# chrisquince/DESMAN

Measured on AMD Instinct MI355X. Metric: Gibbs iterations/sec (VxS updates/s) at V=10k S=64 G=8, higher is better.
Workload: dtype f64; 1 GPU; synthetic V=10000 x S=64, G=8, full Gibbs iteration, 1 chain per GPU (configs[2]); V=10000, S=64, G=8, chains=1, tau_rng=mt19937

## Files before the change

### desman_amd/_lib.py

```python
import ctypes as C
import os

import numpy as np

_HERE = os.path.dirname(os.path.abspath(__file__))
LIB_PATH = os.environ.get("DESMAN_HIP_LIB") or os.path.join(_HERE, "lib", "libdesman_hip.so")
AB_LIB_PATH = os.path.join(_HERE, "lib", "libdesman_hip_ab.so")
HEADER_PATH = os.path.join(os.path.dirname(_HERE), "include", "desman_hip.h")

DSM_OK = 0
RNG_MT19937, RNG_PHILOX = 0, 1
STATS_AGG = 2
K_NAMES = ("stats", "dirichlet", "tau", "finalize", "mt", "nmft_a", "nmft_gamma", "nmft_b", "stats2", "stats_big", "stats_pat")


class DesmanHipError(RuntimeError):
    pass


_i64p = np.ctypeslib.ndpointer(np.int64, flags="C_CONTIGUOUS")
_f64p = np.ctypeslib.ndpointer(np.float64, flags="C_CONTIGUOUS")
_u64p = np.ctypeslib.ndpointer(np.uint64, flags="C_CONTIGUOUS")
_u32p = np.ctypeslib.ndpointer(np.uint32, flags="C_CONTIGUOUS")
_i32p = np.ctypeslib.ndpointer(np.int32, flags="C_CONTIGUOUS")
_vp, _i, _d = C.c_void_p, C.c_int, C.c_double

SIGNATURES = {
    "dsm_last_error": (C.c_char_p, []),
    "dsm_device_count": (_i, []),
    "dsm_version": (C.c_char_p, []),
    "dsm_initRNG": (_i, []),
    "dsm_setRNG": (_i, [C.c_ulong]),
    "dsm_freeRNG": (_i, []),
    "dsm_sample_tau": (_i, [_i64p, _f64p, _f64p, _i64p, _i, _i, _i]),
    "c_initRNG": (None, []),
    "c_setRNG": (None, [C.c_ulong]),
    "c_freeRNG": (None, []),
    "c_sample_tau": (_i, [_i64p, _f64p, _f64p, _i64p, _i, _i, _i]),
    "dsm_getRNG_state": (_i, [_u32p]),
    "dsm_setRNG_state": (_i, [_u32p]),
    "dsm_ctx_create": (_i, [C.POINTER(_vp), _i]),
    "dsm_ctx_destroy": (_i, [_vp]),
    "dsm_ctx_sync": (_i, [_vp]),
    "dsm_ctx_set_counts": (_i, [_vp, _i64p, _i, _i]),
    "dsm_ctx_set_state": (_i, [_vp, _i64p, _f64p, _f64p, _i]),
    "dsm_ctx_get_state": (_i, [_vp, _vp, _vp, _vp]),
    "dsm_ctx_set_gamma_eta": (_i, [_vp, _vp, _vp]),
    "dsm_ctx_set_priors": (_i, [_vp, _d, _d, _d]),
    "dsm_ctx_seed": (_i, [_vp, C.c_ulong, C.c_uint64]),
    "dsm_ctx_set_tau_rng": (_i, [_vp, _i]),
    "dsm_ctx_get_mt_state": (_i, [_vp, _u32p]),
    "dsm_ctx_set_mt_state": (_i, [_vp, _u32p]),
    "dsm_mt_seed_state": (_i, [C.c_ulong, _u32p]),
    "dsm_ctx_debug_mt_fill": (_i, [_vp, C.c_size_t, _u32p]),
    "dsm_ctx_sample_tau": (_i, [_vp, C.POINTER(_i), _vp]),
    "dsm_ctx_sample_stats": (_i, [_vp, C.c_uint32, _u64p, _u64p]),
    "dsm_ctx_stats_spec": (_i, [_vp]),
    "dsm_ctx_sweep_stats": (_i, [_vp, C.POINTER(C.c_uint64), C.POINTER(C.c_uint64), _i]),
    "dsm_ctx_set_tau_screen": (_i, [_vp, _i]),
    "dsm_ctx_set_tau_neartie": (_i, [_vp, _i]),
    "dsm_ctx_set_nmft_fused": (_i, [_vp, _i]),
    "dsm_ctx_set_nmft_persist": (_i, [_vp, _i]),
    "dsm_ctx_tau_launch_info": (_i, [_vp, C.POINTER(_i), C.POINTER(_i)]),
    "dsm_ctx_debug_log2f": (_i, [_vp, _vp, _vp, C.c_size_t]),
    "dsm_debug_fdiv": (_i, [_i, _f64p, _f64p, _f64p, _i]),
    "dsm_release_device_caches": (_i, []),
    "dsm_ctx_force_stats_spec": (_i, [_vp, _i]),
    "dsm_ctx_debug_stage1": (_i, [_vp, C.c_uint32, _vp, _u64p]),
    "dsm_ctx_debug_binom": (_i, [_vp, _i, C.c_uint32, _f64p, C.c_uint64, _i, _u32p, _i]),
    "dsm_ctx_draw_gamma_eta": (_i, [_vp, C.c_uint32, _u64p, _u64p, _f64p, _f64p]),
    "dsm_ctx_loglik": (_i, [_vp, C.POINTER(_d), C.POINTER(_d)]),
    "dsm_ctx_gibbs_update": (_i, [_vp, _i]),
    "dsm_ctx_get_counters": (_i, [_vp, C.POINTER(C.c_uint64), C.POINTER(C.c_uint32)]),
    "dsm_ctx_set_counters": (_i, [_vp, C.c_uint64, C.c_uint32]),
    "dsm_ctx_get_screen_state": (_i, [_vp, _u32p]),
    "dsm_ctx_set_screen_state": (_i, [_vp, _u32p]),
    "dsm_ctx_gibbs_update_sharded": (_i, [_vp, _i, _i, _i, _vp, _vp]),
    "dsm_ctx_gibbs_update_sharded_comm": (_i, [_vp, _i, _i, _i, _vp]),
    "dsm_comm_unique_id": (_i, [_vp]),
    "dsm_comm_create": (_i, [C.POINTER(_vp), _vp, _i, _i, _i]),
    "dsm_comm_destroy": (_i, [_vp]),
    "dsm_comm_rank": (_i, [_vp]),
    "dsm_comm_world": (_i, [_vp]),
    "dsm_comm_allgather_f64": (_i, [_vp, _f64p, _f64p, C.c_size_t]),
    "dsm_comm_allreduce_f64": (_i, [_vp, _vp, C.c_size_t, _i]),
    "dsm_comm_barrier": (_i, [_vp]),
    "dsm_device_read": (_i, [_i, _vp, _vp, C.c_size_t]),
    "dsm_device_write": (_i, [_i, _vp, _vp, C.c_size_t]),
    "dsm_batch_gibbs_update": (_i, [C.POINTER(_vp), _i, _i]),
    "dsm_batch_update_tau": (_i, [C.POINTER(_vp), _i, _i, C.POINTER(_vp), C.POINTER(_vp)]),
    "dsm_batch_nmft_factorize": (_i, [C.POINTER(_vp), _i, _i, _d, _i, C.POINTER(_i), _vp]),
    "dsm_ctx_update_tau": (_i, [_vp, _i, _f64p, _f64p]),
    "dsm_ctx_get_trace": (_i, [_vp, _vp, _vp, _vp, _vp, _vp]),
    "dsm_ctx_get_star": (_i, [_vp, _vp, _vp, _vp, C.POINTER(_d), C.POINTER(_i)]),
    "dsm_ctx_get_tau_sum": (_i, [_vp, _i64p]),
    "dsm_ctx_get_tau_at": (_i, [_vp, _i, _i64p]),
    "dsm_nmft_set": (_i, [_vp, _f64p, _f64p, _i]),
    "dsm_nmft_get": (_i, [_vp, _vp, _vp]),
    "dsm_nmft_factorize": (_i, [_vp, _i, _d, _i, C.POINTER(_i), _vp]),
    "dsm_nmft_objective": (_i, [_vp, C.POINTER(_d)]),
    "dsm_nmft_debug_path": (_i, [_vp, _i, C.POINTER(_i)]),
    "dsm_nmft_get_tau": (_i, [_vp, _i64p]),
    "dsm_lrt_step": (_i, [_i, _f64p, _i32p, _i32p, _f64p, _d, _i, _i, _f64p, _f64p, _f64p]),
    "dsm_assign_tau": (_i, [_i, _i64p, _i, _i, _i, _f64p, _f64p, C.c_uint64, _vp, _vp, _vp, _vp, _vp]),
    "dsm_ctx_assign_tau": (_i, [_vp, _f64p, _f64p, _i, C.c_uint64, _vp, _vp, _vp, _vp, _vp]),
    "dsm_assign_debug_set_chunk": (_i, [_i]),
    "dsm_fit_gamma": (_i, [_i, _i64p, _i, _i, _i, _i64p, _f64p, _i, _d, _i, _vp, _vp, _vp, _vp, _vp, _vp]),
    "dsm_ctx_fit_gamma": (_i, [_vp, _i, _vp, _f64p, _i, _d, _i, _vp, _vp, _vp, _vp, _vp, _vp]),
    "dsm_abund_debug_set_chunk": (_i, [_i]),
    "dsm_fit_gamma_interval": (_i, [_i, _i64p, _i, _i, _i, _i64p, _f64p, _f64p, _d, _i, _d, _d, _vp, _vp, _vp]),
    "dsm_ctx_fit_gamma_interval": (_i, [_vp, _i, _vp, _f64p, _f64p, _d, _i, _d, _d, _vp, _vp, _vp]),
    "dsm_genes_create": (_i, [C.POINTER(_vp), _i]),
    "dsm_genes_destroy": (_i, [_vp]),
    "dsm_genes_set_data": (_i, [_vp, _vp, _i, _i, _i, _i32p, _f64p]),
    "dsm_genes_set_model": (_i, [_vp, _f64p, _f64p, _f64p, _i, _i, _f64p, _f64p, _f64p]),
    "dsm_genes_set_state": (_i, [_vp, _vp, _vp]),
    "dsm_genes_get_state": (_i, [_vp, _vp, _vp]),
    "dsm_genes_seed": (_i, [_vp, C.c_ulong, C.c_uint64]),
    "dsm_genes_set_gene_base": (_i, [_vp, _i]),
    "dsm_genes_get_mt_state": (_i, [_vp, _u32p]),
    "dsm_genes_set_mt_state": (_i, [_vp, _u32p]),
    "dsm_genes_nmft_tau": (_i, [_vp, _vp, _f64p, _i, _d, _vp]),
    "dsm_genes_sweep_all": (_i, [_vp, _vp, _i, _vp, _vp, _vp]),
    "dsm_genes_step_candidates": (_i, [_vp, _i, _i, _f64p, _vp]),
    "dsm_genes_step_choose": (_i, [_vp, _i, _i, _i]),
    "dsm_genes_update": (_i, [_vp, _i, _i, _vp, _vp, _vp, _vp]),
    "dsm_genes_loglik": (_i, [_vp, _vp]),
    "dsm_genes_get_star": (_i, [_vp, _vp, _vp]),
    "dsm_genes_set_star": (_i, [_vp, _vp, _vp]),
    "dsm_genes_debug_tile": (_i, [_vp, C.POINTER(_i), C.POINTER(_i), C.POINTER(_i), C.POINTER(C.c_size_t)]),
    "dsm_kl_assign": (_i, [_i, _f64p, _f64p, _f64p, _i, _i, _i, _i, _d, C.POINTER(_i), C.POINTER(_d)]),
    "dsm_ctx_set_timing": (_i, [_vp, _i]),
    "dsm_ctx_get_timing": (_i, [_vp, _vp, _vp]),
    "dsm_kernel_name": (C.c_char_p, [_i]),
}

EXCHANGE_FN = C.CFUNCTYPE(C.c_int, C.c_void_p, C.c_void_p, C.c_size_t, C.c_void_p, C.c_size_t)
_lib = None


def _digest(a):
    try:
        import xxhash
# ... 259 lines not shown
        return dict(tau=tau, gamma=gamma, eta=eta, mt_state=mt, ctr_seed=np.uint64(key), iter_ctr=np.uint32(it), screen=self.screen_state())

    def counters(self):
        key, it = C.c_uint64(0), C.c_uint32(0)
        check(self.lib.dsm_ctx_get_counters(self._h, C.byref(key), C.byref(it)))
        return int(key.value), int(it.value)

    def screen_state(self):
        out = np.zeros(2, dtype=np.uint32)
        check(self.lib.dsm_ctx_get_screen_state(self._h, out))
        return out

    def set_screen_state(self, words):
        check(self.lib.dsm_ctx_set_screen_state(self._h, np.ascontiguousarray(words, dtype=np.uint32)))

    def restore(self, ck):
        self.set_state(np.ascontiguousarray(ck["tau"], dtype=np.int64), np.ascontiguousarray(ck["gamma"], dtype=np.float64),
                       np.ascontiguousarray(ck["eta"], dtype=np.float64))
        mt = np.asarray(ck["mt_state"], dtype=np.uint32)
        if mt.size == 625:
            self.set_mt_state(np.ascontiguousarray(mt))
        check(self.lib.dsm_ctx_set_counters(self._h, int(ck["ctr_seed"]), int(ck["iter_ctr"])))
        self.set_screen_state(ck["screen"] if "screen" in ck else np.zeros(2, dtype=np.uint32))

    def set_mt_state(self, st):
        check(self.lib.dsm_ctx_set_mt_state(self._h, np.ascontiguousarray(st, dtype=np.uint32)))

    def debug_mt_fill(self, n):
        out = np.empty(int(n), dtype=np.uint32)
        check(self.lib.dsm_ctx_debug_mt_fill(self._h, int(n), out))
        return out

    def set_tau_rng(self, mode):
        check(self.lib.dsm_ctx_set_tau_rng(self._h, int(mode)))

    def assign_tau(self, gamma, eta, seed=None):
        gamma, eta = _assign_model(gamma, eta, self.S)
        G = gamma.shape[1]
        out = _assign_out(self.V, G, seed)
        check(self.lib.dsm_ctx_assign_tau(self._h, gamma, eta, G, int(seed or 0) & 0xFFFFFFFFFFFFFFFF, _ptr(out["map_state"]),
                                          _ptr(out["conf"]), _ptr(out["logz"]), _ptr(out["marg"]), _ptr(out.get("draw_state"))))
        return out

    def fit_gamma(self, eta, tau=None, max_iter=FIT_MAX_ITER, tol=FIT_TOL, presence=False):
        eta = _fit_eta(eta)
        t = None if tau is None else _fit_tau(tau, self.V)
        G = self.G if t is None else t.shape[1]
        out = _fit_out(self.S, G, presence)
        check(self.lib.dsm_ctx_fit_gamma(self._h, G, _ptr(t), eta, int(max_iter), float(tol), int(bool(presence)), _ptr(out["gamma"]),
                                         _ptr(out["loglik"]), _ptr(out["deviance"]), _ptr(out["iters"]), _ptr(out["converged"]),
                                         _ptr(out.get("lr_absent"))))
        return out

    def fit_gamma_interval(self, eta, gamma_hat, tau=None, level=0.95, q=None, max_iter=FIT_MAX_ITER, tol=FIT_TOL, ctol=FIT_CTOL):
        eta = _fit_eta(eta)
        t = None if tau is None else _fit_tau(tau, self.V)
        G = self.G if t is None else t.shape[1]
        g, q, out = _interval_args(gamma_hat, self.S, G, level, q)
        check(self.lib.dsm_ctx_fit_gamma_interval(self._h, G, _ptr(t), eta, g, q, int(max_iter), float(tol), float(ctol), _ptr(out["lo"]),
                                                  _ptr(out["hi"]), _ptr(out["flags"])))
        return out

    def sample_tau(self, want_logp=False):
        n = _i(0)
        logp = np.empty((self.V, self.G, 4)) if want_logp else None
        check(self.lib.dsm_ctx_sample_tau(self._h, C.byref(n), _ptr(logp)))
        return (n.value, logp) if want_logp else n.value

    def sample_stats(self, it):
        mu = np.zeros((self.S, self.G), dtype=np.uint64)
        E = np.zeros((4, 4), dtype=np.uint64)
        check(self.lib.dsm_ctx_sample_stats(self._h, int(it), mu, E))
        return mu, E

    def debug_log2f(self, x):
        x = np.ascontiguousarray(x, dtype=np.float32)
        out = np.empty_like(x)
        check(self.lib.dsm_ctx_debug_log2f(self._h, x.ctypes.data, out.ctypes.data, x.size))
        return out

    def set_tau_neartie(self, mode=-1):
        check(self.lib.dsm_ctx_set_tau_neartie(self._h, int(mode)))

    def set_tau_screen(self, on):
        check(self.lib.dsm_ctx_set_tau_screen(self._h, 1 if on else 0))

    def tau_launch_info(self):
        a, b = _i(0), _i(0)
        check(self.lib.dsm_ctx_tau_launch_info(self._h, C.byref(a), C.byref(b)))
        return a.value, b.value

    def set_nmft_persist(self, mode=-1):
        check(self.lib.dsm_ctx_set_nmft_persist(self._h, int(mode)))

    def set_nmft_fused(self, mode=-1):
        check(self.lib.dsm_ctx_set_nmft_fused(self._h, int(mode)))

    def sweep_stats(self, reset=False):
        a, b = C.c_uint64(0), C.c_uint64(0)
        check(self.lib.dsm_ctx_sweep_stats(self._h, C.byref(a), C.byref(b), 1 if reset else 0))
        return a.value, b.value

    def stats_spec(self):
        r = self.lib.dsm_ctx_stats_spec(self._h)
        if r < 0:
            check(r)
        return r

    def force_stats_spec(self, spec=0):
        check(self.lib.dsm_ctx_force_stats_spec(self._h, int(spec)))

    def debug_stage1(self, it):
        nt = np.zeros((self.S, 1 << self.G), dtype=np.uint32)
        E = np.zeros((4, 4), dtype=np.uint64)
        check(self.lib.dsm_ctx_debug_stage1(self._h, int(it), nt.ctypes.data, E))
        return nt, E

    def debug_binom(self, kind, n, w, seed, nsamp, spec=STATS_AGG):
        w4 = np.zeros(4)
        w4[:len(w)] = w
        out = np.zeros((nsamp, 4) if kind == 2 else nsamp, dtype=np.uint32)
        check(self.lib.dsm_ctx_debug_binom(self._h, int(kind), int(n), w4, int(seed), int(nsamp), out.reshape(-1), int(spec)))
        return out

    def draw_gamma_eta(self, it, sum_mu, esum):
        g = np.empty((self.S, self.G)); e = np.empty((4, 4))
        check(self.lib.dsm_ctx_draw_gamma_eta(self._h, int(it), np.ascontiguousarray(sum_mu, dtype=np.uint64),
                                              np.ascontiguousarray(esum, dtype=np.uint64), g, e))
        return g, e

    def loglik(self):
        ll, lp = _d(0), _d(0)
        check(self.lib.dsm_ctx_loglik(self._h, C.byref(ll), C.byref(lp)))
        return ll.value, lp.value

    def gibbs_update(self, n_iter):
        check(self.lib.dsm_ctx_gibbs_update(self._h, int(n_iter)))
        self.n_trace = int(n_iter)

    def gibbs_update_sharded(self, n_iter, v_offset, v_total, exchange):
        err = []

        def cb(user, tab, n_tab, vec, n_vec):
            try:
                exchange(tab or 0, int(n_tab), vec, int(n_vec))
                return 0
            except BaseException as e:
                err.append(e)
                return 1
        fn = EXCHANGE_FN(cb)
        rc = self.lib.dsm_ctx_gibbs_update_sharded(self._h, int(n_iter), int(v_offset), int(v_total), C.cast(fn, _vp), None)
        if err:
            raise err[0]
        check(rc)
        self.n_trace = int(n_iter)

    def gibbs_update_sharded_comm(self, n_iter, v_offset, v_total, comm):
        check(self.lib.dsm_ctx_gibbs_update_sharded_comm(self._h, int(n_iter), int(v_offset), int(v_total), comm._h))
        self.n_trace = int(n_iter)

    @staticmethod
    def batch_gibbs_update(ctxs, n_iter):
        ctxs = list(ctxs)
        arr = (_vp * len(ctxs))(*[c._h.value for c in ctxs])
        check(load().dsm_batch_gibbs_update(arr, len(ctxs), int(n_iter)))
        for c in ctxs:
            c.n_trace = int(n_iter)

    def update_tau(self, gamma_store, eta_store):
        g = np.ascontiguousarray(gamma_store, dtype=np.float64)
        e = np.ascontiguousarray(eta_store, dtype=np.float64)
        check(self.lib.dsm_ctx_update_tau(self._h, g.shape[0], g, e))
        self.n_trace = g.shape[0]

    def get_trace(self):
        n = self.n_trace
        ll = np.empty(n); lp = np.empty(n); nch = np.empty(n, dtype=np.int32)
        g = np.empty((n, self.S, self.G)); e = np.empty((n, 4, 4))
        check(self.lib.dsm_ctx_get_trace(self._h, _ptr(ll), _ptr(lp), _ptr(nch), _ptr(g), _ptr(e)))
        return dict(ll=ll, lp=lp, nchange=nch, gamma=g, eta=e)

    def get_star(self):
        tau = np.empty((self.V, self.G, 4), dtype=np.int64)
        g = np.empty((self.S, self.G)); e = np.empty((4, 4))
        lp, it = _d(0), _i(0)
        check(self.lib.dsm_ctx_get_star(self._h, _ptr(tau), _ptr(g), _ptr(e), C.byref(lp), C.byref(it)))
        return dict(tau=tau, gamma=g, eta=e, lp=lp.value, it=it.value)

    def get_tau_sum(self):
        out = np.empty((self.V, self.G, 4), dtype=np.int64)
        check(self.lib.dsm_ctx_get_tau_sum(self._h, out))
        return out

    def get_tau_at(self, it):
        out = np.empty((self.V, self.G, 4), dtype=np.int64)
        check(self.lib.dsm_ctx_get_tau_at(self._h, int(it), out))
        return out

    def nmft_set(self, tau, gamma):
# ... 199 lines not shown
```

### desman_amd/csrc/api.hip

```cpp
#include <math.h>
#include <stdarg.h>
#include <stdio.h>
#include <string.h>

#include <algorithm>
#include <mutex>
#include <numeric>
#include <thread>

#include "dsm_host.h"
#include "log_table.h"

static thread_local char g_err[512] = "";

void dsm_set_error(const char *fmt, ...)
{
    va_list ap;
    va_start(ap, fmt);
    vsnprintf(g_err, sizeof g_err, fmt, ap);
    va_end(ap);
}

extern "C" const char *dsm_last_error(void) { return g_err; }
extern "C" const char *dsm_version(void) { return "desman_hip 0.1 (gfx950)"; }
// ... 81 lines not shown
static void dev_free(T **p) { if (*p) { (void)hipFree(*p); *p = nullptr; } }

template <typename T>
struct Scratch {
    T *p = nullptr;
    ~Scratch() { if (p) (void)hipFree(p); }
    int alloc(size_t n) { return dev_alloc(&p, n); }
    operator T *() const { return p; }
    Scratch() = default;
    Scratch(const Scratch &) = delete;
    Scratch &operator=(const Scratch &) = delete;
};

#define TRY(x) do { int _r = (x); if (_r != DSM_OK) return _r; } while (0)
#define BIND(c) HIP_TRY(hipSetDevice((c)->device))

static int need(dsm_ctx *c, bool counts, bool state)
{
    if (!c) { dsm_set_error("null context"); return DSM_ERR_ARG; }
    if (counts && !c->cnt_vs) { dsm_set_error("no count tensor: call dsm_ctx_set_counts first"); return DSM_ERR_STATE; }
    if (state && !c->have_state) { dsm_set_error("no chain state: call dsm_ctx_set_state first"); return DSM_ERR_STATE; }
    return DSM_OK;
}

static int esum_reset(dsm_ctx *c)
{
    HIP_TRY(hipMemsetAsync(c->esum, 0, (16 + 16 * DSM_ESUM_PARTS) * sizeof(unsigned long long), c->stream));
    return DSM_OK;
}

static int reset_blk_order(dsm_ctx *c)
{
    static const std::vector<uint32_t> ident = [] { std::vector<uint32_t> v((size_t)2 * DSM_MAX_GRID); for (size_t i = 0; i < v.size(); ++i) v[i] = (uint32_t)(i % DSM_MAX_GRID); return v; }();
    c->blk_order_n[0] = c->blk_order_n[1] = 0;
    if (!c->blk_order) return DSM_OK;
    HIP_TRY(hipMemcpyAsync(c->blk_order, ident.data(), ident.size() * sizeof(uint32_t), hipMemcpyHostToDevice, c->stream));
    return DSM_OK;
}

extern "C" int dsm_ctx_create(dsm_ctx **out, int device)
{
    if (!out) return DSM_ERR_ARG;
    *out = nullptr;
    int n = dsm_device_count();
    if (n <= 0) { dsm_set_error("no HIP device visible"); return DSM_ERR_NODEVICE; }
    if (device < 0 || device >= n) { dsm_set_error("device %d out of range (0..%d)", device, n - 1); return DSM_ERR_ARG; }
    HIP_TRY(hipSetDevice(device));
    hipDeviceProp_t prop;
    HIP_TRY(hipGetDeviceProperties(&prop, device));
    if (strncmp(prop.gcnArchName, "gfx950", 6) != 0) {
        dsm_set_error("device %d is %s; this library is built for gfx950 only", device, prop.gcnArchName);
        return DSM_ERR_NODEVICE;
    }
    dsm_ctx *c = new dsm_ctx();
    c->device = device;
    HIP_TRY(hipStreamCreateWithFlags(&c->stream, hipStreamNonBlocking));
    if (getenv("DESMAN_HIP_ONE_STREAM")) c->stream_rng = c->stream;
    else {
        int lo = 0, hi = 0;
        HIP_TRY(hipDeviceGetStreamPriorityRange(&lo, &hi));
        HIP_TRY(hipStreamCreateWithPriority(&c->stream_rng, hipStreamNonBlocking, hi));
    }
    for (int i = 0; i < 2; ++i) {
        HIP_TRY(hipEventCreateWithFlags(&c->ev_u_ready[i], hipEventDisableTiming));
        HIP_TRY(hipEventCreateWithFlags(&c->ev_u_free[i], hipEventDisableTiming));
    }
    TRY(dev_alloc(&c->mt_state, 625));
    TRY(dev_alloc(&c->ll_partial, 2 * DSM_MAX_GRID));
    TRY(dev_alloc(&c->nchange, 2));
    TRY(dev_alloc(&c->sweep_stats, 2));
    HIP_TRY(hipMemsetAsync(c->sweep_stats, 0, 2 * sizeof(unsigned long long), c->stream));
    TRY(dev_alloc(&c->step_cnt, (size_t)2 * 2 * DSM_MAX_GRID));
    HIP_TRY(hipMemsetAsync(c->step_cnt, 0, (size_t)2 * 2 * DSM_MAX_GRID * sizeof(uint32_t), c->stream));
    TRY(dev_alloc(&c->blk_order, (size_t)2 * DSM_MAX_GRID));
    TRY(reset_blk_order(c));
    TRY(dev_alloc(&c->screen_ctl, 4));
    HIP_TRY(hipMemsetAsync(c->screen_ctl, 0, 4 * sizeof(uint32_t), c->stream));
    TRY(dev_alloc(&c->prior, 2 * (DSM_MAX_S + 4)));
    TRY(dev_alloc(&c->scalars, 8));
    TRY(dev_alloc(&c->star, 2));
    TRY(dev_alloc(&c->eta, 16));
    TRY(dev_alloc(&c->eta_new, 16));
    TRY(dev_alloc(&c->eta_star, 16));
    TRY(dev_alloc(&c->esum, 16 + 16 * DSM_ESUM_PARTS));
    TRY(dev_alloc(&c->log_tab, 2 * DSM_LOG_TAB_N + DSM_EXP_TAB_N));
    HIP_TRY(hipMemcpyAsync(c->log_tab, dsm_log_table_host, sizeof dsm_log_table_host, hipMemcpyHostToDevice, c->stream));
    HIP_TRY(hipMemcpyAsync(c->log_tab + 2 * DSM_LOG_TAB_N, dsm_exp_table_host, sizeof dsm_exp_table_host, hipMemcpyHostToDevice, c->stream));
    HIP_TRY(hipMemsetAsync(c->nchange, 0, 2 * sizeof(int), c->stream));
    TRY(esum_reset(c));
    HIP_TRY(hipStreamSynchronize(c->stream));
    *out = c;
    return DSM_OK;
}

static void free_traces(dsm_ctx *c)
{
    dev_free(&c->tau_trace); dev_free(&c->ll_trace); dev_free(&c->lp_trace); dev_free(&c->nchange_trace);
    dev_free(&c->gamma_trace); dev_free(&c->eta_trace); dev_free(&c->gamma_in); dev_free(&c->eta_in);
    c->in_cap = 0;
    c->n_trace = 0;
    c->trace_cap = 0;
}

extern "C" int dsm_ctx_destroy(dsm_ctx *c)
{
    if (!c) return DSM_OK;
    (void)hipSetDevice(c->device);
    (void)hipStreamSynchronize(c->stream);
    collect_spans(c);
    for (auto e : c->free_events) (void)hipEventDestroy(e);
    free_traces(c);
    dev_free(&c->cnt_vs); dev_free(&c->items); dev_free(&c->nitems); dev_free(&c->tau);
    dev_free(&c->pat_rep); dev_free(&c->pat_x); dev_free(&c->pat_list); c->pat_rep_len = c->pat_x_len = 0;
    if (c->h_rare) { (void)hipHostFree(c->h_rare); c->h_rare = nullptr; }
    dev_free(&c->s2_scratch);
    dev_free(&c->blk_tab); stats_release_ntab(c); dev_free(&c->big_list); dev_free(&c->big_count);
    dev_free(&c->gamma); dev_free(&c->eta);
    dev_free(&c->eta_new); dev_free(&c->sum_mu); dev_free(&c->esum); dev_free(&c->mt_state); dev_free(&c->mt_jstates); dev_free(&c->u_raw);
    dev_free(&c->ll_partial); dev_free(&c->nchange); dev_free(&c->sweep_stats); dev_free(&c->step_cnt); dev_free(&c->blk_order); dev_free(&c->screen_ctl); dev_free(&c->prior); dev_free(&c->prior_all); dev_free(&c->scalars); dev_free(&c->star);
    dev_free(&c->gamma_star); dev_free(&c->eta_star); dev_free(&c->log_tab); dev_free(&c->shard_vec); dev_free(&c->np_part); if (c->np_bar) { (void)hipFree(c->np_bar); c->np_bar = nullptr; } dev_free(&c->F); dev_free(&c->ntau); dev_free(&c->ntau2); dev_free(&c->ngam); dev_free(&c->ngam_raw);
    dev_free(&c->npart); dev_free(&c->nstat); dev_free(&c->ngam2); dev_free(&c->ngam_raw2);
    for (int i = 0; i < 2; ++i) { (void)hipEventDestroy(c->ev_u_ready[i]); (void)hipEventDestroy(c->ev_u_free[i]); }
    if (c->stream_rng != c->stream) (void)hipStreamDestroy(c->stream_rng);
    (void)hipStreamDestroy(c->stream);
    delete c;
    return DSM_OK;
}

extern "C" int dsm_ctx_sync(dsm_ctx *c)
{
    if (!c) return DSM_ERR_ARG;
    BIND(c);
    HIP_TRY(hipStreamSynchronize(c->stream));
    HIP_TRY(hipStreamSynchronize(c->stream_rng));
    return DSM_OK;
}

extern "C" int dsm_ctx_set_counts(dsm_ctx *c, const int64_t *variants, int V, int S)
{
    if (!c || !variants || V < 1 || S < 1) { dsm_set_error("set_counts: bad arguments"); return DSM_ERR_ARG; }
    if (S > DSM_MAX_S) { dsm_set_error("S=%d exceeds DSM_MAX_S=%d", S, DSM_MAX_S); return DSM_ERR_UNSUPPORTED; }
    if ((int64_t)V * S >= ((int64_t)1 << 32)) { dsm_set_error("V*S must be below 2^32"); return DSM_ERR_UNSUPPORTED; }
    BIND(c);
    HIP_TRY(hipStreamSynchronize(c->stream));
    HIP_TRY(hipStreamSynchronize(c->stream_rng));
    const size_t n = (size_t)V * S;
    c->V = V; c->S = S;
    c->have_state = false;
    c->G = 0;
    TRY(dev_alloc(&c->cnt_vs, n * 4));
    TRY(dev_alloc(&c->nitems, (size_t)S));
    TRY(dev_alloc(&c->tau, (size_t)V));
    dev_free(&c->F); dev_free(&c->ntau); dev_free(&c->ntau2); dev_free(&c->ngam); dev_free(&c->ngam_raw); c->nG = 0;
    free_traces(c);
    Scratch<int64_t> d_in; Scratch<int> d_flag; Scratch<double> d_part; Scratch<unsigned long long> d_depth;
    const int nblk = (int)((n + 255) / 256 < 1024 ? (n + 255) / 256 : 1024);
    TRY(d_in.alloc(n * 4));
    TRY(d_flag.alloc(1));
    TRY(d_part.alloc((size_t)nblk));
    TRY(d_depth.alloc((size_t)S));
    HIP_TRY(hipMemcpyAsync(d_in, variants, n * 4 * sizeof(int64_t), hipMemcpyHostToDevice, c->stream));
    HIP_TRY(hipMemsetAsync(d_flag, 0, sizeof(int), c->stream));
    HIP_TRY(hipMemsetAsync(d_depth, 0, (size_t)S * sizeof(unsigned long long), c->stream));
    TRY(k_convert_counts(c, d_in, d_flag, d_part, nblk, d_depth));
    std::vector<double> part(nblk);
    std::vector<unsigned long long> dep((size_t)S);
    int flag = 0;
    HIP_TRY(hipMemcpyAsync(part.data(), d_part, nblk * sizeof(double), hipMemcpyDeviceToHost, c->stream));
    HIP_TRY(hipMemcpyAsync(dep.data(), d_depth, (size_t)S * sizeof(unsigned long long), hipMemcpyDeviceToHost, c->stream));
    HIP_TRY(hipMemcpyAsync(&flag, d_flag, sizeof(int), hipMemcpyDeviceToHost, c->stream));
    HIP_TRY(hipStreamSynchronize(c->stream));
    c->items_built = false;
    c->max_items = 0;
    c->blk_gmax = 0;
    c->stats_grid = 0;
    dev_free(&c->pat_x); c->pat_x_len = 0;
    TRY(reset_blk_order(c));
    HIP_TRY(hipMemsetAsync(c->screen_ctl, 0, 4 * sizeof(uint32_t), c->stream));
    dev_free(&c->items);
    c->depth.assign((size_t)S, 0);
    c->max_depth = 0;
    for (int s = 0; s < S; ++s) { c->depth[s] = (int64_t)dep[s]; c->max_depth = std::max<uint64_t>(c->max_depth, dep[s]); }
    if (flag) {
        dev_free(&c->cnt_vs); dev_free(&c->items);
        dsm_set_error("set_counts: negative count or depth above 2^31-1");
        return DSM_ERR_ARG;
    }
    double s = 0.0;
    for (double p : part) s += p;
    c->ll_const = s;
    return DSM_OK;
}

int build_stats_items(dsm_ctx *c)
{
    const int V = c->V, S = c->S;
    std::vector<int32_t> cnt((size_t)V * S * 4);
    HIP_TRY(hipMemcpyAsync(cnt.data(), c->cnt_vs, cnt.size() * sizeof(int32_t), hipMemcpyDeviceToHost, c->stream));
    HIP_TRY(hipStreamSynchronize(c->stream));
    const int64_t cells = (int64_t)V * S;
    const int CH = cells <= 65536 ? 64 : cells <= 262144 ? 128 : 0;
    c->chunked = CH != 0;
    std::vector<int32_t> nit(S);
    std::vector<std::vector<std::pair<int32_t, int32_t>>> lst((size_t)S);
    std::vector<int32_t> top(S, 0);
    for (int s = 0; s < S; ++s) lst[s].reserve((size_t)V * 2);
    for (int v = 0; v < V; ++v) {
        const int32_t *row = cnt.data() + (size_t)v * S * 4;
        for (int s = 0; s < S; ++s)
            for (int b = 0; b < 4; ++b) {
                const int64_t x = row[s * 4 + b];
                if (x <= 0) continue;
                if (!CH) {
                    lst[s].emplace_back((int32_t)x, v * 4 + b);
                    if (x > top[s]) top[s] = (int32_t)x;
                } else {
                    for (int64_t j = 0; j * CH < x; ++j) {
                        const int32_t nrd = (int32_t)(x - j * CH < CH ? x - j * CH : CH);
                        lst[s].emplace_back(nrd | (int32_t)(j << 12), v * 4 + b);
                        if (nrd > top[s]) top[s] = nrd;
                    }
                }
            }
    }
    int max_items = 0;
    for (int s = 0; s < S; ++s) max_items = std::max(max_items, (int)lst[s].size());
    c->item_stride = max_items > 0 ? max_items : 1;
    std::vector<int32_t> items((size_t)S * c->item_stride * 2, 0);
    TRY(dev_alloc(&c->items, items.size()));
    std::vector<int32_t> first;
    const int32_t rd_mask = CH ? 0xfff : 0x7fffffff;
    for (int s = 0; s < S; ++s) {
        const auto &l = lst[s];
        nit[s] = (int32_t)l.size();
        int32_t *dst = items.data() + (size_t)s * c->item_stride * 2;
        if (top[s] <= (1 << 20)) {
            first.assign((size_t)top[s] + 2, 0);
            for (const auto &e : l) first[e.first & rd_mask]++;
            int32_t run = 0;
            for (int32_t cval = top[s]; cval >= 1; --cval) { const int32_t h = first[cval]; first[cval] = run; run += h; }
            for (const auto &e : l) { const int32_t k = first[e.first & rd_mask]++; dst[2 * k] = e.second; dst[2 * k + 1] = e.first; }
        } else {
            std::vector<std::pair<int32_t, int32_t>> t(l);
            std::stable_sort(t.begin(), t.end(), [](const std::pair<int32_t, int32_t> &p, const std::pair<int32_t, int32_t> &q) { return p.first > q.first; });
            for (size_t k = 0; k < t.size(); ++k) { dst[2 * k] = t[k].second; dst[2 * k + 1] = t[k].first; }
        }
    }
    c->max_items = max_items;
    c->nitems_h = nit;
    c->blk_gmax = 0;
    HIP_TRY(hipMemcpyAsync(c->items, items.data(), items.size() * sizeof(int32_t), hipMemcpyHostToDevice, c->stream));
    HIP_TRY(hipMemcpyAsync(c->nitems, nit.data(), (size_t)S * sizeof(int32_t), hipMemcpyHostToDevice, c->stream));
    HIP_TRY(hipStreamSynchronize(c->stream));
    c->items_built = true;
    return DSM_OK;
}

static int ensure_state_buffers(dsm_ctx *c, int G)
{
    if (G < 1 || G > DSM_MAX_G) { dsm_set_error("G=%d outside 1..%d", G, DSM_MAX_G); return DSM_ERR_UNSUPPORTED; }
    if (G != c->G || !c->gamma) {
        c->G = G;
        const size_t sg = (size_t)c->S * G;
        TRY(dev_alloc(&c->gamma, sg));
        TRY(dev_alloc(&c->gamma_star, sg));
        TRY(dev_alloc(&c->sum_mu, sg));
        HIP_TRY(hipMemsetAsync(c->sum_mu, 0, sg * sizeof(unsigned long long), c->stream));
        c->stats_grid = 0;
        c->u_cap = (size_t)c->V * G;
        c->u_chunk_words = c->u_cap * std::max<size_t>(1, std::min<size_t>(DSM_U_CHUNK, ((size_t)16 << 20) / std::max<size_t>(1, c->u_cap)));
        TRY(dev_alloc(&c->u_raw, 2 * c->u_chunk_words));
        free_traces(c);
    }
    return DSM_OK;
}

extern "C" int dsm_ctx_set_state(dsm_ctx *c, const int64_t *tau, const double *gamma, const double *eta, int G)
{
    TRY(need(c, true, false));
    if (!tau || !gamma || !eta) { dsm_set_error("set_state: null pointer"); return DSM_ERR_ARG; }
    BIND(c);
    HIP_TRY(hipStreamSynchronize(c->stream));
    TRY(ensure_state_buffers(c, G));
    const size_t nt = (size_t)c->V * G * 4;
    Scratch<int64_t> d_t;
    TRY(d_t.alloc(nt));
    HIP_TRY(hipMemcpyAsync(d_t, tau, nt * sizeof(int64_t), hipMemcpyHostToDevice, c->stream));
    TRY(k_pack_tau(c, d_t, c->tau, c->V, G));
    HIP_TRY(hipMemcpyAsync(c->gamma, gamma, (size_t)c->S * G * sizeof(double), hipMemcpyHostToDevice, c->stream));
    c->tau_rare_n = tau_rare_from_host(gamma, c->S, G);
    HIP_TRY(hipMemcpyAsync(c->eta, eta, 16 * sizeof(double), hipMemcpyHostToDevice, c->stream));
    HIP_TRY(hipStreamSynchronize(c->stream));
    c->have_state = true;
    return DSM_OK;
}

extern "C" int dsm_ctx_set_gamma_eta(dsm_ctx *c, const double *gamma, const double *eta)
{
    TRY(need(c, true, true));
    BIND(c);
    if (gamma) HIP_TRY(hipMemcpyAsync(c->gamma, gamma, (size_t)c->S * c->G * sizeof(double), hipMemcpyHostToDevice, c->stream));
    if (gamma) c->tau_rare_n = tau_rare_from_host(gamma, c->S, c->G);
    if (eta) HIP_TRY(hipMemcpyAsync(c->eta, eta, 16 * sizeof(double), hipMemcpyHostToDevice, c->stream));
    HIP_TRY(hipStreamSynchronize(c->stream));
    return DSM_OK;
}

static int fetch_tau(dsm_ctx *c, const uint64_t *d_packed, int64_t *host_onehot)
{
    const size_t nt = (size_t)c->V * c->G * 4;
    Scratch<int64_t> d_t;
    TRY(d_t.alloc(nt));
    TRY(k_unpack_tau(c, d_packed, d_t, c->V, c->G));
    HIP_TRY(hipMemcpyAsync(host_onehot, d_t, nt * sizeof(int64_t), hipMemcpyDeviceToHost, c->stream));
    HIP_TRY(hipStreamSynchronize(c->stream));
    return DSM_OK;
}

extern "C" int dsm_ctx_get_state(dsm_ctx *c, int64_t *tau, double *gamma, double *eta)
{
    TRY(need(c, true, true));
    BIND(c);
    if (tau) TRY(fetch_tau(c, c->tau, tau));
    if (gamma) HIP_TRY(hipMemcpyAsync(gamma, c->gamma, (size_t)c->S * c->G * sizeof(double), hipMemcpyDeviceToHost, c->stream));
    if (eta) HIP_TRY(hipMemcpyAsync(eta, c->eta, 16 * sizeof(double), hipMemcpyDeviceToHost, c->stream));
    HIP_TRY(hipStreamSynchronize(c->stream));
    return DSM_OK;
}

extern "C" int dsm_ctx_set_priors(dsm_ctx *c, double alpha, double delta, double epsilon)
{
    if (!c || !(alpha > 0) || !(delta > 0) || !(epsilon >= 0)) { dsm_set_error("set_priors: bad value"); return DSM_ERR_ARG; }
    c->alpha = alpha; c->delta = delta; c->epsilon = epsilon;
    return DSM_OK;
}

static void mt_seed_host(uint32_t *st, unsigned long seed)
{
    if (seed == 0) seed = 4357;
    st[0] = (uint32_t)(seed & 0xffffffffUL);
    for (int i = 1; i < 624; ++i) st[i] = 1812433253u * (st[i - 1] ^ (st[i - 1] >> 30)) + (uint32_t)i;
    st[624] = 624;
}

static int seed_mt(dsm_ctx *c, unsigned long seed)
{
    uint32_t st[625];
    mt_seed_host(st, seed);
    HIP_TRY(hipStreamSynchronize(c->stream_rng));
    HIP_TRY(hipMemcpyAsync(c->mt_state, st, sizeof st, hipMemcpyHostToDevice, c->stream));
    HIP_TRY(hipStreamSynchronize(c->stream));
    c->mt_seeded = true;
    return DSM_OK;
}

extern "C" int dsm_ctx_seed(dsm_ctx *c, unsigned long mt_seed, uint64_t ctr_seed)
{
    if (!c) return DSM_ERR_ARG;
    BIND(c);
    c->ctr_seed = ctr_seed;
    c->iter_ctr = 0;
    return seed_mt(c, mt_seed);
}

extern "C" int dsm_ctx_get_screen_state(dsm_ctx *c, uint32_t *out2)
{
    if (!c || !out2) { dsm_set_error("get_screen_state: null argument"); return DSM_ERR_ARG; }
    BIND(c);
    HIP_TRY(hipMemcpyAsync(out2, c->screen_ctl, 2 * sizeof(uint32_t), hipMemcpyDeviceToHost, c->stream));
    HIP_TRY(hipStreamSynchronize(c->stream));
    return DSM_OK;
}
extern "C" int dsm_ctx_set_screen_state(dsm_ctx *c, const uint32_t *in2)
{
    if (!c || !in2) { dsm_set_error("set_screen_state: null argument"); return DSM_ERR_ARG; }
// ... 110 lines not shown
            if (filled < total) TRY(fill_next());
            HIP_TRY(hipStreamWaitEvent(c->stream, c->ev_u_ready[slot], 0));
        }
        *u = c->u_raw + (size_t)slot * c->u_chunk_words + (size_t)(it - first[slot]) * c->u_cap;
        return DSM_OK;
    }
    int release(int it)
    {
        if (!active()) return DSM_OK;
        for (int slot = 0; slot < 2; ++slot)
            if (len[slot] && it == first[slot] + len[slot] - 1) HIP_TRY(hipEventRecord(c->ev_u_free[slot], c->stream));
        return DSM_OK;
    }
};

extern "C" int dsm_ctx_sample_tau(dsm_ctx *c, int *nchange, double *logp_out)
{
    TRY(need(c, true, true));
    BIND(c);
    Scratch<double> d_logp;
    const size_t nl = (size_t)c->V * c->G * 4;
    if (logp_out) TRY(d_logp.alloc(nl));
    const uint32_t *u = nullptr;
    SweepWords words(c, 1);
    HIP_TRY(hipMemsetAsync(c->nchange, 0, sizeof(int), c->stream));
    TRY(words.acquire(0, &u));
    TRY(k_tau_sweep(c, 1, c->gamma, c->eta, c->eta, nullptr, d_logp, c->iter_ctr++, nullptr, u));
    TRY(words.release(0));
    int n = 0;
    HIP_TRY(hipMemcpyAsync(&n, c->nchange, sizeof(int), hipMemcpyDeviceToHost, c->stream));
    if (logp_out) HIP_TRY(hipMemcpyAsync(logp_out, d_logp, nl * sizeof(double), hipMemcpyDeviceToHost, c->stream));
    HIP_TRY(hipMemsetAsync(c->nchange, 0, sizeof(int), c->stream));
    HIP_TRY(hipStreamSynchronize(c->stream));
    if (nchange) *nchange = n;
    return DSM_OK;
}

extern "C" int dsm_ctx_sample_stats(dsm_ctx *c, uint32_t iter, uint64_t *sum_mu, uint64_t *esum)
{
    TRY(need(c, true, true));
    BIND(c);
    const size_t sg = (size_t)c->S * c->G;
    HIP_TRY(hipMemsetAsync(c->sum_mu, 0, sg * sizeof(unsigned long long), c->stream));
    TRY(stats_ensure_ntab(c));
    TRY(esum_reset(c));
    TRY(k_stats(c, iter));
    TRY(k_esum_fold(c));
    if (sum_mu) HIP_TRY(hipMemcpyAsync(sum_mu, c->sum_mu, sg * sizeof(uint64_t), hipMemcpyDeviceToHost, c->stream));
    if (esum) HIP_TRY(hipMemcpyAsync(esum, c->esum, 16 * sizeof(uint64_t), hipMemcpyDeviceToHost, c->stream));
    HIP_TRY(hipMemsetAsync(c->sum_mu, 0, sg * sizeof(unsigned long long), c->stream));
    TRY(esum_reset(c));
    HIP_TRY(hipStreamSynchronize(c->stream));
    return DSM_OK;
}

extern "C" int dsm_ctx_stats_spec(dsm_ctx *c)
{
    if (!c || c->G < 1) { dsm_set_error("stats_spec: no chain state"); return DSM_ERR_STATE; }
    return stats_spec(c);
}

extern "C" int dsm_ctx_force_stats_spec(dsm_ctx *c, int spec)
{
    if (!c || spec < 0 || spec > 4) { dsm_set_error("force_stats_spec: 0 (rule), 1, 2, 3 or 4"); return DSM_ERR_ARG; }
    c->force_stats_spec = spec;
    return DSM_OK;
}

extern "C" int dsm_ctx_debug_stage1(dsm_ctx *c, uint32_t iter, uint32_t *ntab, uint64_t *esum)
{
    TRY(need(c, true, true));
    if (stats_spec(c) < 2) { dsm_set_error("debug_stage1: the aggregated specification does not apply to this shape (force it with dsm_ctx_force_stats_spec)"); return DSM_ERR_UNSUPPORTED; }
    BIND(c);
    TRY(esum_reset(c));
    TRY(k_stats_stage1(c, iter));
    TRY(k_esum_fold(c));
    const size_t NH = (size_t)1 << c->G, S = (size_t)c->S;
    const size_t ld = (size_t)c->ntab_ld;
    std::vector<uint32_t> t((size_t)c->ntab_rep * NH * ld);
    HIP_TRY(hipMemcpyAsync(t.data(), c->ntab, t.size() * sizeof(uint32_t), hipMemcpyDeviceToHost, c->stream));
    if (esum) HIP_TRY(hipMemcpyAsync(esum, c->esum, 16 * sizeof(uint64_t), hipMemcpyDeviceToHost, c->stream));
    HIP_TRY(hipMemsetAsync(c->ntab, 0, t.size() * sizeof(uint32_t), c->stream));
    TRY(esum_reset(c));
    HIP_TRY(hipMemsetAsync(c->big_count, 0, DSM_BIG_NT * DSM_BIG_NL * DSM_BIG_STRIDE * sizeof(uint32_t), c->stream));
    HIP_TRY(hipStreamSynchronize(c->stream));
    if (ntab)
        for (size_t h = 0; h < NH; ++h)
            for (size_t s = 0; s < S; ++s) {
                uint32_t v = 0;
                for (int r = 0; r < c->ntab_rep; ++r) v += t[((size_t)r * NH + ((h * DSM_NTAB_HMUL + (s >> 4) * DSM_NTAB_SWZ) & (NH - 1))) * ld + s];
                ntab[s * NH + h] = v;
            }
    return DSM_OK;
}

extern "C" int dsm_ctx_debug_binom(dsm_ctx *c, int kind, uint32_t n, const double *w4, uint64_t seed, int nsamp, uint32_t *out, int spec)
{
    if (!c || !w4 || !out || nsamp < 1 || kind < 0 || kind > 2 || spec < 2 || spec > 3) { dsm_set_error("debug_binom: bad arguments"); return DSM_ERR_ARG; }
    BIND(c);
    const size_t len = (size_t)nsamp * (kind == 2 ? 4 : 1);
    Scratch<uint32_t> d;
    TRY(d.alloc(len));
    TRY(k_binom_test(c, kind, n, w4, seed, nsamp, d, spec));
    HIP_TRY(hipMemcpyAsync(out, d, len * sizeof(uint32_t), hipMemcpyDeviceToHost, c->stream));
    HIP_TRY(hipStreamSynchronize(c->stream));
    return DSM_OK;
}

extern "C" int dsm_ctx_draw_gamma_eta(dsm_ctx *c, uint32_t iter, const uint64_t *sum_mu, const uint64_t *esum,
                                      double *gamma_out, double *eta_out)
{
    TRY(need(c, true, true));
    if (!sum_mu || !esum) { dsm_set_error("draw_gamma_eta: null sums"); return DSM_ERR_ARG; }
    BIND(c);
    const size_t sg = (size_t)c->S * c->G;
    Scratch<double> d_g, d_e;
    TRY(d_g.alloc(sg));
    TRY(d_e.alloc(16));
    HIP_TRY(hipMemcpyAsync(c->sum_mu, sum_mu, sg * sizeof(uint64_t), hipMemcpyHostToDevice, c->stream));
    HIP_TRY(hipMemcpyAsync(c->esum, esum, 16 * sizeof(uint64_t), hipMemcpyHostToDevice, c->stream));
    TRY(k_dirichlet(c, iter, d_g, nullptr, d_e, nullptr, c->prior, -1, 0, nullptr));
    if (gamma_out) HIP_TRY(hipMemcpyAsync(gamma_out, d_g, sg * sizeof(double), hipMemcpyDeviceToHost, c->stream));
    if (eta_out) HIP_TRY(hipMemcpyAsync(eta_out, d_e, 16 * sizeof(double), hipMemcpyDeviceToHost, c->stream));
    HIP_TRY(hipStreamSynchronize(c->stream));
    return DSM_OK;
}

static int eval_state(dsm_ctx *c, const double *gamma, const double *eta, uint64_t *trace_slot, int star_mode)
{
    int nb = 0;
    TRY(k_prior(c, gamma, eta, c->prior));
    TRY(k_tau_sweep(c, 2, gamma, eta, eta, trace_slot, nullptr, 0, &nb, nullptr));
    return k_finalize(c, nb, -1, star_mode, c->prior, gamma, eta);
}

extern "C" int dsm_ctx_loglik(dsm_ctx *c, double *ll, double *lp)
{
    TRY(need(c, true, true));
    BIND(c);
    double sc[2];
    TRY(eval_state(c, c->gamma, c->eta, nullptr, 2));
    HIP_TRY(hipMemcpyAsync(sc, c->scalars, sizeof sc, hipMemcpyDeviceToHost, c->stream));
    HIP_TRY(hipStreamSynchronize(c->stream));
    if (ll) *ll = sc[0];
    if (lp) *lp = sc[1];
    return DSM_OK;
}

static int alloc_traces(dsm_ctx *c, int n)
{
    const size_t sg = (size_t)c->S * c->G;
    if (n > c->trace_cap || !c->tau_trace) {
        free_traces(c);
        const int want = n;
        if (n < 512 && (size_t)513 * c->V * sizeof(uint64_t) <= ((size_t)1 << 30)) n = 512;
        TRY(dev_alloc(&c->tau_trace, (size_t)(n + 1) * c->V));
        TRY(dev_alloc(&c->ll_trace, (size_t)n));
        TRY(dev_alloc(&c->lp_trace, (size_t)n));
        TRY(dev_alloc(&c->nchange_trace, (size_t)n));
        TRY(dev_alloc(&c->gamma_trace, (size_t)n * sg));
        TRY(dev_alloc(&c->eta_trace, (size_t)n * 16));
        c->trace_cap = n;
        n = want;
    }
    c->n_trace = n;
    return DSM_OK;
}

thread_local BatchCtl g_batch;

struct Chains {
    dsm_ctx *const *c;
    int K;
    bool batched;
    struct Home { hipStream_t stream, stream_rng; bool timing; int nmft_fused; };
    std::vector<Home> home;
    dsm_ctx *lead() const { return c[0]; }
    ~Chains()
    {
        if (home.empty()) return;
        (void)hipStreamSynchronize(lead()->stream);
        (void)hipStreamSynchronize(lead()->stream_rng);
        for (size_t k = 0; k < home.size(); ++k) {
            c[k]->stream = home[k].stream; c[k]->stream_rng = home[k].stream_rng; c[k]->timing = home[k].timing; c[k]->nmft_fused = home[k].nmft_fused;
        }
    }
    template <class Fits> int open(bool state, bool nmft, Fits fits)
    {
        if (!c || K < 1 || K > DSM_MAX_BATCH) { dsm_set_error("batch of %d chains (1..%d)", K, DSM_MAX_BATCH); return DSM_ERR_ARG; }
        for (int k = 0; k < K; ++k) {
            TRY(need(c[k], true, state));
            const dsm_ctx *a = c[0], *b = c[k];
            if (b->device != a->device || b->V != a->V || b->S != a->S) { dsm_set_error("batch: chain %d differs from chain 0 in device or shape", k); return DSM_ERR_ARG; }
            TRY(fits(a, b, k));
            for (int j = 0; j < k; ++j) if (c[j] == b) { dsm_set_error("batch: chain %d listed twice", k); return DSM_ERR_ARG; }
        }
        BIND(lead());
        for (int k = 0; batched && k < K; ++k) {
            HIP_TRY(hipStreamSynchronize(c[k]->stream));
            HIP_TRY(hipStreamSynchronize(c[k]->stream_rng));
            home.push_back(Home{c[k]->stream, c[k]->stream_rng, c[k]->timing, c[k]->nmft_fused});
            c[k]->stream = lead()->stream; c[k]->stream_rng = lead()->stream_rng; c[k]->timing = false;
            if (nmft) c[k]->nmft_fused = home[0].nmft_fused;
        }
        return DSM_OK;
    }
    template <class F> int each(F f) const
    {
        for (int k = 0; k < K; ++k) TRY(f(c[k], k));
        return DSM_OK;
    }
    template <class F> int launch(F f) const
    {
        int r = DSM_OK;
        for (int k = 0; k < K && r == DSM_OK; ++k) {
            if (batched) g_batch = BatchCtl{K, k};
            r = f(c[k], k);
        }
        g_batch = BatchCtl{};
        return r;
    }
};

static int same_G_and_rng(const dsm_ctx *a, const dsm_ctx *b, int k)
{
    if (b->G != a->G || b->tau_rng != a->tau_rng) { dsm_set_error("batch: chain %d differs from chain 0 in shape or tau RNG", k); return DSM_ERR_ARG; }
    return DSM_OK;
}

static double *prior_slot(dsm_ctx *c, int it) { return c->prior + (it & 1) * (DSM_MAX_S + 4); }

static int gibbs_update(dsm_ctx *const *ctxs, int K, bool batched, int n_iter)
{
    if (n_iter < 0) { dsm_set_error("n_iter < 0"); return DSM_ERR_ARG; }
    Chains ch{ctxs, K, batched};
    TRY(ch.open(true, false, [](const dsm_ctx *a, const dsm_ctx *b, int k) -> int {
        TRY(same_G_and_rng(a, b, k));
        if (stats_spec(b) == stats_spec(a)) return DSM_OK;
        dsm_set_error("batch: chain %d runs mu/E specification %d, chain 0 specification %d (different tables or different dsm_ctx_force_stats_spec)", k, stats_spec(b), stats_spec(a));
        return DSM_ERR_ARG;
    }));
    dsm_ctx *const lead = ch.lead();
    const int spec = stats_spec(lead);
    const bool agg = spec >= 2;
    const bool fuse_s2 = agg && lead->G < 10;
    const size_t sg = (size_t)lead->S * lead->G;
    std::vector<SweepWords> words;
    words.reserve(K);
    std::vector<int> nb_prev(K, 0);
    std::vector<uint32_t> ic(K);
    std::vector<const uint32_t *> u(K, nullptr);
    TRY(ch.each([&](dsm_ctx *c, int) -> int {
        TRY(alloc_traces(c, n_iter));
        HIP_TRY(hipMemsetAsync(c->nchange, 0, sizeof(int), c->stream));
        TRY(eval_state(c, c->gamma, c->eta, c->tau_trace, 1));
        TRY(stats_ensure_ntab(c));
        if (!batched) TRY(k_tau_neartie_hint(c));
        words.emplace_back(c, n_iter);
        return DSM_OK;
    }));
    TRY(ch.launch([&](dsm_ctx *, int k) { return words[k].prefetch(); }));
    for (int it = 0; it < n_iter; ++it) {
        if (!batched && it && (it & 63) == 0 && lead->tau_neartie_mode == -1) { TRY(k_tau_rare_count(lead, true)); TRY(k_tau_neartie_hint(lead)); }
        TRY(ch.launch([&](dsm_ctx *c, int k) { ic[k] = c->iter_ctr++; return agg ? k_stats_stage1(c, ic[k]) : k_stats_v1(c, ic[k]); }));
        if (agg && !fuse_s2) TRY(ch.launch([&](dsm_ctx *c, int k) { return k_stats_stage2(c, ic[k]); }));
        TRY(ch.launch([&](dsm_ctx *c, int k) {
            return k_dirichlet(c, ic[k], c->gamma, c->gamma_trace + (size_t)it * sg, c->eta_new, c->eta_trace + (size_t)it * 16,
                               prior_slot(c, it), it - 1, nb_prev[k], prior_slot(c, it - 1), fuse_s2 ? 1 : 0);
        }));
        TRY(ch.launch([&](dsm_ctx *, int k) { return words[k].acquire(it, &u[k]); }));
        TRY(ch.launch([&](dsm_ctx *c, int k) {
            return k_tau_sweep(c, 3, c->gamma, c->eta, c->eta_new, c->tau_trace + (size_t)(it + 1) * c->V, nullptr, ic[k], &nb_prev[k], u[k]);
        }));
        TRY(ch.each([&](dsm_ctx *c, int k) -> int {
            TRY(words[k].release(it));
            std::swap(c->eta, c->eta_new);
            return DSM_OK;
        }));
    }
    const bool want_rare = !batched && n_iter > 0 && lead->tau_neartie_mode == -1;
    if (want_rare && !lead->h_rare) HIP_TRY(hipHostMalloc((void **)&lead->h_rare, sizeof(int), hipHostMallocDefault));
    if (n_iter > 0)
        TRY(ch.each([&](dsm_ctx *c, int k) {
            return k_finalize(c, nb_prev[k], n_iter - 1, 0, prior_slot(c, n_iter - 1), c->gamma_trace + (size_t)(n_iter - 1) * sg,
                              c->eta_trace + (size_t)(n_iter - 1) * 16, 0, want_rare ? c->h_rare : nullptr);
        }));
    HIP_TRY(hipStreamSynchronize(lead->stream));
    if (want_rare) lead->tau_rare_n = *lead->h_rare;
    return DSM_OK;
}

extern "C" int dsm_ctx_gibbs_update(dsm_ctx *c, int n_iter) { return gibbs_update(&c, 1, false, n_iter); }

extern "C" int dsm_batch_gibbs_update(dsm_ctx *const *ctxs, int K, int n_iter) { return gibbs_update(ctxs, K, true, n_iter); }

struct dsm_comm;
int comm_enqueue_exchange(dsm_comm *m, uint32_t *tab, size_t n_tab, double *vec, size_t n_vec, hipStream_t stream);
int comm_device(const dsm_comm *m);

static int gibbs_update_sharded(dsm_ctx *c, int n_iter, int v_offset, int v_total, dsm_exchange_fn exchange, void *user, dsm_comm *comm)
{
    TRY(need(c, true, true));
    c->tau_neartie_on = false;
    if (n_iter < 0 || (!exchange && !comm) || v_offset < 0 || v_total < v_offset + c->V) { dsm_set_error("gibbs_update_sharded: bad arguments"); return DSM_ERR_ARG; }
    if (comm && comm_device(comm) != c->device) { dsm_set_error("gibbs_update_sharded: the communicator lives on device %d, the context on %d", comm_device(comm), c->device); return DSM_ERR_ARG; }
    if (c->tau_rng != DSM_RNG_PHILOX) { dsm_set_error("gibbs_update_sharded: needs counter-based tau uniforms (DSM_RNG_PHILOX)"); return DSM_ERR_STATE; }
    BIND(c);
    const int keep_force = c->force_stats_spec;
    if (c->force_stats_spec < 2) c->force_stats_spec = DSM_STATS_AGG;
    struct Guard { dsm_ctx *c; int f; ~Guard() { c->shard_on = false; c->force_stats_spec = f; } } guard{c, keep_force};
    if (stats_spec(c) < 2) { dsm_set_error("gibbs_update_sharded: the aggregated mu/E pass does not apply to this shape (G <= 16)"); return DSM_ERR_UNSUPPORTED; }
    if (!c->shard_vec) TRY(dev_alloc(&c->shard_vec, (size_t)18));
    c->shard_on = true; c->shard_voff = v_offset; c->shard_vtot = v_total;
    TRY(alloc_traces(c, n_iter));
    const size_t sg = (size_t)c->S * c->G;
    HIP_TRY(hipMemsetAsync(c->nchange, 0, sizeof(int), c->stream));
    TRY(esum_reset(c));
    auto swap_vec = [&](uint32_t *tab, size_t n_tab) -> int {
        if (comm) return comm_enqueue_exchange(comm, tab, n_tab, c->shard_vec, (size_t)18, c->stream);
        HIP_TRY(hipStreamSynchronize(c->stream));
        if (exchange(user, tab, n_tab, c->shard_vec, (size_t)18) != 0) { dsm_set_error("gibbs_update_sharded: the exchange callback failed"); return DSM_ERR_STATE; }
        return DSM_OK;
    };
    {
        int nb = 0;
        TRY(k_prior(c, c->gamma, c->eta, c->prior));
        TRY(k_tau_sweep(c, 2, c->gamma, c->eta, c->eta, c->tau_trace, nullptr, 0, &nb, nullptr));
        TRY(k_shard_pack(c, nb));
        TRY(swap_vec(nullptr, 0));
        TRY(k_finalize(c, nb, -1, 1, c->prior, c->gamma, c->eta));
        TRY(esum_reset(c));
    }
    TRY(stats_ensure_ntab(c));
    double *const P[2] = {c->prior, c->prior + (DSM_MAX_S + 4)};
    int nb_prev = 0;
    for (int it = 0; it < n_iter; ++it) {
        const uint32_t ic = c->iter_ctr++;
        const bool fuse_s2 = c->G < 10;
        TRY(k_stats_stage1(c, ic));
        TRY(k_shard_pack(c, nb_prev));
        TRY(swap_vec(c->ntab, c->ntab_len));
        TRY(k_shard_unpack(c));
        if (!fuse_s2) TRY(k_stats_stage2(c, ic));
        TRY(k_dirichlet(c, ic, c->gamma, c->gamma_trace + (size_t)it * sg, c->eta_new, c->eta_trace + (size_t)it * 16,
                        P[it & 1], it - 1, nb_prev, P[(it - 1) & 1], fuse_s2 ? 1 : 0));
        TRY(k_tau_sweep(c, 3, c->gamma, c->eta, c->eta_new, c->tau_trace + (size_t)(it + 1) * c->V, nullptr, ic, &nb_prev, nullptr));
        std::swap(c->eta, c->eta_new);
    }
    if (n_iter > 0) {
        TRY(k_shard_pack(c, nb_prev));
        TRY(swap_vec(nullptr, 0));
        TRY(k_finalize(c, nb_prev, n_iter - 1, 0, P[(n_iter - 1) & 1], c->gamma_trace + (size_t)(n_iter - 1) * sg,
                       c->eta_trace + (size_t)(n_iter - 1) * 16));
        TRY(esum_reset(c));
    }
    HIP_TRY(hipStreamSynchronize(c->stream));
    return DSM_OK;
}

extern "C" int dsm_ctx_gibbs_update_sharded(dsm_ctx *c, int n_iter, int v_offset, int v_total, dsm_exchange_fn exchange, void *user)
{
    if (!exchange) { dsm_set_error("gibbs_update_sharded: no exchange callback"); return DSM_ERR_ARG; }
    return gibbs_update_sharded(c, n_iter, v_offset, v_total, exchange, user, nullptr);
}

extern "C" int dsm_ctx_gibbs_update_sharded_comm(dsm_ctx *c, int n_iter, int v_offset, int v_total, dsm_comm *comm)
{
    if (!comm) { dsm_set_error("gibbs_update_sharded_comm: no communicator"); return DSM_ERR_ARG; }
    return gibbs_update_sharded(c, n_iter, v_offset, v_total, nullptr, nullptr, comm);
}

// ... 43 lines not shown
    words.reserve(K);
    TRY(ch.each([&](dsm_ctx *c, int) -> int { TRY(alloc_traces(c, n_iter)); words.emplace_back(c, n_iter); return DSM_OK; }));
    TRY(ch.launch([&](dsm_ctx *, int k) { return words[k].prefetch(); }));
    TRY(ch.each([&](dsm_ctx *c, int k) { return tau_inputs(c, n_iter, gamma_stores[k], eta_stores[k]); }));
    std::vector<int> nb_prev(K, 0);
    std::vector<const uint32_t *> u(K, nullptr);
    for (int it = 0; it < n_iter; ++it) {
        TRY(ch.launch([&](dsm_ctx *, int k) { return words[k].acquire(it, &u[k]); }));
        TRY(ch.launch([&](dsm_ctx *c, int k) -> int {
            const uint32_t ic = c->iter_ctr++;
            const double *g = c->gamma_in + (size_t)it * sg, *e = c->eta_in + (size_t)it * 16;
            TauFinalRider rider;
            if (it > 0) {
                rider.nblocks = nb_prev[k]; rider.it = it - 1; rider.prior = c->prior_all + (size_t)(it - 1) * (c->S + 4);
                rider.gamma_src = c->gamma_in + (size_t)(it - 1) * sg; rider.eta_src = c->eta_in + (size_t)(it - 1) * 16;
            }
            return k_tau_sweep(c, 3, g, e, e, c->tau_trace + (size_t)(it + 1) * c->V, nullptr, ic, &nb_prev[k], u[k], it & 1,
                               it > 0 ? &rider : nullptr);
        }));
        TRY(ch.each([&](dsm_ctx *, int k) { return words[k].release(it); }));
    }
    TRY(ch.each([&](dsm_ctx *c, int k) {
        return k_finalize(c, nb_prev[k], n_iter - 1, 0, c->prior_all + (size_t)(n_iter - 1) * (c->S + 4),
                          c->gamma_in + (size_t)(n_iter - 1) * sg, c->eta_in + (size_t)(n_iter - 1) * 16, (n_iter - 1) & 1);
    }));
    HIP_TRY(hipStreamSynchronize(ch.lead()->stream));
    return DSM_OK;
}

extern "C" int dsm_ctx_update_tau(dsm_ctx *c, int n_iter, const double *gamma_store, const double *eta_store) { return update_tau(&c, 1, false, n_iter, &gamma_store, &eta_store); }

extern "C" int dsm_batch_update_tau(dsm_ctx *const *ctxs, int K, int n_iter, const double *const *gamma_stores, const double *const *eta_stores)
{
    return update_tau(ctxs, K, true, n_iter, gamma_stores, eta_stores);
}

extern "C" int dsm_release_device_caches(void)
{
    mt_jump_release();
    return DSM_OK;
}

extern "C" int dsm_ctx_debug_log2f(dsm_ctx *c, const float *in, float *out, size_t n)
{
    if (!c || !in || !out) { dsm_set_error("debug_log2f: bad arguments"); return DSM_ERR_ARG; }
    if (n == 0) return DSM_OK;
    BIND(c);
    Scratch<float> d_in, d_out;
    TRY(d_in.alloc(n)); TRY(d_out.alloc(n));
    HIP_TRY(hipMemcpyAsync(d_in, in, n * sizeof(float), hipMemcpyHostToDevice, c->stream));
    TRY(k_log2f_test(c, d_in, d_out, n));
    HIP_TRY(hipMemcpyAsync(out, d_out, n * sizeof(float), hipMemcpyDeviceToHost, c->stream));
    HIP_TRY(hipStreamSynchronize(c->stream));
    return DSM_OK;
}

extern "C" int dsm_ctx_tau_launch_info(dsm_ctx *c, int *launched, int *resident)
{
    TRY(need(c, true, true));
    if (!launched || !resident) { dsm_set_error("tau_launch_info: null argument"); return DSM_ERR_ARG; }
    BIND(c);
    return tau_launch_info(c, launched, resident);
}

extern "C" int dsm_ctx_set_nmft_persist(dsm_ctx *c, int mode)
{
    if (!c || mode < -1 || mode > 1) { dsm_set_error("set_nmft_persist: mode -1, 0 or 1"); return DSM_ERR_ARG; }
    c->nmft_persist = mode;
    return DSM_OK;
}

extern "C" int dsm_ctx_set_nmft_fused(dsm_ctx *c, int mode)
{
    if (!c || mode < -1 || mode > 3 || mode == 2) { dsm_set_error("set_nmft_fused: mode -1, 0, 1 or 3"); return DSM_ERR_ARG; }
    c->nmft_fused = mode;
    return DSM_OK;
}

extern "C" int dsm_ctx_set_tau_neartie(dsm_ctx *c, int mode)
{
    if (!c || mode < -1 || mode > 1) { dsm_set_error("set_tau_neartie: -1 (by the abundances), 0 or 1"); return DSM_ERR_ARG; }
    c->tau_neartie_mode = mode;
    return DSM_OK;
}

extern "C" int dsm_ctx_set_tau_screen(dsm_ctx *c, int on)
{
    if (!c) { dsm_set_error("set_tau_screen: null context"); return DSM_ERR_ARG; }
    c->tau_screen = on != 0;
    return DSM_OK;
}

extern "C" int dsm_ctx_sweep_stats(dsm_ctx *c, uint64_t *steps, uint64_t *exact_steps, int mode)
{
    if (!c || mode < 0 || mode > 1) { dsm_set_error("sweep_stats: bad arguments"); return DSM_ERR_ARG; }
    BIND(c);
    unsigned long long h[2] = {0, 0};
    HIP_TRY(hipMemcpyAsync(h, c->sweep_stats, sizeof h, hipMemcpyDeviceToHost, c->stream));
    if (mode == 1) HIP_TRY(hipMemsetAsync(c->sweep_stats, 0, sizeof h, c->stream));
    HIP_TRY(hipStreamSynchronize(c->stream));
    if (steps) *steps = h[0];
    if (exact_steps) *exact_steps = h[1];
    return DSM_OK;
}

extern "C" int dsm_ctx_get_trace(dsm_ctx *c, double *ll, double *lp, int32_t *nchange, double *gamma_store, double *eta_store)
{
    TRY(need(c, true, true));
    BIND(c);
    const size_t n = (size_t)c->n_trace, sg = (size_t)c->S * c->G;
    if (n == 0) return DSM_OK;
    if (ll) HIP_TRY(hipMemcpyAsync(ll, c->ll_trace, n * sizeof(double), hipMemcpyDeviceToHost, c->stream));
    if (lp) HIP_TRY(hipMemcpyAsync(lp, c->lp_trace, n * sizeof(double), hipMemcpyDeviceToHost, c->stream));
    if (nchange) HIP_TRY(hipMemcpyAsync(nchange, c->nchange_trace, n * sizeof(int), hipMemcpyDeviceToHost, c->stream));
    if (gamma_store) HIP_TRY(hipMemcpyAsync(gamma_store, c->gamma_trace, n * sg * sizeof(double), hipMemcpyDeviceToHost, c->stream));
    if (eta_store) HIP_TRY(hipMemcpyAsync(eta_store, c->eta_trace, n * 16 * sizeof(double), hipMemcpyDeviceToHost, c->stream));
    HIP_TRY(hipStreamSynchronize(c->stream));
    return DSM_OK;
}

extern "C" int dsm_ctx_get_star(dsm_ctx *c, int64_t *tau_star, double *gamma_star, double *eta_star, double *lp_star, int *iter_star)
{
    TRY(need(c, true, true));
    if (!c->tau_trace) { dsm_set_error("get_star: no update has run"); return DSM_ERR_STATE; }
    BIND(c);
    double st[2];
    HIP_TRY(hipMemcpyAsync(st, c->star, sizeof st, hipMemcpyDeviceToHost, c->stream));
    HIP_TRY(hipStreamSynchronize(c->stream));
    const int slot = (int)st[1];
    if (tau_star) TRY(fetch_tau(c, c->tau_trace + (size_t)slot * c->V, tau_star));
    if (gamma_star) HIP_TRY(hipMemcpyAsync(gamma_star, c->gamma_star, (size_t)c->S * c->G * sizeof(double), hipMemcpyDeviceToHost, c->stream));
    if (eta_star) HIP_TRY(hipMemcpyAsync(eta_star, c->eta_star, 16 * sizeof(double), hipMemcpyDeviceToHost, c->stream));
    HIP_TRY(hipStreamSynchronize(c->stream));
    if (lp_star) *lp_star = st[0];
    if (iter_star) *iter_star = slot > 0 ? slot - 1 : 0;
    return DSM_OK;
}

extern "C" int dsm_ctx_get_tau_sum(dsm_ctx *c, int64_t *tau_sum)
{
    TRY(need(c, true, true));
    if (!c->tau_trace || !tau_sum) { dsm_set_error("get_tau_sum: no update has run"); return DSM_ERR_STATE; }
    BIND(c);
    const size_t nt = (size_t)c->V * c->G * 4;
    Scratch<int64_t> d;
    TRY(d.alloc(nt));
    TRY(k_tau_sum(c, c->tau_trace, c->n_trace, d));
    HIP_TRY(hipMemcpyAsync(tau_sum, d, nt * sizeof(int64_t), hipMemcpyDeviceToHost, c->stream));
    HIP_TRY(hipStreamSynchronize(c->stream));
    return DSM_OK;
}

extern "C" int dsm_ctx_get_tau_at(dsm_ctx *c, int it, int64_t *tau)
{
    TRY(need(c, true, true));
    if (!c->tau_trace || !tau || it < -1 || it >= c->n_trace) { dsm_set_error("get_tau_at: bad iteration"); return DSM_ERR_ARG; }
    BIND(c);
    return fetch_tau(c, c->tau_trace + (size_t)(it + 1) * c->V, tau);
}

extern "C" int dsm_nmft_set(dsm_ctx *c, const double *tau, const double *gamma, int G)
{
    TRY(need(c, true, false));
    if (!tau || !gamma || G < 1 || G > DSM_MAX_G) { dsm_set_error("nmft_set: bad arguments"); return DSM_ERR_ARG; }
    BIND(c);
    HIP_TRY(hipStreamSynchronize(c->stream));
// ... 336 lines not shown
```

### desman_amd/csrc/dsm_host.h

```cpp
#pragma once
#include <hip/hip_runtime.h>
#include <stdint.h>
#include <string>
#include <vector>

#include "../../include/desman_hip.h"

#define DSM_MAX_GRID 4096
#define DSM_ESUM_PARTS 64
#define DSM_BIG_NL 64
#define DSM_BIG_STRIDE 16
#define DSM_BIG_NT 3
#define DSM_U_CHUNK 8

#define DSM_STATS_AGG 2
#define DSM_MAX_BATCH 8

void dsm_set_error(const char *fmt, ...);

#ifdef DSM_AB_SWITCHES
#define DSM_AB_ENV(name) getenv(name)
#else
#define DSM_AB_ENV(name) ((const char *)nullptr)
#endif

struct BatchCtl { int K = 0, k = 0; };
extern thread_local BatchCtl g_batch;
template <class P> struct BatchArgs { P p[DSM_MAX_BATCH]; };
#define LAUNCH_OR_COLLECT(PT, P, NORMAL, BATCHED)                                          \
    do {                                                                                    \
        if (g_batch.K == 0) { NORMAL; }                                                     \
        else {                                                                              \
            static thread_local BatchArgs<PT> acc;                                          \
            acc.p[g_batch.k] = (P);                                                         \
            if (g_batch.k == g_batch.K - 1) { const int K = g_batch.K; (void)K; BATCHED; }  \
        }                                                                                   \
    } while (0)

#define HIP_TRY(expr)                                                                       \
    do {                                                                                    \
        hipError_t _e = (expr);                                                             \
        if (_e != hipSuccess) {                                                             \
            dsm_set_error("%s failed: %s (%s:%d)", #expr, hipGetErrorString(_e), __FILE__, \
                          __LINE__);                                                        \
            return DSM_ERR_HIP;                                                             \
        }                                                                                   \
    } while (0)

struct TimedSpan { int k; hipEvent_t e0, e1; };

struct dsm_ctx {
    int device = 0;
    hipStream_t stream = nullptr;
    hipStream_t stream_rng = nullptr;
    hipEvent_t ev_u_ready[2] = {nullptr, nullptr}, ev_u_free[2] = {nullptr, nullptr};
    int V = 0, S = 0, G = 0;
    int32_t *cnt_vs = nullptr;
    int32_t *items = nullptr;
    int32_t *nitems = nullptr;
    int max_items = 0;
    bool items_built = false;
    uint64_t max_depth = 0;
    int force_stats_spec = 0;
    uint32_t *ntab = nullptr;
    size_t ntab_len = 0;
    unsigned long long *pat_rep = nullptr;
    uint32_t *pat_x = nullptr;
    uint32_t *pat_list = nullptr;
    size_t pat_rep_len = 0, pat_x_len = 0;
    uint32_t pat_gen = 0;
    uint32_t *s2_scratch = nullptr;
    uint32_t *ntab_raw = nullptr;
    int ntab_ld = 0;
    int ntab_rep = 1;
    unsigned long long *big_list = nullptr;
    uint32_t *big_count = nullptr;
    size_t big_cap = 0;
    int stats_grid = 0;
    int stats_grid_key = -1;
    int item_stride = 1;
    bool chunked = false;
    int32_t *blk_tab = nullptr;
    int blk_n = 0, blk_gmax = 0;
    std::vector<int64_t> depth;
    std::vector<int32_t> nitems_h;
    double ll_const = 0.0;
    uint64_t *tau = nullptr;
    double *gamma = nullptr;
    double *eta = nullptr;
    double *eta_new = nullptr;
    bool have_state = false;
    double alpha = 0.1, delta = 0.1, epsilon = 1e-6;
    unsigned long long *sum_mu = nullptr;
    unsigned long long *esum = nullptr;
    uint32_t *mt_state = nullptr;
    uint32_t *mt_jstates = nullptr;
    bool mt_seeded = false;
    uint32_t *u_raw = nullptr;
    size_t u_cap = 0;
    size_t u_chunk_words = 0;
    bool mt_attr_set = false;
    uint64_t ctr_seed = 0x243F6A8885A308D3ull;
    uint32_t iter_ctr = 0;
    int tau_rng = DSM_RNG_MT19937;
    double *ll_partial = nullptr;
    int *nchange = nullptr;
    unsigned long long *sweep_stats = nullptr;
    uint32_t *blk_order = nullptr;
    int tau_resident = 0, tau_resident_key = -1;
    int blk_order_n[2] = {0, 0};
    uint32_t *step_cnt = nullptr;
    uint32_t *screen_ctl = nullptr;
    bool tau_screen = true;
    int tau_neartie_mode = -1;
    bool tau_neartie_on = false;
    int tau_rare_n = 0;
    int *h_rare = nullptr;
    double *prior_all = nullptr;
    double *prior = nullptr;
    double *scalars = nullptr;
    double *log_tab = nullptr;
    int n_trace = 0, trace_cap = 0;
    uint64_t *tau_trace = nullptr;
    double *ll_trace = nullptr, *lp_trace = nullptr;
    int *nchange_trace = nullptr;
    double *gamma_trace = nullptr;
    double *eta_trace = nullptr;
    double *gamma_in = nullptr, *eta_in = nullptr;
    int in_cap = 0;
    double *star = nullptr;
    double *gamma_star = nullptr;
    double *eta_star = nullptr;
    bool shard_on = false;
    int shard_voff = 0, shard_vtot = 0;
    double *shard_vec = nullptr;
    double *F = nullptr;
    double *ntau = nullptr;
    double *ntau2 = nullptr;
    double *ngam = nullptr;
    double *ngam_raw = nullptr;
    int npart_cols = 0;
    double *npart = nullptr;
    double *nstat = nullptr;
    double *ndiv_trace = nullptr;
    int nG = 0;
    int nmft_blocks = 0;
    int nmft_persist = -1;
    double *np_part = nullptr;
    size_t np_cap = 0;
    unsigned *np_bar = nullptr;
    int nmft_fix_gamma = 0;
    int nmft_fused = -1;
    double *ngam2 = nullptr, *ngam_raw2 = nullptr;
    int nmft_gstep = 0, nmft_gstep_parity = 0, nmft_gstep_max_iter = 0;
    double nmft_gstep_min_change = 0.0;
    bool timing = false;
    std::vector<TimedSpan> spans;
    std::vector<hipEvent_t> free_events;
    double k_ms[DSM_K_COUNT] = {0};
    int64_t k_launches[DSM_K_COUNT] = {0};
};

struct KTimer {
    dsm_ctx *c; int k; hipStream_t st; hipEvent_t e0 = nullptr, e1 = nullptr;
    KTimer(dsm_ctx *ctx, int kid, hipStream_t stream = nullptr);
    ~KTimer();
};

int k_convert_counts(dsm_ctx *c, const int64_t *d_in, int *d_flag, double *d_partial, int nblk, unsigned long long *d_depth);
int k_pack_tau(dsm_ctx *c, const int64_t *d_onehot, uint64_t *d_packed, int V, int G);
int k_unpack_tau(dsm_ctx *c, const uint64_t *d_packed, int64_t *d_onehot, int V, int G);
int k_tau_sum(dsm_ctx *c, const uint64_t *trace, int n, int64_t *d_sum);
int k_mt_fill(dsm_ctx *c, uint32_t *out, size_t n, hipStream_t stream);
int k_stats_v1(dsm_ctx *c, uint32_t iter);
int k_log2f_test(dsm_ctx *c, const float *d_in, float *d_out, size_t n);
int build_stats_items(dsm_ctx *c);

#define DSM_NTAB_HMUL 0x9E3779B1u
#define DSM_NTAB_SWZ 17u
int stats_ensure_ntab(dsm_ctx *c);
void stats_release_ntab(dsm_ctx *c);
void mt_jump_release();
int stats_ntab_rep(const dsm_ctx *c);
int stats_spec(const dsm_ctx *c);
static inline int stats_draw_version(int spec) { return spec == 4 ? 2 : spec; }
int k_tau_neartie_hint(dsm_ctx *c);
int k_tau_rare_count(dsm_ctx *c, bool wait);
int tau_rare_from_host(const double *gamma, int S, int G);
int k_stats(dsm_ctx *c, uint32_t iter);
int k_stats_stage1(dsm_ctx *c, uint32_t iter);
int k_stats_stage2(dsm_ctx *c, uint32_t iter);
int k_binom_test(dsm_ctx *c, int kind, uint32_t n, const double *w, uint64_t seed, int nsamp, uint32_t *d_out, int spec);
int k_esum_fold(dsm_ctx *c);
int k_dirichlet(dsm_ctx *c, uint32_t iter, double *gamma_out, double *gamma_trace, double *eta_out, double *eta_trace,
                double *prior_out, int fin_it, int fin_nblocks, const double *fin_prior, int do_s2 = 0);
int k_prior(dsm_ctx *c, const double *gamma, const double *eta, double *prior_out);
int k_prior_batch(dsm_ctx *c, const double *gamma, const double *eta, int n, double *prior_out);
struct TauFinalRider { int nblocks, it; const double *prior, *gamma_src, *eta_src; };
int k_tau_sweep(dsm_ctx *c, int mode, const double *gamma, const double *eta_sweep,
                const double *eta_ll, uint64_t *trace_slot, double *d_logp, uint32_t iter, int *nblocks,
                const uint32_t *u_raw, int slot = 0, const TauFinalRider *rider = nullptr);
int tau_launch_info(dsm_ctx *c, int *launched, int *resident);
int k_shard_pack(dsm_ctx *c, int nblocks);
int k_shard_unpack(dsm_ctx *c);
int k_finalize(dsm_ctx *c, int nblocks, int it, int star_mode, const double *prior, const double *gamma_src,
               const double *eta_src, int slot = 0, int *rare_out = nullptr);

int k_nmft_freq(dsm_ctx *c);
int k_nmft_clamp(dsm_ctx *c);
int k_nmft_pass_a(dsm_ctx *c);
int k_nmft_gamma(dsm_ctx *c, int max_iter, double min_change, int fix_gamma, int adjust, int parity);
int k_nmft_reduce(dsm_ctx *c);
bool nmft_gstep_applies(const dsm_ctx *c, int fix_gamma);
int k_nmft_pass_b(dsm_ctx *c, int adjust);
int k_nmft_get_tau(dsm_ctx *c, uint64_t *d_packed);
int nmft_grid(dsm_ctx *c);
bool nmft_use_wave(const dsm_ctx *c);
bool nmft_use_mfma(const dsm_ctx *c);
bool nmft_use_wide(const dsm_ctx *c);
int nmft_wide_grid(const dsm_ctx *c);
int nmft_mfma_grid(const dsm_ctx *c, bool fix = false);
int k_nmft_wave(dsm_ctx *c, int adjust, int do_update);
int k_nmft_persist(dsm_ctx *c, int max_iter, double min_change, int fix_gamma, int adjust, int *used);
int nmft_debug_path(const dsm_ctx *c, int fix_gamma, int out[8]);
```

### desman_amd/csrc/dsm_stage2.h

```cpp
#pragma once
#include "dsm_binom.h"
#include "log_table.h"

#define S2_MAX_NODES 32
#define S2_MAX_LEVELS 6
#define S2_TAB_ENTRIES 1024
struct S2Plan {
    int nlevels, tab_entries;
    int level_start[S2_MAX_LEVELS + 2];
    signed char lo[S2_MAX_NODES], hi[S2_MAX_NODES], child[S2_MAX_NODES];
    unsigned char idx[S2_MAX_NODES];
    short off[S2_MAX_NODES];
};

struct Stage2Params {
    uint32_t *ntab;
    int rep, ld;
    const double *gamma;
    unsigned long long *sum_mu;
    const double *log_tab;
    int S, G;
    uint32_t k0, k1, iter;
    uint32_t hmul, swz;
    uint32_t *big_count;
    int nsplit;
    uint32_t *scratch, *ticket;
};

S2Plan make_stage2_plan(int G);

#define S2_SMEM_BYTES (DSM_LOG_TAB_N * 16 + DSM_EXP_TAB_N * 8 + DSM_RCP_TAB_N * 8 + 32 * 8 + S2_TAB_ENTRIES * 4 + 32 * 4 + 5 * S2_MAX_NODES * 4)

#ifdef DSM_AB_SWITCHES
__device__ unsigned long long s2_clk[1024 * 8];
#define S2_CLK(row, k) do { if (threadIdx.x == 0 && blockIdx.y == 0 && (row) < 1024) s2_clk[(size_t)(row) * 8 + (k)] = __builtin_amdgcn_s_memrealtime(); } while (0)
#else
#define S2_CLK(row, k) do { } while (0)
#endif
template <int SPEC>
__device__ __forceinline__ const uint32_t *stage2_sample(const Stage2Params &p, const S2Plan &pl, int s, char *smem, bool to_global, int part = 0)
{
    const int G = p.G, tid = threadIdx.x, nthr = blockDim.x;
    double2 *ltab = reinterpret_cast<double2 *>(smem);
    double *etab = reinterpret_cast<double *>(ltab + DSM_LOG_TAB_N);
    double *rcp = etab + DSM_EXP_TAB_N;
    double *gs = rcp + DSM_RCP_TAB_N;
    uint32_t *tab = reinterpret_cast<uint32_t *>(gs + 32);
    uint32_t *leaf = tab + S2_TAB_ENTRIES;
    int *n_lo = reinterpret_cast<int *>(leaf + 32);
    int *n_hi = n_lo + S2_MAX_NODES, *n_off = n_hi + S2_MAX_NODES, *n_idx = n_off + S2_MAX_NODES, *n_child = n_idx + S2_MAX_NODES;

    const int nsplit = p.nsplit > 1 ? p.nsplit : 1;
    S2_CLK(s, 0);
    uint32_t pre_n = 0;
    bool pre_ok = false;
    {
        const int total0 = 1 << G, share0 = nsplit > 1 ? (total0 + nsplit - 1) / nsplit : total0;
        const int j0 = (nsplit > 1 ? part * share0 : 0) + tid, jh0 = nsplit > 1 ? min(total0, part * share0 + share0) : total0;
        if (p.rep == 1 && j0 < jh0 && j0 != 0) {
            pre_n = p.ntab[(size_t)(((uint32_t)j0 * p.hmul + ((uint32_t)s >> 4) * p.swz) & ((1u << G) - 1u)) * (size_t)p.ld + s];
            pre_ok = true;
        }
    }
    if (s == 0 && part == 0 && tid < DSM_BIG_NT * DSM_BIG_NL && p.big_count) p.big_count[tid * DSM_BIG_STRIDE] = 0u;
    if (tid < DSM_LOG_TAB_N) ltab[tid] = reinterpret_cast<const double2 *>(p.log_tab)[tid];
    if (tid < DSM_EXP_TAB_N) etab[tid] = p.log_tab[2 * DSM_LOG_TAB_N + tid];
    for (int k = tid; k < DSM_RCP_TAB_N; k += nthr) rcp[k] = k ? 1.0 / (double)k : 0.0;
    if (tid < 32) {
        gs[tid] = (tid < G) ? p.gamma[(size_t)s * G + tid] : 0.0; leaf[tid] = 0u;
        n_lo[tid] = pl.lo[tid]; n_hi[tid] = pl.hi[tid]; n_off[tid] = pl.off[tid]; n_idx[tid] = pl.idx[tid];
        n_child[tid] = pl.child[tid];
    }
    for (int i = tid; i < S2_TAB_ENTRIES; i += nthr) tab[i] = 0u;
    __syncthreads();
    S2_CLK(s, 1);

    const int nlev = pl.nlevels > 1 ? pl.nlevels - 1 : pl.nlevels;
    for (int level = 0; level < nlev; ++level) {
        const int n0 = pl.level_start[level], n1 = pl.level_start[level + 1];
        const int base = pl.off[n0];
        const int total = (level == 0) ? (1 << G) : (pl.off[n1 - 1] + (1 << (pl.hi[n1 - 1] - pl.lo[n1 - 1]))) - base;
        const int share = (level == 0 && nsplit > 1) ? (total + nsplit - 1) / nsplit : total;
        const int j_lo = (level == 0 && nsplit > 1) ? part * share : 0, j_hi = (level == 0 && nsplit > 1) ? min(total, j_lo + share) : total;
        for (int j = j_lo + tid; j < j_hi; j += nthr) {
            int i = n0;
            for (int k = n0 + 1; k < n1; ++k) if (j + base >= pl.off[k]) i = k;
            const int lo = n_lo[i], hi = n_hi[i], w = hi - lo;
            const uint32_t Hs = (uint32_t)(j + base - n_off[i]);
            if (Hs == 0) continue;
            uint32_t n;
            if (level == 0) {
                uint32_t *cell = p.ntab + (size_t)((Hs * p.hmul + ((uint32_t)s >> 4) * p.swz) & ((1u << G) - 1u)) * (size_t)p.ld + s;
                const size_t cstride = ((size_t)1 << G) * (size_t)p.ld;
                if (p.rep == 8) {
                    uint32_t m[8];
#pragma unroll
                    for (int r = 0; r < 8; ++r) m[r] = __builtin_nontemporal_load(cell + r * cstride);
                    n = 0;
#pragma unroll
                    for (int r = 0; r < 8; ++r) { n += m[r]; if (m[r]) cell[r * cstride] = 0u; }
                } else {
                    n = (pre_ok && j == j_lo + tid) ? pre_n : *cell;
                    if (n) *cell = 0u;
                    for (int r = 1; r < p.rep; ++r) {
                        const uint32_t m = cell[r * cstride];
                        if (m) { cell[r * cstride] = 0u; n += m; }
                    }
                }
            } else n = tab[base + j];
            if (w == 1) {
                if (level == 0) leaf[lo] = n;
                continue;
            }
            if (!n) continue;
            const int wl = w / 2, wh = w - wl, mid = lo + wl;
            const int ch = n_child[i];
            uint32_t *L = tab + n_off[ch], *R = tab + n_off[ch + 1];
            const uint32_t HL = Hs & ((1u << wl) - 1u), HR = Hs >> wl;
            if (wl == 1) L = leaf + lo - 1;
            if (wh == 1) R = leaf + mid - 1;
            if (!HR) { atomicAdd(&L[HL], n); continue; }
            if (!HL) { atomicAdd(&R[HR], n); continue; }
            double wL = 0.0, wR = 0.0;
            for (int jj = 0; jj < wl; ++jj) if ((HL >> jj) & 1u) wL = wL + gs[lo + jj];
            for (int jj = 0; jj < wh; ++jj) if ((HR >> jj) & 1u) wR = wR + gs[mid + jj];
            Xo128 rng = xo_seed(Hs, (uint32_t)s | ((uint32_t)n_idx[i] << 16) | ((uint32_t)level << 24), p.iter, DSM_STREAM_STA2,
                                p.k0, p.k1);
            bool dummy = false;
            const uint32_t k = binom<true, SPEC>(rng, n, wL, wR, rcp, ltab, dummy, DSM_BINV_MEAN_CAP_S2);
            if (k) atomicAdd(&L[HL], k);
            if (n - k) atomicAdd(&R[HR], n - k);
        }
        __syncthreads();
        if (level < 4) S2_CLK(s, 2 + level);
        if (level == 0 && nsplit > 1) {
            const int l1 = pl.level_start[1], l2 = pl.level_start[2];
            const int b1 = pl.off[l1], n1 = (pl.off[l2 - 1] + (1 << (pl.hi[l2 - 1] - pl.lo[l2 - 1]))) - b1;
            uint32_t *row = p.scratch + (size_t)s * S2_TAB_ENTRIES;
            uint32_t sink = 0;
            for (int i = tid; i < n1; i += nthr) { const uint32_t v = tab[b1 + i]; if (v) sink += atomicAdd(&row[i], v); }
            asm volatile("" :: "v"(sink));
            __syncthreads();
            __shared__ int last_wg;
            if (tid == 0) last_wg = (atomicAdd(&p.ticket[s], 1u) == (uint32_t)(nsplit - 1)) ? 1 : 0;
            __syncthreads();
            if (!last_wg) return leaf;
            for (int i = tid; i < n1; i += nthr) tab[b1 + i] = atomicExch(&row[i], 0u);
            if (tid == 0) p.ticket[s] = 0u;
            __syncthreads();
        }
    }
    if (to_global && tid < G && leaf[tid]) p.sum_mu[(size_t)s * G + tid] += leaf[tid];
    return leaf;
}
```

### desman_amd/csrc/kernels_gibbs.hip

```cpp
#include <string.h>

#include <mutex>

#include "dsm_device.h"
#include "dsm_host.h"
#include "dsm_stage2.h"
#include "log_table.h"

__global__ __launch_bounds__(256) void convert_counts_kernel(const int64_t *__restrict__ in,
                                                             int32_t *__restrict__ cnt_vs, int V, int S,
                                                             int *flag, double *partial,
                                                             unsigned long long *__restrict__ depth)
{
    __shared__ double red[256];
    __shared__ unsigned long long dep[DSM_MAX_S];
    for (int i = threadIdx.x; i < S; i += 256) dep[i] = 0ull;
    __syncthreads();
    const size_t n = (size_t)V * S;
    double acc = 0.0;
    for (size_t i = (size_t)blockIdx.x * 256 + threadIdx.x; i < n; i += (size_t)gridDim.x * 256) {
        int4 c;
        int64_t x[4];
        int64_t tot = 0;
        bool bad = false;
// ... 460 lines not shown
            p.sweep_stats[0] += (unsigned long long)red[0];
            p.sweep_stats[1] += (unsigned long long)redp[0];
            if (any_plain) { if (p.screen_ctl[0] > 0) p.screen_ctl[0] -= 1; }
            else if (5.0 * redp[0] > 4.0 * red[0]) p.screen_ctl[0] = 15;
        }
        if (p.blk_order) {
            __syncthreads();
            int *cnt = reinterpret_cast<int *>(red);
            const int per = (p.nblocks + nthr - 1) / nthr, lo = tid * per, hi = min(p.nblocks, lo + per);
            auto cold = [&](int i) { const uint32_t b = p.step_cnt[2 * i + 1]; return b != 0u && b != 0xFFFFFFFFu; };
            int nc = 0;
            for (int i = lo; i < hi; ++i) nc += cold(i) ? 1 : 0;
            int incl = nc;
            for (int o = 1; o < 64; o <<= 1) { const int y = __shfl_up(incl, o, 64); if ((tid & 63) >= o) incl += y; }
            if ((tid & 63) == 63) cnt[tid >> 6] = incl;
            __syncthreads();
            int before = incl - nc, total = 0;
            for (int k = 0; k < nthr / 64; ++k) { const int x = cnt[k]; if (k < (tid >> 6)) before += x; total += x; }
            int pc = before, pw = total + (lo - before);
            for (int i = lo; i < hi; ++i) { if (cold(i)) p.blk_order[pc++] = (uint32_t)i; else p.blk_order[pw++] = (uint32_t)i; }
        }
    }
}

__global__ __launch_bounds__(256) void finalize_kernel(FinalParams p)
{
    __shared__ double red[256], redp[256];
    __shared__ int flag;
    finalize_body(p, red, redp, &flag, threadIdx.x, 256);
    if (p.rare_out) {
        __syncthreads();
        if (threadIdx.x == 0) flag = 0;
        __syncthreads();
        for (int g = threadIdx.x; g < p.G; g += 256) {
            double m = 0.0;
            for (int s = 0; s < p.S; ++s) m = fmax(m, p.gamma_src[(size_t)s * p.G + g]);
            if ((float)m <= (float)DSM_NT_RARE) atomicAdd(&flag, 1);
        }
        __syncthreads();
        if (threadIdx.x == 0) *p.rare_out = flag;
    }
}

__device__ double gamma_variate(double shape, uint32_t idx, uint32_t iter, uint32_t k0, uint32_t k1)
{
    const double a = (shape < 1.0) ? shape + 1.0 : shape;
    const double d = a - 1.0 / 3.0;
    const double c = 1.0 / sqrt(9.0 * d);
    double res = 0.0, uboost = 1.0;
    for (uint32_t attempt = 0; attempt < 4096u; ++attempt) {
        uint32_t r0[4], r1[4];
        philox4x32_10(idx, 2u * attempt, iter, DSM_STREAM_DIRI, k0, k1, r0);
        philox4x32_10(idx, 2u * attempt + 1u, iter, DSM_STREAM_DIRI, k0, k1, r1);
        const double u1 = u01_open(r0[0], r0[1]), u2 = u01_open(r0[2], r0[3]);
        const double u3 = u01_open(r1[0], r1[1]);
        uboost = u01_open(r1[2], r1[3]);
        const double x = sqrt(-2.0 * log(u1)) * cos(6.283185307179586 * u2);
        double vv = 1.0 + c * x;
        if (vv <= 0.0) continue;
        vv = vv * vv * vv;
        const double x2 = x * x;
        if (u3 < 1.0 - 0.0331 * x2 * x2 || log(u3) < 0.5 * x2 + d * (1.0 - vv + log(vv))) {
            res = d * vv;
            break;
        }
    }
    if (shape < 1.0) res *= pow(uboost, 1.0 / shape);
    return res;
}

struct DirParams {
    unsigned long long *sum_mu, *esum;
    int S, G;
    double alpha, delta, epsilon, lgc_gamma, lgc_eta;
    uint32_t k0, k1, iter;
    int zero_after;
    double *gamma_out, *gamma_trace, *eta_out, *eta_trace, *rowprior;
    int do_fin;
    FinalParams fin;
    int do_s2;
    Stage2Params s2;
};

__device__ __forceinline__ void dirichlet_body(const DirParams &q, const S2Plan &plan)
{
    unsigned long long *__restrict__ sum_mu = q.sum_mu, *__restrict__ esum = q.esum;
    const int S = q.S, G = q.G;
    const double alpha = q.alpha, delta = q.delta, epsilon = q.epsilon, lgc_gamma = q.lgc_gamma, lgc_eta = q.lgc_eta;
    const uint32_t k0 = q.k0, k1 = q.k1, iter = q.iter;
    const int zero_after = q.zero_after;
    double *__restrict__ gamma_out = q.gamma_out, *__restrict__ gamma_trace = q.gamma_trace;
    double *__restrict__ eta_out = q.eta_out, *__restrict__ eta_trace = q.eta_trace, *__restrict__ rowprior = q.rowprior;
    const int do_fin = q.do_fin, do_s2 = q.do_s2;
    const FinalParams &fin = q.fin;
    const Stage2Params &s2 = q.s2;
    __shared__ __attribute__((aligned(16))) char smem_d[S2_SMEM_BYTES];
    if (do_fin && (int)blockIdx.x == S + 4) {
        double *red = reinterpret_cast<double *>(smem_d), *redp = red + 256;
        int *flag = reinterpret_cast<int *>(redp + 256);
        finalize_body(fin, red, redp, flag, threadIdx.x, 256);
        return;
    }
    const int row = blockIdx.x;
    const bool is_gamma = row < S;
    const uint32_t *leaf = nullptr;
    if (do_s2 && is_gamma)
        leaf = do_s2 >= 3 ? stage2_sample<3>(s2, plan, row, smem_d, false) : stage2_sample<2>(s2, plan, row, smem_d, false);
    if (!is_gamma) {
        static_assert(DSM_ESUM_PARTS * 4 == 256, "one thread per (copy, observed base)");
        unsigned long long *ef = reinterpret_cast<unsigned long long *>(smem_d);
        if (threadIdx.x < 4) ef[threadIdx.x] = 0ull;
        __syncthreads();
        const int ob = threadIdx.x & 3, k = threadIdx.x >> 2;
        unsigned long long *pp = esum + 16 + k * 16 + ob * 4 + (row - S);
        const unsigned long long v = *pp;
        if (v) { *pp = 0ull; atomicAdd(&ef[ob], v); }
        __syncthreads();
    }
    S2_CLK(row, 6);
    if (threadIdx.x >= 64) return;
    const int lane = threadIdx.x;
    const int n = is_gamma ? G : 4;
    const int SG = S * G;
    double y = 0.0;
    if (lane < n) {
        double shape;
        uint32_t vid;
        if (is_gamma) { vid = (uint32_t)(row * G + lane); shape = alpha + (double)(sum_mu[vid] + (leaf ? (unsigned long long)leaf[lane] : 0ull)); }
        else { const int a = row - S; vid = (uint32_t)(SG + a * 4 + lane); shape = delta + (double)(esum[lane * 4 + a] + reinterpret_cast<const unsigned long long *>(smem_d)[lane]); }
        y = gamma_variate(shape, vid, iter, k0, k1);
        if (zero_after) { if (is_gamma) sum_mu[row * G + lane] = 0ull; else esum[lane * 4 + (row - S)] = 0ull; }
    }
    double x = y / group_allreduce_sum<64>(y);
    if (is_gamma) {
        if (lane < n && x < epsilon) x = epsilon;
        x = x / group_allreduce_sum<64>(lane < n ? x : 0.0);
    }
    const double a1 = is_gamma ? alpha : delta;
    const double lsum = group_allreduce_sum<64>(lane < n ? (a1 - 1.0) * log(x) : 0.0);
    if (lane == 0) rowprior[row] = (is_gamma ? lgc_gamma : lgc_eta) + lsum;
    if (lane < n) {
        if (is_gamma) { gamma_out[row * G + lane] = x; if (gamma_trace) gamma_trace[row * G + lane] = x; }
        else { eta_out[(row - S) * 4 + lane] = x; if (eta_trace) eta_trace[(row - S) * 4 + lane] = x; }
    }
    S2_CLK(row, 7);
}
#ifdef DSM_AB_SWITCHES
extern "C" int dsm_debug_s2_clocks(unsigned long long *out, int nrows)
{
    if (nrows > 1024) nrows = 1024;
    if (hipMemcpyFromSymbol(out, HIP_SYMBOL(s2_clk), (size_t)nrows * 8 * sizeof(unsigned long long)) != hipSuccess) return -1;
    return 8;
}
#endif

struct DirBatch { DirParams p[DSM_MAX_BATCH]; S2Plan plan; };
__global__ __launch_bounds__(256) void dirichlet_kernel(DirParams q, S2Plan plan) { dirichlet_body(q, plan); }
__global__ __launch_bounds__(256) void dirichlet_kernel_b(DirBatch b) { dirichlet_body(b.p[blockIdx.y], b.plan); }
static_assert(sizeof(DirBatch) <= 4096, "kernarg segment");

__global__ __launch_bounds__(256) void prior_kernel(const double *__restrict__ gamma, const double *__restrict__ eta,
                                                    int S, int G, double alpha, double delta, double lgc_gamma,
                                                    double lgc_eta, double *__restrict__ rowprior)
{
    for (int r = blockIdx.x * 256 + threadIdx.x; r < S + 4; r += gridDim.x * 256) {
        double lsum = 0.0;
        if (r < S) { for (int g = 0; g < G; ++g) lsum += (alpha - 1.0) * log(gamma[(size_t)r * G + g]); rowprior[r] = lgc_gamma + lsum; }
        else { for (int b = 0; b < 4; ++b) lsum += (delta - 1.0) * log(eta[(r - S) * 4 + b]); rowprior[r] = lgc_eta + lsum; }
    }
}

struct TauParams {
    const int32_t *cnt_vs;
    uint64_t *tau;
    uint64_t *trace;
    const double *gamma, *eta_sweep, *eta_ll;
    const uint32_t *u_raw;
    double *logp;
    double *ll_partial;
    const double *log_tab;
    int *nchange;
    uint32_t *step_cnt;
    const uint32_t *screen_ctl;
    int screen;
    int nt_skip;
    int V, S, G;
    int v_off;
    uint32_t k0, k1, iter;
    const uint32_t *order;
    int do_fin;
    FinalParams fin;
};

#ifdef TAU_NO_LEAN
#define TAU_LEAN(LPV, NSL) false
#else
#ifdef TAU_LEAN2
#define TAU_LEAN(LPV, NSL) ((LPV) >= 32 && ((NSL) == 2 || (NSL) == 3 || (NSL) == 6 || (NSL) == 8))
#else
#define TAU_LEAN(LPV, NSL) ((LPV) >= 32 && ((NSL) == 3 || (NSL) == 6 || (NSL) == 8))
#endif
#endif

template <int LPV, int NSL, bool SWEEP, bool LL, bool NT = false>
__device__ __forceinline__ void tau_body(const TauParams &p)
{
    extern __shared__ __attribute__((aligned(16))) char smem_t[];
    const int nblk = (int)gridDim.x - p.do_fin;
    if (p.do_fin && (int)blockIdx.x == nblk) {
        double *fr = reinterpret_cast<double *>(smem_t);
        finalize_body(p.fin, fr, fr + 256, reinterpret_cast<int *>(fr + 512), threadIdx.x, 256);
        return;
    }
    constexpr bool LEAN = TAU_LEAN(LPV, NSL) && SWEEP;
    const int bid = p.order ? (int)p.order[blockIdx.x] : (int)blockIdx.x;
    constexpr int SP = LPV * NSL;
    constexpr int GPB = 256 / LPV;
    double *gT = reinterpret_cast<double *>(smem_t);
    double *eS = gT + (size_t)p.G * SP;
    double *eL = eS + 16;
    double *red = eL + 16;
    int *redi = reinterpret_cast<int *>(red + 4);
    double2 *ltab = reinterpret_cast<double2 *>(red + 6);
    float *gT32 = reinterpret_cast<float *>(ltab + DSM_LOG_TAB_N);
    float *eS32 = gT32 + (size_t)p.G * SP;
    uint32_t *gmaxb = reinterpret_cast<uint32_t *>(eS32 + 24);
    const int tid = threadIdx.x, G = p.G, S = p.S;
    if (tid < DSM_LOG_TAB_N) ltab[tid] = reinterpret_cast<const double2 *>(p.log_tab)[tid];
    if constexpr (NT) {
        if (tid < 32) gmaxb[tid] = 0u;
        __syncthreads();
    }
    for (int i = tid; i < G * SP; i += 256) {
        const int g = i / SP, s = i % SP;
        const double x = (s < S) ? p.gamma[(size_t)s * G + g] : 1.0;
        gT[i] = x;
        if (SWEEP) gT32[i] = (float)x;
        if constexpr (NT) { if (s < S && g < 32) atomicMax(&gmaxb[g], __float_as_uint((float)x)); }
    }
    if (tid < 16) { eS[tid] = p.eta_sweep[tid]; eL[tid] = p.eta_ll[tid]; if (SWEEP) eS32[tid] = (float)p.eta_sweep[tid]; }
    if (SWEEP && tid < 4) {
// ... 372 lines not shown
    if (c->blk_gmax != key) {
        int occ = 0;
        HIP_TRY(hipOccupancyMaxActiveBlocksPerMultiprocessor(&occ, fn, 256, 0));
        hipDeviceProp_t prop;
        HIP_TRY(hipGetDeviceProperties(&prop, c->device));
        if (occ < 1) occ = 1;
        const int S = c->S, budget = std::max(S, occ * prop.multiProcessorCount);
        double tot = 0.0;
        for (int s = 0; s < S; ++s) tot += (double)c->depth[s];
        std::vector<int32_t> nb(S, 1);
        int used = S;
        if (tot > 0)
            for (int s = 0; s < S; ++s) {
                int extra = (int)((double)(budget - S) * (double)c->depth[s] / tot);
                const int most = (c->nitems_h[s] + 255) / 256;
                if (1 + extra > most) extra = std::max(0, most - 1);
                nb[s] += extra; used += extra;
            }
        std::vector<int32_t> tab;
        tab.reserve((size_t)used * 3);
        int maxnb = 0;
        for (int s = 0; s < S; ++s) maxnb = std::max(maxnb, nb[s]);
        for (int j = 0; j < maxnb; ++j)
            for (int s = 0; s < S; ++s)
                if (j < nb[s]) { tab.push_back(s); tab.push_back(j); tab.push_back(nb[s]); }
        if (c->blk_tab) { (void)hipFree(c->blk_tab); c->blk_tab = nullptr; }
        HIP_TRY(hipMalloc((void **)&c->blk_tab, tab.size() * sizeof(int32_t)));
        HIP_TRY(hipMemcpyAsync(c->blk_tab, tab.data(), tab.size() * sizeof(int32_t), hipMemcpyHostToDevice, c->stream));
        HIP_TRY(hipStreamSynchronize(c->stream));
        c->blk_n = used;
        c->blk_gmax = key;
    }
    const dim3 grid(c->blk_n), block(256);
    const uint32_t k0 = (uint32_t)c->ctr_seed, k1 = (uint32_t)(c->ctr_seed >> 32);
#define LAUNCH_STATS(GM, EX)                                                                                          \
    hipLaunchKernelGGL((stats_kernel<GM, EX>), grid, block, 0, c->stream, reinterpret_cast<const int2 *>(c->items),   \
                       c->nitems, c->blk_tab, c->tau, c->gamma, c->eta,                                               \
                       c->V, c->S, c->G, c->item_stride, c->chunked ? 1 : 0, k0, k1, iter, c->sum_mu, c->esum)
#define STATS_CASE(GM) if (gm == GM) { if (exact) LAUNCH_STATS(GM, true); else LAUNCH_STATS(GM, (GM <= 8)); }
    STATS_CASE(1); STATS_CASE(2); STATS_CASE(3); STATS_CASE(4); STATS_CASE(5); STATS_CASE(6); STATS_CASE(7);
    STATS_CASE(8); STATS_CASE(10); STATS_CASE(12); STATS_CASE(14); STATS_CASE(16); STATS_CASE(20); STATS_CASE(24);
    STATS_CASE(28); STATS_CASE(32);
#undef STATS_CASE
#undef LAUNCH_STATS
    HIP_TRY(hipGetLastError());
    return DSM_OK;
}

static void dirichlet_consts(const dsm_ctx *c, double *lgc_gamma, double *lgc_eta)
{
    *lgc_gamma = lgamma(c->alpha * c->G) - c->G * lgamma(c->alpha);
    *lgc_eta = lgamma(c->delta * 4) - 4 * lgamma(c->delta);
}

static FinalParams make_final(dsm_ctx *c, int nblocks, int it, int star_mode, const double *prior, const double *gamma_src,
                              const double *eta_src, int slot = 0)
{
    FinalParams p;
    p.ll_partial = c->ll_partial + (size_t)slot * DSM_MAX_GRID; p.nblocks = nblocks;
    p.ll_const = c->ll_const;
    p.tau_prior = (double)(c->shard_on ? c->shard_vtot : c->V) * (double)c->G * log(1.0 / 4.0);
    p.ll_given = c->shard_on ? c->shard_vec : nullptr;
    p.prior = prior; p.S = c->S; p.nchange = c->nchange + slot; p.it = it;
    p.ll_trace = c->ll_trace; p.lp_trace = c->lp_trace; p.nchange_trace = c->nchange_trace;
    p.star = c->star; p.gamma_src = gamma_src; p.gamma_star = c->gamma_star; p.SG = c->S * c->G;
    p.eta_src = eta_src; p.eta_star = c->eta_star;
    p.star_mode = star_mode; p.scalars = c->scalars;
    p.step_cnt = c->step_cnt + (size_t)slot * 2 * DSM_MAX_GRID; p.sweep_stats = c->sweep_stats; p.screen_ctl = c->screen_ctl + slot;
    static const bool order_on = !(getenv("DESMAN_HIP_TAU_ORDER") && atoi(getenv("DESMAN_HIP_TAU_ORDER")) == 0);
    p.blk_order = nullptr;
    p.rare_out = nullptr; p.G = c->G;
    if (order_on && c->blk_order && nblocks > 0 && nblocks <= DSM_MAX_GRID) {
        if (c->tau_resident_key != c->S * 64 + c->G) {
            int launched = 0, resident = 0;
            if (tau_launch_info(c, &launched, &resident) == DSM_OK) { c->tau_resident = resident; c->tau_resident_key = c->S * 64 + c->G; }
        }
        if (c->tau_resident > 0 && nblocks > c->tau_resident) { p.blk_order = c->blk_order + (size_t)slot * DSM_MAX_GRID; c->blk_order_n[slot] = nblocks; }
        else c->blk_order_n[slot] = 0;
    }
    return p;
}

int k_dirichlet(dsm_ctx *c, uint32_t iter, double *gamma_out, double *gamma_trace, double *eta_out, double *eta_trace,
                double *prior_out, int fin_it, int fin_nblocks, const double *fin_prior, int do_s2)
{
    KTimer tm(c, DSM_K_DIRICH);
    double lg, le;
    dirichlet_consts(c, &lg, &le);
    const uint32_t k0 = (uint32_t)c->ctr_seed, k1 = (uint32_t)(c->ctr_seed >> 32);
    const int do_fin = fin_it >= 0 ? 1 : 0;
    FinalParams fin = {};
    if (do_fin)
        fin = make_final(c, fin_nblocks, fin_it, 0, fin_prior, c->gamma_trace + (size_t)fin_it * c->S * c->G,
                         c->eta_trace + (size_t)fin_it * 16);
    Stage2Params s2 = {};
    if (do_s2) {
        s2.ntab = c->ntab; s2.rep = c->ntab_rep; s2.ld = c->ntab_ld; s2.gamma = c->gamma; s2.sum_mu = c->sum_mu; s2.log_tab = c->log_tab;
        s2.S = c->S; s2.G = c->G; s2.k0 = k0; s2.k1 = k1; s2.iter = iter; s2.hmul = DSM_NTAB_HMUL; s2.swz = DSM_NTAB_SWZ;
        s2.big_count = c->big_count;
    }
    DirParams q;
    q.sum_mu = c->sum_mu; q.esum = c->esum; q.S = c->S; q.G = c->G;
    q.alpha = c->alpha; q.delta = c->delta; q.epsilon = c->epsilon; q.lgc_gamma = lg; q.lgc_eta = le;
    q.k0 = k0; q.k1 = k1; q.iter = iter; q.zero_after = 1;
    q.gamma_out = gamma_out; q.gamma_trace = gamma_trace; q.eta_out = eta_out; q.eta_trace = eta_trace; q.rowprior = prior_out;
    q.do_fin = do_fin; q.fin = fin; q.do_s2 = do_s2 ? stats_draw_version(stats_spec(c)) : 0; q.s2 = s2;
    if (g_batch.K == 0) {
        const S2Plan plan = do_s2 ? make_stage2_plan(c->G) : S2Plan{};
        hipLaunchKernelGGL(dirichlet_kernel, dim3(c->S + 4 + do_fin), dim3(256), 0, c->stream, q, plan);
    } else {
        static thread_local DirBatch acc;
        acc.p[g_batch.k] = q;
        if (g_batch.k == g_batch.K - 1) {
            acc.plan = do_s2 ? make_stage2_plan(c->G) : S2Plan{};
            hipLaunchKernelGGL(dirichlet_kernel_b, dim3(c->S + 4 + do_fin, g_batch.K), dim3(256), 0, c->stream, acc);
        }
    }
    HIP_TRY(hipGetLastError());
    return DSM_OK;
}

__global__ __launch_bounds__(256) void prior_batch_kernel(const double *__restrict__ gamma, const double *__restrict__ eta,
                                                          int n, int S, int G, double alpha, double delta,
                                                          double lgc_gamma, double lgc_eta, double *__restrict__ rowprior)
{
    const int rows = S + 4;
    for (size_t i = (size_t)blockIdx.x * 256 + threadIdx.x; i < (size_t)n * rows; i += (size_t)gridDim.x * 256) {
        const int it = (int)(i / rows), r = (int)(i % rows);
        double lsum = 0.0;
        if (r < S) {
            const double *g = gamma + ((size_t)it * S + r) * G;
            for (int k = 0; k < G; ++k) lsum += (alpha - 1.0) * log(g[k]);
            rowprior[i] = lgc_gamma + lsum;
        } else {
            const double *e = eta + (size_t)it * 16 + (r - S) * 4;
            for (int b = 0; b < 4; ++b) lsum += (delta - 1.0) * log(e[b]);
            rowprior[i] = lgc_eta + lsum;
        }
    }
}

int k_prior_batch(dsm_ctx *c, const double *gamma, const double *eta, int n, double *prior_out)
{
    double lg, le;
    dirichlet_consts(c, &lg, &le);
    const size_t tot = (size_t)n * (c->S + 4);
    const int grid = (int)std::min<size_t>((tot + 255) / 256, 1024);
    hipLaunchKernelGGL(prior_batch_kernel, dim3(grid), dim3(256), 0, c->stream, gamma, eta, n, c->S, c->G, c->alpha, c->delta,
                       lg, le, prior_out);
    HIP_TRY(hipGetLastError());
    return DSM_OK;
}

int k_prior(dsm_ctx *c, const double *gamma, const double *eta, double *prior_out)
{
    double lg, le;
    dirichlet_consts(c, &lg, &le);
    hipLaunchKernelGGL(prior_kernel, dim3(1), dim3(256), 0, c->stream, gamma, eta, c->S, c->G, c->alpha, c->delta, lg,
                       le, prior_out);
    HIP_TRY(hipGetLastError());
    return DSM_OK;
}

__global__ __launch_bounds__(256) void gamma_rare_kernel(const double *__restrict__ gamma, int S, int G, int *__restrict__ out)
{
    __shared__ int cnt;
    if (threadIdx.x == 0) cnt = 0;
    __syncthreads();
    for (int g = threadIdx.x; g < G; g += 256) {
        double m = 0.0;
        for (int s = 0; s < S; ++s) m = fmax(m, gamma[(size_t)s * G + g]);
        if ((float)m <= (float)DSM_NT_RARE) atomicAdd(&cnt, 1);
    }
    __syncthreads();
    if (threadIdx.x == 0) *out = cnt;
}
int k_tau_neartie_hint(dsm_ctx *c)
{
    c->tau_neartie_on = false;
    if (c->tau_neartie_mode == 0 || g_batch.K || c->shard_on || !c->tau_screen || c->G < 2) return DSM_OK;
    c->tau_neartie_on = c->tau_neartie_mode == 1 || (c->tau_rare_n > 0 && c->tau_rare_n < c->G);
    return DSM_OK;
}
int tau_rare_from_host(const double *gamma, int S, int G)
{
    int n = 0;
    for (int g = 0; g < G; ++g) {
        double m = 0.0;
        for (int s = 0; s < S; ++s) m = std::max(m, gamma[(size_t)s * G + g]);
        n += (float)m <= (float)DSM_NT_RARE;
    }
    return n;
// ... 164 lines not shown
```

### desman_amd/csrc/kernels_stats.hip

```cpp
#include "dsm_binom.h"
#include "dsm_host.h"
#include "log_table.h"

#include <string.h>

#include <algorithm>
#include <vector>

#ifdef DSM_AB_SWITCHES
#define STATS_DBG(p, mask) ((p).dbg & (mask))
#else
#define STATS_DBG(p, mask) 0
#endif
#ifdef DSM_AB_SWITCHES
#define S1_NCLK 16
__device__ unsigned long long s1_clk[8192 * S1_NCLK];
#define S1_CLK(k) do { if ((threadIdx.x & 63) == 0 && blockIdx.y == 0) s1_clk[(size_t)(blockIdx.x * 4 + (threadIdx.x >> 6)) * S1_NCLK + (k)] = __builtin_amdgcn_s_memrealtime(); } while (0)
extern "C" int dsm_debug_s1_clocks(unsigned long long *out, int nwaves)
{
    if (nwaves > 8192) nwaves = 8192;
    if (hipMemcpyFromSymbol(out, HIP_SYMBOL(s1_clk), (size_t)nwaves * S1_NCLK * sizeof(unsigned long long)) != hipSuccess) return -1;
    return S1_NCLK;
}
#else
#define S1_CLK(k) do { } while (0)
#endif
#define S1_CLKP(j) do { if (s1_pass < 3) S1_CLK(2 + 4 * s1_pass + (j)); } while (0)
struct StatsAggParams {
    const int32_t *cnt_vs;
    const uint64_t *tau;
    const double *gamma, *eta;
    int V, S, G;
    int v_off, V_tot;
    uint32_t k0, k1, iter;
    uint32_t *ntab;
    int rep, ld;
    unsigned long long *esum;
    const double *log_tab;
    unsigned long long *big_list;
    uint32_t *big_count;
    size_t big_seg;
    double lean_cap;
    uint32_t swz;
    uint32_t hmul;
    int xcd;
    const unsigned long long *pat_rep;
    uint32_t *pat_x;
    const uint32_t *pat_list, *pat_n;
    int dbg;
};

__device__ __forceinline__ uint64_t wave_uniform_u64(uint64_t x)
{
    const uint32_t lo = __builtin_amdgcn_readfirstlane((uint32_t)x), hi = __builtin_amdgcn_readfirstlane((uint32_t)(x >> 32));
    return ((uint64_t)hi << 32) | lo;
}

template <int LPV, int SPEC, bool PAT = false>
__device__ __forceinline__ void stats_agg_body(const StatsAggParams &p)
{
    extern __shared__ __attribute__((aligned(16))) char smem_s[];
    S1_CLK(0);
#ifdef DSM_AB_SWITCHES
    if ((threadIdx.x & 63) == 0 && blockIdx.y == 0)
        s1_clk[(size_t)(blockIdx.x * 4 + (threadIdx.x >> 6)) * S1_NCLK + 13] =
            ((unsigned long long)(__builtin_amdgcn_s_getreg((31 << 11) | 4)) << 8) | (__builtin_amdgcn_s_getreg((3 << 11) | 20) & 15u) | (1ull << 63);
#endif
    constexpr int NG = 64 / LPV;
    constexpr int NTAB = SPEC >= 3 ? (2 * DSM_LOG_TAB_N + DSM_EXP_TAB_N) : 0;
    const int S = p.S, G = p.G, V = p.V;
    const int NCH = (S + LPV - 1) / LPV, SP = NCH * LPV;
    double *tabs = reinterpret_cast<double *>(smem_s);
    double *gT = tabs + NTAB;
    double *rcp = gT + (size_t)G * SP;
    double *es = rcp + DSM_RCP_TAB_N;
    uint32_t *eacc = reinterpret_cast<uint32_t *>(es + 16);
    const double2 *ltab = reinterpret_cast<const double2 *>(tabs);
    const int tid = threadIdx.x, lane = tid & 63;
    const int grp = lane / LPV, lig = lane % LPV;
    const int nwaves = gridDim.x * 4;
    const int wid = __builtin_amdgcn_readfirstlane(blockIdx.x * 4 + (tid >> 6));
    const int nunit = PAT ? (int)__builtin_amdgcn_readfirstlane((int)*p.pat_n) : V;
    const int ntask = nunit * NCH;
    const int nslot = (ntask + NG - 1) / NG;
// ... 211 lines not shown
    const int chunk = (int)blockIdx.x / nvsplit, part = (int)blockIdx.x % nvsplit;
    const int s = chunk * LPW + (lane % LPW);
    const uint64_t mask = (1ull << (2 * G)) - 1ull;
    for (int v0 = (part * 16 + wv) * PPW; v0 < V; v0 += nvsplit * 16 * PPW) {
        const int v = v0 + lane / LPW;
        if (v < V && s < S) {
            const int4 c = reinterpret_cast<const int4 *>(cnt_vs)[(size_t)v * S + s];
            uint32_t *row = ptab + (size_t)(tau[v] & mask) * 4 * LPW + (lane % LPW);
            if (c.x) atomicAdd(row, (uint32_t)c.x);
            if (c.y) atomicAdd(row + LPW, (uint32_t)c.y);
            if (c.z) atomicAdd(row + 2 * LPW, (uint32_t)c.z);
            if (c.w) atomicAdd(row + 3 * LPW, (uint32_t)c.w);
        }
    }
    __syncthreads();
    for (int i = tid; i < words * 4 * LPW; i += 1024) {
        const uint32_t n = ptab[i];
        if (!n) continue;
        const int w = i / (4 * LPW), b = (i / LPW) & 3, sl = chunk * LPW + i % LPW;
        atomicAdd(x + ((size_t)(uint32_t)rep[w] * 4 + b) * S + sl, n);
    }
}

__global__ __launch_bounds__(256) void pat_list_kernel(const unsigned long long *__restrict__ rep, int words, uint32_t hi, uint32_t *__restrict__ list,
                                                       uint32_t *__restrict__ n_this, uint32_t *__restrict__ n_next)
{
    const int w = blockIdx.x * 256 + threadIdx.x;
    if (w == 0) *n_next = 0u;
    if (w >= words) return;
    const unsigned long long e = rep[w];
    if ((uint32_t)(e >> 32) == hi) list[atomicAdd(n_this, 1u)] = (uint32_t)e;
}

__global__ __launch_bounds__(256) void pat_agg_kernel(const int32_t *__restrict__ cnt_vs, const uint64_t *__restrict__ tau, int V, int S, int G,
                                                      const unsigned long long *__restrict__ rep, uint32_t *__restrict__ x)
{
    const size_t n = (size_t)V * S;
    for (size_t i = (size_t)blockIdx.x * 256 + threadIdx.x; i < n; i += (size_t)gridDim.x * 256) {
        const int v = (int)(i / (size_t)S), s = (int)(i - (size_t)v * S);
        const int4 c = reinterpret_cast<const int4 *>(cnt_vs)[i];
        const uint32_t r = (uint32_t)rep[tau[v] & ((1ull << (2 * G)) - 1ull)];
        uint32_t *xr = x + (size_t)r * 4 * S + s;
        if (c.x) atomicAdd(xr, (uint32_t)c.x);
        if (c.y) atomicAdd(xr + S, (uint32_t)c.y);
        if (c.z) atomicAdd(xr + 2 * (size_t)S, (uint32_t)c.z);
        if (c.w) atomicAdd(xr + 3 * (size_t)S, (uint32_t)c.w);
    }
}
template <int LPV, int SPEC>
__global__ __launch_bounds__(256, 6) void stats_agg_kernel_b(BatchArgs<StatsAggParams> b) { stats_agg_body<LPV, SPEC>(b.p[blockIdx.y]); }
template <int LPV>
__global__ __launch_bounds__(256, 5) void stats_pat_kernel_b(BatchArgs<StatsAggParams> b) { stats_agg_body<LPV, 2, true>(b.p[blockIdx.y]); }

template <int SPEC>
__device__ __forceinline__ void stats_big_body(const StatsAggParams &p)
{
    __shared__ double2 ltab[DSM_LOG_TAB_N + DSM_EXP_TAB_N / 2];
    __shared__ double rcp[DSM_RCP_TAB_N];
    __shared__ double es[16];
    __shared__ unsigned long long acc[16];
    __shared__ uint32_t eacc[16 * 256];
    const int tid = threadIdx.x, lane = tid & 63;
    const uint32_t sub = blockIdx.x % (DSM_BIG_NT * DSM_BIG_NL), bi = blockIdx.x / (DSM_BIG_NT * DSM_BIG_NL), nb = gridDim.x / (DSM_BIG_NT * DSM_BIG_NL);
    const uint32_t nbig = p.big_count[sub * DSM_BIG_STRIDE];
    if (bi * 256u >= nbig) return;
    const unsigned long long *list = p.big_list + (size_t)sub * p.big_seg;
    ltab[tid] = reinterpret_cast<const double2 *>(p.log_tab)[tid];
    if (tid < DSM_EXP_TAB_N / 2) ltab[DSM_LOG_TAB_N + tid] = reinterpret_cast<const double2 *>(p.log_tab)[DSM_LOG_TAB_N + tid];
    for (int k = tid; k < DSM_RCP_TAB_N; k += blockDim.x) rcp[k] = k ? 1.0 / (double)k : 0.0;
    if (tid < 16) { es[tid] = p.eta[tid]; acc[tid] = 0ull; }
#pragma unroll
    for (int i = 0; i < 16; ++i) eacc[i * 256 + tid] = 0u;
    __syncthreads();
    const int S = p.S, G = p.G;
    for (uint32_t i = bi * 256u + tid; i < nbig; i += nb * 256u) {
        const unsigned long long item = list[i];
        const uint32_t cell = (uint32_t)(item >> 2);
        const int b = (int)(item & 3ull);
        const int s = (int)(cell / (uint32_t)p.V_tot), v = (int)(cell - (uint32_t)s * (uint32_t)p.V_tot) - p.v_off;
        const uint64_t t = p.tau[v];
        uint32_t xb;
        if (p.pat_x) { uint32_t *xw = p.pat_x + ((size_t)v * 4 + b) * S + s; xb = *xw; *xw = 0u; }
        else xb = (uint32_t)p.cnt_vs[((size_t)v * S + s) * 4 + b];
        uint32_t H[4] = {0, 0, 0, 0};
        double Gam[4] = {0.0, 0.0, 0.0, 0.0};
        for (int g = 0; g < G; ++g) {
            const int a = (int)((t >> (2 * g)) & 3);
            const double x = p.gamma[(size_t)s * G + g];
#pragma unroll
            for (int k = 0; k < 4; ++k) if (a == k) { H[k] |= 1u << g; Gam[k] = Gam[k] + x; }
        }
        double W[4];
#pragma unroll
        for (int a = 0; a < 4; ++a) W[a] = es[a * 4 + b] * Gam[a];
        const double Wt = ((W[0] + W[1]) + W[2]) + W[3];
        if (!(Wt > 0.0)) {
#pragma unroll
            for (int a = 0; a < 4; ++a) W[a] = Gam[a];
        }
        uint32_t n[4], cbase[4];
        philox4x32_10(cell, 0u, p.iter, DSM_STREAM_STA1, p.k0, p.k1, cbase);
        Xo128 rng = item_seed<SPEC>(cbase, (uint32_t)b, p.k0, p.k1);
        bool defer = false;
        mult4<true, SPEC>(rng, xb, W, n, rcp, ltab, defer);
        uint32_t *erow = eacc + (b * 4) * 256 + tid;
#pragma unroll
        for (int a = 0; a < 4; ++a) {
            erow[a * 256] += n[a];
            if (n[a]) atomicAdd(p.ntab + (size_t)(blockIdx.x % (unsigned)p.rep) * (((size_t)1 << G) * (size_t)p.ld) + (size_t)((H[a] * p.hmul + ((uint32_t)s >> 4) * p.swz) & ((1u << G) - 1u)) * (size_t)p.ld + s, n[a]);
        }
    }
    {
        uint32_t e[16];
#pragma unroll
        for (int i = 0; i < 16; ++i) e[i] = eacc[i * 256 + tid];
        const uint32_t tot = wave_transpose_reduce<16>(e);
        const int idx = transpose_index<16>(lane);
        if (lane < 16 && tot) atomicAdd(&acc[idx], (unsigned long long)tot);
    }
    __syncthreads();
    if (tid < 16 && acc[tid]) atomicAdd(&p.esum[tid], acc[tid]);
}

__global__ __launch_bounds__(256) void esum_fold_kernel(unsigned long long *__restrict__ esum)
{
    static_assert(DSM_ESUM_PARTS * 4 == 256, "one thread per (copy, group of four counters)");
    const int k = threadIdx.x >> 2, q = threadIdx.x & 3;
    unsigned long long *pp = esum + 16 + k * 16 + q * 4;
#pragma unroll
    for (int i = 0; i < 4; ++i) {
        const unsigned long long v = pp[i];
        if (v) { pp[i] = 0ull; atomicAdd(&esum[q * 4 + i], v); }
    }
}
int k_esum_fold(dsm_ctx *c)
{
    hipLaunchKernelGGL(esum_fold_kernel, dim3(1), dim3(256), 0, c->stream, c->esum);
    HIP_TRY(hipGetLastError());
    return DSM_OK;
}

template <int SPEC>
__global__ __launch_bounds__(256) void stats_big_kernel(StatsAggParams p) { stats_big_body<SPEC>(p); }
template <int SPEC>
__global__ __launch_bounds__(256) void stats_big_kernel_b(BatchArgs<StatsAggParams> b) { stats_big_body<SPEC>(b.p[blockIdx.y]); }

#include "dsm_stage2.h"

struct Stage2Batch { Stage2Params p[DSM_MAX_BATCH]; S2Plan plan; };
template <int SPEC>
__global__ __launch_bounds__(1024) void stats_stage2_kernel(Stage2Params p, S2Plan plan)
{
    __shared__ __attribute__((aligned(16))) char smem2[S2_SMEM_BYTES];
    stage2_sample<SPEC>(p, plan, (int)blockIdx.x / p.nsplit, smem2, true, (int)blockIdx.x % p.nsplit);
}
template <int SPEC>
__global__ __launch_bounds__(1024) void stats_stage2_kernel_b(Stage2Batch b)
{
    __shared__ __attribute__((aligned(16))) char smem2[S2_SMEM_BYTES];
    stage2_sample<SPEC>(b.p[blockIdx.y], b.plan, blockIdx.x, smem2, true);
}

template <int SPEC>
__global__ __launch_bounds__(256) void binom_test_kernel(int kind, uint32_t n, double wa, double wb, double w2, double w3,
                                                         uint32_t k0, uint32_t k1, int nsamp, const double *log_tab,
                                                         uint32_t *out)
{
    __shared__ double2 ltab[DSM_LOG_TAB_N + DSM_EXP_TAB_N / 2];
    __shared__ double rcp[DSM_RCP_TAB_N];
    const int tid = threadIdx.x;
    ltab[tid] = reinterpret_cast<const double2 *>(log_tab)[tid];
    if (tid < DSM_EXP_TAB_N / 2) ltab[DSM_LOG_TAB_N + tid] = reinterpret_cast<const double2 *>(log_tab)[DSM_LOG_TAB_N + tid];
    for (int k = tid; k < DSM_RCP_TAB_N; k += blockDim.x) rcp[k] = k ? 1.0 / (double)k : 0.0;
    __syncthreads();
    const int i = blockIdx.x * 256 + tid;
    if (i >= nsamp) return;
    Xo128 rng = xo_seed((uint32_t)i, 0u, 0u, DSM_STREAM_TEST, k0, k1);
    bool dummy = false;
    if (kind != 2) out[i] = binom<true, SPEC>(rng, n, wa, wb, rcp, ltab, dummy, kind == 0 ? DSM_BINV_MEAN_CAP : DSM_BINV_MEAN_CAP_S2);
    else {
        const double W[4] = {wa, wb, w2, w3};
        uint32_t m[4];
        mult4<true, SPEC>(rng, n, W, m, rcp, ltab, dummy);
        out[i * 4 + 0] = m[0]; out[i * 4 + 1] = m[1]; out[i * 4 + 2] = m[2]; out[i * 4 + 3] = m[3];
    }
}

static int stats_agg_lpv(int S)
{
    int best = 64;
    for (int l : {32, 16}) if ((S + l - 1) / l * l < (S + best - 1) / best * best) best = l;
    return best;
}

int stats_spec(const dsm_ctx *c)
{
    int force = c->force_stats_spec;
    if (force == 0) {
        const char *e = getenv("DESMAN_HIP_STATS_SPEC");
        if (e && (e[0] == '1' || e[0] == '2' || e[0] == '3' || e[0] == '4') && e[1] == 0) force = e[0] - '0';
    }
    if (force == 1) return 1;
    if (c->G < 1 || c->G > 16) return 1;
    if (((size_t)1 << c->G) * (size_t)c->S * 4 > ((size_t)64 << 20)) return 1;
    if (c->max_depth >= ((uint64_t)1 << 32)) return 1;
    const bool pat_ok = c->G <= 8 && !c->shard_on;
    if (force == 4) return pat_ok ? 4 : 2;
    if (force >= 2) return force;
    double reads = 0.0;
    for (int64_t d : c->depth) reads += (double)d;
    const int lpv = stats_agg_lpv(c->S);
    const double cells = (double)c->V * (double)((c->S + lpv - 1) / lpv * lpv);
    const double g = (double)c->G;
    const double t1 = 25.0 + (0.25 + 0.02 * g + 0.0029 * g * g) * 1e-6 * reads;
    const double stage2 = 14.0 + (c->G >= 10 ? 0.012 * (double)(1u << c->G) : 0.0);
    const int rep = stats_ntab_rep(c);
    const double per = 3.0 * (double)c->V / (double)(1u << c->G);
    const double t2 = 24.0 + stage2 + 0.062e-3 * cells + (rep == 1 ? 0.03 * per : 0.003 * per / rep);
    if (pat_ok && force == 0 && t2 < t1) {
        const bool small_g = (c->G <= 2 && cells >= 0.5e6) || (c->G == 3 && cells >= 1.0e6);
        const bool mid_g = c->G >= 4 && cells >= 2.5e6 && 64.0 * (double)((size_t)1 << c->G) <= (double)c->V;
        if (small_g || mid_g) return 4;
    }
    return t2 < t1 ? DSM_STATS_AGG : 1;
}

int stats_ntab_rep(const dsm_ctx *c)
{
    const double per = 3.0 * (double)(c->shard_on ? c->shard_vtot : c->V) / (double)((size_t)1 << c->G);
    if (per <= 128.0) return 1;
    const double lines = (double)((((size_t)1 << c->G) * (size_t)c->S * 4 + 63) / 64);
    int rep = 2;
    while (lines * rep < 384.0 && rep < 64 && (size_t)(2 * rep) * ((size_t)1 << c->G) * (size_t)c->S * 4 <= ((size_t)64 << 20)) rep *= 2;
    return rep;
}

void stats_release_ntab(dsm_ctx *c)
{
    if (c->ntab_raw) (void)hipFree(c->ntab_raw);
    c->ntab_raw = nullptr; c->ntab = nullptr; c->ntab_len = 0;
}
static int ensure_ntab(dsm_ctx *c)
{
    const int rep = stats_ntab_rep(c), ld = c->S;
    const size_t need = (size_t)rep * ((size_t)1 << c->G) * (size_t)ld;
    if (c->ntab && c->ntab_len == need && c->ntab_ld == ld && c->ntab_rep == rep) return DSM_OK;
    stats_release_ntab(c);
    c->ntab_rep = rep; c->ntab_ld = ld;
    const char *eo = DSM_AB_ENV("DESMAN_HIP_NTAB_OFF");
    const size_t off = eo ? ((size_t)strtoull(eo, nullptr, 0) & ~(size_t)255) : 0;
    const size_t spare = off + 4096;
    hipError_t e = hipMalloc((void **)&c->ntab_raw, need * sizeof(uint32_t) + spare);
    if (e != hipSuccess) { dsm_set_error("hipMalloc(%zu B) failed: %s", need * 4 + spare, hipGetErrorString(e)); return DSM_ERR_NOMEM; }
    c->ntab = reinterpret_cast<uint32_t *>(((uintptr_t)c->ntab_raw + 4095) & ~(uintptr_t)4095) + off / 4;
    c->ntab_len = need;
    HIP_TRY(hipMemsetAsync(c->ntab, 0, need * sizeof(uint32_t), c->stream));
    return DSM_OK;
}

int stats_ensure_ntab(dsm_ctx *c)
{
    return stats_spec(c) < 2 ? DSM_OK : ensure_ntab(c);
}

static int ensure_big_list(dsm_ctx *c, size_t seg)
{
    const size_t need = seg * DSM_BIG_NT * DSM_BIG_NL;
    if (c->big_list && c->big_cap == need) return DSM_OK;
    if (c->big_list) { (void)hipFree(c->big_list); c->big_list = nullptr; }
    if (!c->big_count) {
        hipError_t e = hipMalloc((void **)&c->big_count, DSM_BIG_NT * DSM_BIG_NL * DSM_BIG_STRIDE * sizeof(uint32_t));
        if (e != hipSuccess) { dsm_set_error("hipMalloc failed: %s", hipGetErrorString(e)); return DSM_ERR_NOMEM; }
    }
    hipError_t e = hipMalloc((void **)&c->big_list, need * sizeof(unsigned long long));
    if (e != hipSuccess) { dsm_set_error("hipMalloc(%zu B) failed: %s", need * 8, hipGetErrorString(e)); return DSM_ERR_NOMEM; }
    c->big_cap = need;
    HIP_TRY(hipMemsetAsync(c->big_count, 0, DSM_BIG_NT * DSM_BIG_NL * DSM_BIG_STRIDE * sizeof(uint32_t), c->stream));
    return DSM_OK;
}

static int ensure_pat(dsm_ctx *c)
{
    const size_t nrep = (size_t)1 << (2 * c->G), nx = (size_t)c->V * 4 * (size_t)c->S;
    if (!c->pat_rep || c->pat_rep_len != nrep) {
        if (c->pat_rep) { (void)hipFree(c->pat_rep); c->pat_rep = nullptr; }
        hipError_t e = hipMalloc((void **)&c->pat_rep, nrep * sizeof(unsigned long long));
        if (e != hipSuccess) { dsm_set_error("hipMalloc(%zu B) failed: %s", nrep * 8, hipGetErrorString(e)); return DSM_ERR_NOMEM; }
        c->pat_rep_len = nrep;
        c->pat_gen = 0;
        HIP_TRY(hipMemsetAsync(c->pat_rep, 0xFF, nrep * sizeof(unsigned long long), c->stream));
    }
    if (!c->pat_list || c->pat_rep_len != nrep || c->pat_gen == 0) {
        if (c->pat_list) { (void)hipFree(c->pat_list); c->pat_list = nullptr; }
        hipError_t e = hipMalloc((void **)&c->pat_list, (nrep + 2) * sizeof(uint32_t));
        if (e != hipSuccess) { dsm_set_error("hipMalloc(%zu B) failed: %s", (nrep + 2) * 4, hipGetErrorString(e)); return DSM_ERR_NOMEM; }
        HIP_TRY(hipMemsetAsync(c->pat_list + nrep, 0, 2 * sizeof(uint32_t), c->stream));
    }
    if (!c->pat_x || c->pat_x_len != nx) {
        if (c->pat_x) { (void)hipFree(c->pat_x); c->pat_x = nullptr; }
        hipError_t e = hipMalloc((void **)&c->pat_x, nx * sizeof(uint32_t));
        if (e != hipSuccess) { dsm_set_error("hipMalloc(%zu B) failed: %s", nx * 4, hipGetErrorString(e)); return DSM_ERR_NOMEM; }
        c->pat_x_len = nx;
        HIP_TRY(hipMemsetAsync(c->pat_x, 0, nx * sizeof(uint32_t), c->stream));
    }
    return DSM_OK;
}

int k_stats_stage1(dsm_ctx *c, uint32_t iter)
{
    int r = ensure_ntab(c);
    if (r != DSM_OK) return r;
    const int S = c->S, G = c->G, V = c->V;
    const int LPV = stats_agg_lpv(S);
    const int NCH = (S + LPV - 1) / LPV, SP = NCH * LPV, NG = 64 / LPV;
    const int spec_full = stats_spec(c);
    const bool pat = spec_full == 4;
    const int spec = stats_draw_version(spec_full);
    const size_t sh = ((size_t)G * SP + (spec >= 3 ? 2 * DSM_LOG_TAB_N + DSM_EXP_TAB_N : 0) + DSM_RCP_TAB_N + 16) * sizeof(double) +
                      16 * 256 * sizeof(uint32_t);
    if (sh > 160 * 1024) { dsm_set_error("stats_agg: gamma tile (%zu B) exceeds LDS", sh); return DSM_ERR_UNSUPPORTED; }
    const void *fn = nullptr, *fn_b = nullptr;
#define AGG_CASE(L, SP_) if (LPV == L && spec == SP_) { fn = (const void *)stats_agg_kernel<L, SP_>; fn_b = (const void *)stats_agg_kernel_b<L, SP_>; }
    AGG_CASE(16, 2) AGG_CASE(32, 2) AGG_CASE(64, 2) AGG_CASE(16, 3) AGG_CASE(32, 3) AGG_CASE(64, 3)
#undef AGG_CASE
    if (pat) {
        fn = LPV == 16 ? (const void *)stats_pat_kernel<16> : LPV == 32 ? (const void *)stats_pat_kernel<32> : (const void *)stats_pat_kernel<64>;
        fn_b = LPV == 16 ? (const void *)stats_pat_kernel_b<16> : LPV == 32 ? (const void *)stats_pat_kernel_b<32> : (const void *)stats_pat_kernel_b<64>;
    }
    if (!fn) { dsm_set_error("stats_agg: no kernel for spec %d", spec); return DSM_ERR_UNSUPPORTED; }
    if (c->stats_grid == 0 || c->stats_grid_key != spec_full) {
        int occ = 0;
        HIP_TRY(hipOccupancyMaxActiveBlocksPerMultiprocessor(&occ, fn, 256, sh));
        hipDeviceProp_t prop;
        HIP_TRY(hipGetDeviceProperties(&prop, c->device));
        const int wgs = std::min(6, std::max(1, occ));
        const int n_xcd = prop.multiProcessorCount % 8 == 0 && prop.multiProcessorCount >= 64 ? 8 : 1;
        const long passes4 = (((long)V * NCH + NG - 1) / NG) / std::max(1L, (long)wgs * prop.multiProcessorCount);
        const int leave = (c->tau_rng == DSM_RNG_MT19937 && passes4 <= 12) ? n_xcd : 0;
        c->stats_grid = wgs * std::max(1, prop.multiProcessorCount - leave);
        c->stats_grid_key = spec_full;
    }
    const long ntask = ((long)V * NCH + NG - 1) / NG;
    const long max_waves = (long)c->stats_grid * 4 / (g_batch.K ? g_batch.K : 1);
    const long waves = std::min<long>(ntask, max_waves);
    const int grid = (int)std::max<long>(1, (waves + 3) / 4);
    const long per_wg = ((ntask + waves - 1) / waves) * 4 * 64 * 4;
    const size_t seg = (size_t)std::min<long>((long)V * S * 4, ((grid + DSM_BIG_NL - 1) / DSM_BIG_NL) * per_wg);
    r = ensure_big_list(c, seg);
    if (r != DSM_OK) return r;
    StatsAggParams p;
    p.cnt_vs = c->cnt_vs; p.tau = c->tau; p.gamma = c->gamma; p.eta = c->eta;
    p.V = V; p.S = S; p.G = G; p.big_seg = seg;
    p.v_off = c->shard_on ? c->shard_voff : 0; p.V_tot = c->shard_on ? c->shard_vtot : V;
    p.k0 = (uint32_t)c->ctr_seed; p.k1 = (uint32_t)(c->ctr_seed >> 32); p.iter = iter;
    p.ntab = c->ntab; p.rep = c->ntab_rep; p.ld = c->ntab_ld; p.esum = c->esum; p.log_tab = c->log_tab;
    p.xcd = 0;
    p.hmul = DSM_NTAB_HMUL; p.swz = DSM_NTAB_SWZ;
    p.big_list = c->big_list; p.big_count = c->big_count;
    p.pat_rep = nullptr; p.pat_x = nullptr; p.pat_list = nullptr; p.pat_n = nullptr;
    if (pat) {
        r = ensure_pat(c);
        if (r != DSM_OK) return r;
        p.pat_rep = c->pat_rep; p.pat_x = c->pat_x;
        KTimer tm(c, DSM_K_STATSPAT);
        const uint32_t hi = 0xFFFFFFFFu - (++c->pat_gen);
        const int words = 1 << (2 * G);
        uint32_t *n_this = c->pat_list + words + (c->pat_gen & 1u), *n_next = c->pat_list + words + ((c->pat_gen + 1u) & 1u);
        p.pat_list = c->pat_list; p.pat_n = n_this;
        if (G <= 6) hipLaunchKernelGGL(pat_rep_lds_kernel, dim3(std::max(1, std::min(64, V / 4096))), dim3(1024), 0, c->stream, c->tau, V, G, c->pat_rep, hi);
        else hipLaunchKernelGGL(pat_rep_kernel, dim3((V + 255) / 256), dim3(256), 0, c->stream, c->tau, V, G, c->pat_rep, hi);
        hipLaunchKernelGGL(pat_list_kernel, dim3((words + 255) / 256), dim3(256), 0, c->stream, c->pat_rep, words, hi, c->pat_list, n_this, n_next);
        const size_t ncell = (size_t)V * S;
        const int lpw = G <= 3 ? 64 : 32;
        const size_t lds = ((size_t)1 << (2 * G)) * 4 * lpw * sizeof(uint32_t);
        if (G <= 4 && lds <= 128 * 1024 && V >= 4096) {
            const int nchunk = (S + lpw - 1) / lpw;
            const int nvsplit = std::max(1, std::min(256 / nchunk, V / (16 * (64 / lpw) * 8)));
            const void *fl = lpw == 64 ? (const void *)pat_agg_lds_kernel<64> : (const void *)pat_agg_lds_kernel<32>;
            static bool attr_done[2] = {false, false};
            if (!attr_done[lpw == 32]) { HIP_TRY(hipFuncSetAttribute(fl, hipFuncAttributeMaxDynamicSharedMemorySize, 128 * 1024)); attr_done[lpw == 32] = true; }
            const int32_t *cv = c->cnt_vs; const uint64_t *tp = c->tau; const unsigned long long *rp = c->pat_rep; uint32_t *xp = c->pat_x;
            int Vv = V, Ss = S, Gg = G, nvs = nvsplit;
            void *args[] = {(void *)&cv, (void *)&tp, (void *)&Vv, (void *)&Ss, (void *)&Gg, (void *)&rp, (void *)&xp, (void *)&nvs};
            HIP_TRY(hipLaunchKernel(fl, dim3(nchunk * nvsplit), dim3(1024), args, lds, c->stream));
        } else
            hipLaunchKernelGGL(pat_agg_kernel, dim3((unsigned)std::min<size_t>((ncell + 255) / 256, 16384)), dim3(256), 0, c->stream,
                               c->cnt_vs, c->tau, V, S, G, c->pat_rep, c->pat_x);
        HIP_TRY(hipGetLastError());
    }
    {
        static const char *e = DSM_AB_ENV("DESMAN_HIP_LEAN_CAP");
        p.lean_cap = e ? atof(e) : DSM_LEAN_CAP;
        static const int dbg = DSM_AB_ENV("DESMAN_HIP_STATS_DBG") ? atoi(DSM_AB_ENV("DESMAN_HIP_STATS_DBG")) : 0;
        p.dbg = dbg;
        if (!(p.lean_cap > 0.0 && p.lean_cap <= DSM_BINV_MEAN_CAP)) p.lean_cap = DSM_LEAN_CAP;
    }
    const int big_wgs = 16;
    const int big_grid = DSM_BIG_NT * DSM_BIG_NL *
        (int)std::max<long>(1, std::min<long>((ntask * 64 * 4 / DSM_BIG_NL + 255) / 256, g_batch.K ? std::max(2, big_wgs / g_batch.K) : big_wgs));
    if (g_batch.K) {
        static thread_local BatchArgs<StatsAggParams> acc;
        acc.p[g_batch.k] = p;
        if (g_batch.k == g_batch.K - 1) {
            const dim3 g(grid, g_batch.K);
            void *args[] = {(void *)&acc};
            HIP_TRY(hipLaunchKernel(fn_b, g, dim3(256), args, sh, c->stream));
            if (spec >= 3) hipLaunchKernelGGL(stats_big_kernel_b<3>, dim3(big_grid, g_batch.K), dim3(256), 0, c->stream, acc);
            else hipLaunchKernelGGL(stats_big_kernel_b<2>, dim3(big_grid, g_batch.K), dim3(256), 0, c->stream, acc);
        }
        HIP_TRY(hipGetLastError());
        return DSM_OK;
    }
    {
        KTimer tm(c, DSM_K_STATS);
        void *args[] = {(void *)&p};
        HIP_TRY(hipLaunchKernel(fn, dim3(grid), dim3(256), args, sh, c->stream));
    }
    KTimer tm(c, DSM_K_STATSBIG);
    if (spec >= 3) hipLaunchKernelGGL(stats_big_kernel<3>, dim3(big_grid), dim3(256), 0, c->stream, p);
    else hipLaunchKernelGGL(stats_big_kernel<2>, dim3(big_grid), dim3(256), 0, c->stream, p);
    HIP_TRY(hipGetLastError());
    return DSM_OK;
}

S2Plan make_stage2_plan(int G)
{
    S2Plan pl;
    memset(&pl, 0, sizeof pl);
    int n = 0, off = 0;
    pl.lo[0] = 0; pl.hi[0] = G; pl.off[0] = 0; pl.idx[0] = 0; pl.child[0] = -1;
    n = 1;
    int lvl_begin = 0, lvl_end = 1, level = 0;
    pl.level_start[0] = 0;
    while (lvl_begin < lvl_end) {
        for (int i = lvl_begin; i < lvl_end; ++i) {
            const int w = pl.hi[i] - pl.lo[i];
            if (w == 1) { pl.child[i] = -1; continue; }
            const int wl = w / 2, mid = pl.lo[i] + wl;
            pl.child[i] = n;
            pl.lo[n] = pl.lo[i]; pl.hi[n] = mid; pl.off[n] = off; pl.idx[n] = 2 * pl.idx[i]; off += 1 << wl; ++n;
            pl.lo[n] = mid; pl.hi[n] = pl.hi[i]; pl.off[n] = off; pl.idx[n] = 2 * pl.idx[i] + 1; off += 1 << (w - wl); ++n;
        }
        lvl_begin = lvl_end; lvl_end = n;
        pl.level_start[++level] = lvl_begin;
    }
    pl.nlevels = level;
    pl.tab_entries = off;
    return pl;
}

int k_stats_stage2(dsm_ctx *c, uint32_t iter)
{
    KTimer tm(c, DSM_K_STATS2);
    Stage2Params p;
    p.ntab = c->ntab; p.rep = c->ntab_rep; p.ld = c->ntab_ld; p.gamma = c->gamma; p.sum_mu = c->sum_mu; p.log_tab = c->log_tab;
    p.S = c->S; p.G = c->G; p.hmul = DSM_NTAB_HMUL; p.swz = DSM_NTAB_SWZ;
    p.k0 = (uint32_t)c->ctr_seed; p.k1 = (uint32_t)(c->ctr_seed >> 32); p.iter = iter;
    p.big_count = c->big_count;
    const int nthr = c->G >= 10 ? 1024 : 256;
    const bool v3 = stats_draw_version(stats_spec(c)) >= 3;
    p.nsplit = 1; p.scratch = nullptr; p.ticket = nullptr;
    if (g_batch.K == 0 && c->G >= 11) {
        if (!c->s2_scratch) {
            hipError_t e = hipMalloc((void **)&c->s2_scratch, ((size_t)DSM_MAX_S * (S2_TAB_ENTRIES + 1)) * sizeof(uint32_t));
            if (e != hipSuccess) { dsm_set_error("hipMalloc failed: %s", hipGetErrorString(e)); return DSM_ERR_NOMEM; }
            HIP_TRY(hipMemsetAsync(c->s2_scratch, 0, ((size_t)DSM_MAX_S * (S2_TAB_ENTRIES + 1)) * sizeof(uint32_t), c->stream));
        }
        p.nsplit = c->G >= 12 ? 4 : 2;
        p.scratch = c->s2_scratch; p.ticket = c->s2_scratch + (size_t)DSM_MAX_S * S2_TAB_ENTRIES;
    }
    if (g_batch.K == 0) {
        if (v3) hipLaunchKernelGGL(stats_stage2_kernel<3>, dim3(c->S * p.nsplit), dim3(nthr), 0, c->stream, p, make_stage2_plan(c->G));
        else hipLaunchKernelGGL(stats_stage2_kernel<2>, dim3(c->S * p.nsplit), dim3(nthr), 0, c->stream, p, make_stage2_plan(c->G));
    } else {
        static thread_local Stage2Batch acc;
        acc.p[g_batch.k] = p;
        if (g_batch.k == g_batch.K - 1) {
            acc.plan = make_stage2_plan(c->G);
            if (v3) hipLaunchKernelGGL(stats_stage2_kernel_b<3>, dim3(c->S, g_batch.K), dim3(nthr), 0, c->stream, acc);
            else hipLaunchKernelGGL(stats_stage2_kernel_b<2>, dim3(c->S, g_batch.K), dim3(nthr), 0, c->stream, acc);
        }
    }
    HIP_TRY(hipGetLastError());
    return DSM_OK;
}

int k_stats(dsm_ctx *c, uint32_t iter)
{
    if (stats_spec(c) >= 2) {
        int r = k_stats_stage1(c, iter);
        if (r != DSM_OK) return r;
        return k_stats_stage2(c, iter);
    }
    return k_stats_v1(c, iter);
}

int k_binom_test(dsm_ctx *c, int kind, uint32_t n, const double *w, uint64_t seed, int nsamp, uint32_t *d_out, int spec)
{
    if (spec >= 3) hipLaunchKernelGGL(binom_test_kernel<3>, dim3((nsamp + 255) / 256), dim3(256), 0, c->stream, kind, n, w[0], w[1], w[2], w[3],
                                      (uint32_t)seed, (uint32_t)(seed >> 32), nsamp, c->log_tab, d_out);
    else hipLaunchKernelGGL(binom_test_kernel<2>, dim3((nsamp + 255) / 256), dim3(256), 0, c->stream, kind, n, w[0], w[1], w[2], w[3],
                       (uint32_t)seed, (uint32_t)(seed >> 32), nsamp, c->log_tab, d_out);
    HIP_TRY(hipGetLastError());
    return DSM_OK;
}
```

### include/desman_hip.h

```cpp
#ifndef DESMAN_HIP_H
#define DESMAN_HIP_H

#include <stdint.h>

#ifdef __cplusplus
extern "C" {
#endif

#define DSM_OK               0
#define DSM_ERR_HIP         -1
#define DSM_ERR_ARG         -2
#define DSM_ERR_STATE       -3
#define DSM_ERR_UNSUPPORTED -4
#define DSM_ERR_NOMEM       -5
#define DSM_ERR_NODEVICE    -6
#define DSM_ERR_COMM        -7

#define DSM_MAX_G  32
#define DSM_MAX_S  512

#define DSM_RNG_MT19937 0
#define DSM_RNG_PHILOX  1

const char *dsm_last_error(void);
// ... 71 lines not shown
int dsm_nmft_objective(dsm_ctx *ctx, double *div);
int dsm_nmft_debug_path(dsm_ctx *ctx, int fix_gamma, int out[8]);
int dsm_nmft_get_tau(dsm_ctx *ctx, int64_t *tau_onehot);

int dsm_lrt_step(int device, const double *ffreq, const int32_t *maxA, const int32_t *maxB,
                 const double *eta, double upperP, int optimise, int V, double *p_inout,
                 double *MLL, double *BLL);

#define DSM_ASSIGN_MAX_G 10
int dsm_assign_tau(int device, const int64_t *counts , int N, int S, int G, const double *gamma, const double *eta,
                   uint64_t seed, uint8_t *map_state, double *conf, double *logz, double *marg, uint8_t *draw_state);
int dsm_ctx_assign_tau(dsm_ctx *ctx, const double *gamma, const double *eta, int G, uint64_t seed, uint8_t *map_state,
                       double *conf, double *logz, double *marg, uint8_t *draw_state);
int dsm_assign_debug_set_chunk(int positions);

int dsm_fit_gamma(int device, const int64_t *counts , int V, int S, int G, const int64_t *tau ,
                  const double *eta, int max_iter, double tol, int presence, double *gamma, double *loglik, double *deviance,
                  int32_t *iters, int32_t *converged, double *lr_absent);
int dsm_ctx_fit_gamma(dsm_ctx *ctx, int G, const int64_t *tau , const double *eta, int max_iter, double tol,
                      int presence, double *gamma, double *loglik, double *deviance, int32_t *iters, int32_t *converged,
                      double *lr_absent);
int dsm_abund_debug_set_chunk(int samples);

int dsm_fit_gamma_interval(int device, const int64_t *counts , int V, int S, int G, const int64_t *tau ,
                           const double *eta, const double *gamma_hat , double q, int max_iter, double tol, double ctol,
                           double *lo, double *hi, int32_t *flags);
int dsm_ctx_fit_gamma_interval(dsm_ctx *ctx, int G, const int64_t *tau , const double *eta,
                               const double *gamma_hat, double q, int max_iter, double tol, double ctol, double *lo, double *hi,
                               int32_t *flags);

typedef struct dsm_genes dsm_genes;
#define DSM_MAX_ETA 8

int dsm_genes_create(dsm_genes **out, int device);
int dsm_genes_destroy(dsm_genes *gs);
int dsm_genes_set_data(dsm_genes *gs, const int64_t *variants, int Vtot, int S, int C,
                       const int32_t *gene_off , const double *cov);
int dsm_genes_set_model(dsm_genes *gs, const double *gamma, const double *epsilon,
                        const double *delta, int G, int max_eta, const double *eta_log_prior,
                        const double *cov_const, const double *mult_const);
int dsm_genes_set_state(dsm_genes *gs, const int32_t *eta, const int64_t *tau);
int dsm_genes_get_state(dsm_genes *gs, int32_t *eta, int64_t *tau);
int dsm_genes_seed(dsm_genes *gs, unsigned long mt_seed, uint64_t ctr_seed);
int dsm_genes_set_gene_base(dsm_genes *gs, int gene_base);
int dsm_genes_get_mt_state(dsm_genes *gs, uint32_t *state625);
int dsm_genes_set_mt_state(dsm_genes *gs, const uint32_t *state625);

int dsm_genes_nmft_tau(dsm_genes *gs, const int32_t *eta_mask ,
                       const double *tau_init, int max_iter, double min_change, int32_t *n_iter);
int dsm_genes_sweep_all(dsm_genes *gs, const int32_t *eta_mask, int sweep, int32_t *nchange,
                        double *logvar, double *v_ll);
int dsm_genes_step_candidates(dsm_genes *gs, int c, int g, double *logvar, int *swept);
int dsm_genes_step_choose(dsm_genes *gs, int c, int g, int eta_value);
int dsm_genes_update(dsm_genes *gs, int n_iter, int reset_star, int32_t *eta_store,
                     double *gene_ll_trace, const uint32_t *u_tau_ext, const double *u_eta_ext);
int dsm_genes_loglik(dsm_genes *gs, double *gene_ll);
int dsm_genes_get_star(dsm_genes *gs, int32_t *eta_star, double *gene_llstar);
int dsm_genes_set_star(dsm_genes *gs, const int32_t *eta_star, const double *gene_llstar);
int dsm_genes_debug_tile(const dsm_genes *gs, int *lpv, int *nsl, int *groups_per_block, size_t *lds_bytes);

int dsm_kl_assign(int device, const double *cov, const double *delta, double *eta, int C, int S,
                  int G, int max_iter, double min_change, int *n_done, double *div);

#define DSM_K_STATS    0
#define DSM_K_DIRICH   1
#define DSM_K_TAU      2
#define DSM_K_FINAL    3
#define DSM_K_MT       4
#define DSM_K_NMFT_A   5
#define DSM_K_NMFT_G   6
#define DSM_K_NMFT_B   7
#define DSM_K_STATS2   8
#define DSM_K_STATSBIG 9
#define DSM_K_STATSPAT 10
#define DSM_K_COUNT    11
int dsm_ctx_sweep_stats(dsm_ctx *ctx, uint64_t *steps, uint64_t *exact_steps, int mode);
int dsm_ctx_debug_log2f(dsm_ctx *ctx, const float *in, float *out, size_t n);
int dsm_release_device_caches(void);
int dsm_debug_fdiv(int kind, const double *a, const double *b, double *out, int n);
int dsm_ctx_set_nmft_fused(dsm_ctx *ctx, int mode);
int dsm_ctx_set_nmft_persist(dsm_ctx *ctx, int mode);
int dsm_ctx_set_tau_screen(dsm_ctx *ctx, int on);
int dsm_ctx_set_tau_neartie(dsm_ctx *ctx, int mode);
int dsm_ctx_tau_launch_info(dsm_ctx *ctx, int *launched, int *resident);
int dsm_ctx_get_counters(dsm_ctx *ctx, uint64_t *ctr_seed, uint32_t *iter_ctr);
int dsm_ctx_set_counters(dsm_ctx *ctx, uint64_t ctr_seed, uint32_t iter_ctr);
int dsm_ctx_get_screen_state(dsm_ctx *ctx, uint32_t *out2);
int dsm_ctx_set_screen_state(dsm_ctx *ctx, const uint32_t *in2);
typedef int (*dsm_exchange_fn)(void *user, uint32_t *dev_tab, size_t n_tab, double *dev_vec, size_t n_vec);
int dsm_ctx_gibbs_update_sharded(dsm_ctx *ctx, int n_iter, int v_offset, int v_total, dsm_exchange_fn exchange, void *user);
typedef struct dsm_comm dsm_comm;
int dsm_comm_unique_id(void *id128);
int dsm_comm_create(dsm_comm **out, const void *id128, int rank, int world, int device);
int dsm_comm_destroy(dsm_comm *comm);
int dsm_comm_rank(const dsm_comm *comm);
int dsm_comm_world(const dsm_comm *comm);
int dsm_comm_allgather_f64(dsm_comm *comm, const double *send, double *recv, size_t n);
int dsm_comm_allreduce_f64(dsm_comm *comm, double *data, size_t n, int op);
int dsm_comm_barrier(dsm_comm *comm);
int dsm_ctx_gibbs_update_sharded_comm(dsm_ctx *ctx, int n_iter, int v_offset, int v_total, dsm_comm *comm);
int dsm_device_read(int device, const void *dev, void *host, size_t bytes);
int dsm_device_write(int device, void *dev, const void *host, size_t bytes);
int dsm_ctx_set_timing(dsm_ctx *ctx, int on);
int dsm_ctx_get_timing(dsm_ctx *ctx, double *ms_total ,
                       int64_t *launches );
const char *dsm_kernel_name(int k);

#ifdef __cplusplus
}
#endif
#endif
```

Baseline: 6.357 billion V*S updates/s.

## Skip the big-item stats launch and draw deferred items inside the Dirichlet kernel

Adds an adaptive mode that skips launching the separate stats_big kernel after stage 1. The deferred big items are instead walked and drawn inside the Dirichlet/stage-2 kernel, using double-buffered big_count lists and a new gamma_new buffer so the old gamma stays readable. A device flag records whether any big items appeared, and the host polls it every 64 iterations to decide whether to keep launching the big kernel. This removes one kernel launch per iteration when the lists are empty. In exchange it adds a periodic host synchronisation and some extra per-sample work in the Dirichlet blocks.

```diff
diff --git a/desman_amd/_lib.py b/desman_amd/_lib.py
--- a/desman_amd/_lib.py
+++ b/desman_amd/_lib.py
@@ -59,6 +59,9 @@
     "dsm_ctx_sweep_stats": (_i, [_vp, C.POINTER(C.c_uint64), C.POINTER(C.c_uint64), _i]),
     "dsm_ctx_set_tau_screen": (_i, [_vp, _i]),
     "dsm_ctx_set_tau_neartie": (_i, [_vp, _i]),
+    "dsm_ctx_set_big_launch": (_i, [_vp, _i]),
+    "dsm_ctx_get_big_launch": (_i, [_vp]),
+    "dsm_ctx_debug_big_lists": (_i, [_vp, C.c_uint32, _vp, _vp]),
     "dsm_ctx_set_nmft_fused": (_i, [_vp, _i]),
     "dsm_ctx_set_nmft_persist": (_i, [_vp, _i]),
     "dsm_ctx_tau_launch_info": (_i, [_vp, C.POINTER(_i), C.POINTER(_i)]),
@@ -484,6 +487,15 @@
     def set_tau_neartie(self, mode=-1):
         check(self.lib.dsm_ctx_set_tau_neartie(self._h, int(mode)))
 
+    def set_big_launch(self, mode=-1):
+        check(self.lib.dsm_ctx_set_big_launch(self._h, int(mode)))
+
+    def get_big_launch(self):
+        r = self.lib.dsm_ctx_get_big_launch(self._h)
+        if r < 0:
+            check(r)
+        return bool(r)
+
     def set_tau_screen(self, on):
         check(self.lib.dsm_ctx_set_tau_screen(self._h, 1 if on else 0))
 
@@ -517,6 +529,12 @@
         E = np.zeros((4, 4), dtype=np.uint64)
         check(self.lib.dsm_ctx_debug_stage1(self._h, int(it), nt.ctypes.data, E))
         return nt, E
+
+    def debug_big_lists(self, it):
+        kinds = np.zeros(3, dtype=np.uint32)
+        per_sample = np.zeros(self.S, dtype=np.uint32)
+        check(self.lib.dsm_ctx_debug_big_lists(self._h, int(it), kinds.ctypes.data, per_sample.ctypes.data))
+        return kinds, per_sample
 
     def debug_binom(self, kind, n, w, seed, nsamp, spec=STATS_AGG):
         w4 = np.zeros(4)
diff --git a/desman_amd/csrc/api.hip b/desman_amd/csrc/api.hip
--- a/desman_amd/csrc/api.hip
+++ b/desman_amd/csrc/api.hip
@@ -187,6 +187,8 @@
     TRY(dev_alloc(&c->eta, 16));
     TRY(dev_alloc(&c->eta_new, 16));
     TRY(dev_alloc(&c->eta_star, 16));
+    TRY(dev_alloc(&c->big_seen, 1));
+    HIP_TRY(hipMemsetAsync(c->big_seen, 0, sizeof(uint32_t), c->stream));
     TRY(dev_alloc(&c->esum, 16 + 16 * DSM_ESUM_PARTS));
     TRY(dev_alloc(&c->log_tab, 2 * DSM_LOG_TAB_N + DSM_EXP_TAB_N));
     HIP_TRY(hipMemcpyAsync(c->log_tab, dsm_log_table_host, sizeof dsm_log_table_host, hipMemcpyHostToDevice, c->stream));
@@ -218,6 +220,8 @@
     dev_free(&c->cnt_vs); dev_free(&c->items); dev_free(&c->nitems); dev_free(&c->tau);
     dev_free(&c->pat_rep); dev_free(&c->pat_x); dev_free(&c->pat_list); c->pat_rep_len = c->pat_x_len = 0;
     if (c->h_rare) { (void)hipHostFree(c->h_rare); c->h_rare = nullptr; }
+    if (c->h_big_seen) { (void)hipHostFree(c->h_big_seen); c->h_big_seen = nullptr; }
+    dev_free(&c->big_seen); dev_free(&c->gamma_new);
     dev_free(&c->s2_scratch);
     dev_free(&c->blk_tab); stats_release_ntab(c); dev_free(&c->big_list); dev_free(&c->big_count);
     dev_free(&c->gamma); dev_free(&c->eta);
@@ -368,6 +372,7 @@
         c->G = G;
         const size_t sg = (size_t)c->S * G;
         TRY(dev_alloc(&c->gamma, sg));
+        TRY(dev_alloc(&c->gamma_new, sg));
         TRY(dev_alloc(&c->gamma_star, sg));
         TRY(dev_alloc(&c->sum_mu, sg));
         HIP_TRY(hipMemsetAsync(c->sum_mu, 0, sg * sizeof(unsigned long long), c->stream));
@@ -395,7 +400,9 @@
     HIP_TRY(hipMemcpyAsync(c->gamma, gamma, (size_t)c->S * G * sizeof(double), hipMemcpyHostToDevice, c->stream));
     c->tau_rare_n = tau_rare_from_host(gamma, c->S, G);
     HIP_TRY(hipMemcpyAsync(c->eta, eta, 16 * sizeof(double), hipMemcpyHostToDevice, c->stream));
-    HIP_TRY(hipStreamSynchronize(c->stream));
+    HIP_TRY(hipMemsetAsync(c->big_seen, 0, sizeof(uint32_t), c->stream));
+    HIP_TRY(hipStreamSynchronize(c->stream));
+    c->big_launch_on = true;
     c->have_state = true;
     return DSM_OK;
 }
@@ -672,7 +679,7 @@
     if (esum) HIP_TRY(hipMemcpyAsync(esum, c->esum, 16 * sizeof(uint64_t), hipMemcpyDeviceToHost, c->stream));
     HIP_TRY(hipMemsetAsync(c->ntab, 0, t.size() * sizeof(uint32_t), c->stream));
     TRY(esum_reset(c));
-    HIP_TRY(hipMemsetAsync(c->big_count, 0, DSM_BIG_NT * DSM_BIG_NL * DSM_BIG_STRIDE * sizeof(uint32_t), c->stream));
+    HIP_TRY(hipMemsetAsync(c->big_count, 0, 2 * DSM_BIG_WORDS * sizeof(uint32_t), c->stream));
     HIP_TRY(hipStreamSynchronize(c->stream));
     if (ntab)
         for (size_t h = 0; h < NH; ++h)
@@ -681,6 +688,38 @@
                 for (int r = 0; r < c->ntab_rep; ++r) v += t[((size_t)r * NH + ((h * DSM_NTAB_HMUL + (s >> 4) * DSM_NTAB_SWZ) & (NH - 1))) * ld + s];
                 ntab[s * NH + h] = v;
             }
+    return DSM_OK;
+}
+
+extern "C" int dsm_ctx_debug_big_lists(dsm_ctx *c, uint32_t iter, uint32_t *kinds, uint32_t *per_sample)
+{
+    TRY(need(c, true, true));
+    const int spec = stats_spec(c);
+    if (spec < 2 || spec == 4) { dsm_set_error("debug_big_lists: needs the aggregated specification 2 or 3 (dsm_ctx_force_stats_spec)"); return DSM_ERR_UNSUPPORTED; }
+    if (!kinds || !per_sample) { dsm_set_error("debug_big_lists: null argument"); return DSM_ERR_ARG; }
+    BIND(c);
+    TRY(esum_reset(c));
+    TRY(k_stats_stage1(c, iter, false));
+    std::vector<uint32_t> cnt(DSM_BIG_WORDS);
+    HIP_TRY(hipMemcpyAsync(cnt.data(), big_count_cur(c), DSM_BIG_WORDS * sizeof(uint32_t), hipMemcpyDeviceToHost, c->stream));
+    HIP_TRY(hipMemsetAsync(c->ntab, 0, c->ntab_len * sizeof(uint32_t), c->stream));
+    TRY(esum_reset(c));
+    HIP_TRY(hipMemsetAsync(c->big_count, 0, 2 * DSM_BIG_WORDS * sizeof(uint32_t), c->stream));
+    HIP_TRY(hipStreamSynchronize(c->stream));
+    for (int k = 0; k < DSM_BIG_NT; ++k) kinds[k] = 0u;
+    for (int s = 0; s < c->S; ++s) per_sample[s] = 0u;
+    std::vector<unsigned long long> items;
+    for (int sub = 0; sub < DSM_BIG_NT * DSM_BIG_NL; ++sub) {
+        const size_t n = std::min<size_t>(cnt[(size_t)sub * DSM_BIG_STRIDE], c->big_seg);
+        if (!n) continue;
+        kinds[sub / DSM_BIG_NL] += (uint32_t)n;
+        items.resize(n);
+        HIP_TRY(hipMemcpy(items.data(), c->big_list + (size_t)sub * c->big_seg, n * sizeof(unsigned long long), hipMemcpyDeviceToHost));
+        for (size_t i = 0; i < n; ++i) {
+            const uint64_t s = (items[i] >> 2) / (uint64_t)c->V;
+            if (s < (uint64_t)c->S) ++per_sample[s];
+        }
+    }
     return DSM_OK;
 }
 
@@ -840,6 +879,15 @@
     std::vector<int> nb_prev(K, 0);
     std::vector<uint32_t> ic(K);
     std::vector<const uint32_t *> u(K, nullptr);
+    const bool big_opt = !batched && fuse_s2 && spec != 4;
+    if (big_opt && !lead->h_big_seen) HIP_TRY(hipHostMalloc((void **)&lead->h_big_seen, sizeof(uint32_t), hipHostMallocDefault));
+    auto big_launch = [&]() { return !big_opt || lead->big_launch_mode == 1 || (lead->big_launch_mode == -1 && lead->big_launch_on); };
+    auto big_window = [&](bool wait) -> int {
+        HIP_TRY(hipMemcpyAsync(lead->h_big_seen, lead->big_seen, sizeof(uint32_t), hipMemcpyDeviceToHost, lead->stream));
+        HIP_TRY(hipMemsetAsync(lead->big_seen, 0, sizeof(uint32_t), lead->stream));
+        if (wait) { HIP_TRY(hipStreamSynchronize(lead->stream)); lead->big_launch_on = *lead->h_big_seen != 0u; }
+        return DSM_OK;
+    };
     TRY(ch.each([&](dsm_ctx *c, int) -> int {
         TRY(alloc_traces(c, n_iter));
         HIP_TRY(hipMemsetAsync(c->nchange, 0, sizeof(int), c->stream));
@@ -852,19 +900,22 @@
     TRY(ch.launch([&](dsm_ctx *, int k) { return words[k].prefetch(); }));
     for (int it = 0; it < n_iter; ++it) {
         if (!batched && it && (it & 63) == 0 && lead->tau_neartie_mode == -1) { TRY(k_tau_rare_count(lead, true)); TRY(k_tau_neartie_hint(lead)); }
-        TRY(ch.launch([&](dsm_ctx *c, int k) { ic[k] = c->iter_ctr++; return agg ? k_stats_stage1(c, ic[k]) : k_stats_v1(c, ic[k]); }));
+        if (big_opt && it && (it & 63) == 0) TRY(big_window(true));
+        const bool big = big_launch();
+        TRY(ch.launch([&](dsm_ctx *c, int k) { ic[k] = c->iter_ctr++; return agg ? k_stats_stage1(c, ic[k], big) : k_stats_v1(c, ic[k]); }));
         if (agg && !fuse_s2) TRY(ch.launch([&](dsm_ctx *c, int k) { return k_stats_stage2(c, ic[k]); }));
         TRY(ch.launch([&](dsm_ctx *c, int k) {
-            return k_dirichlet(c, ic[k], c->gamma, c->gamma_trace + (size_t)it * sg, c->eta_new, c->eta_trace + (size_t)it * 16,
-                               prior_slot(c, it), it - 1, nb_prev[k], prior_slot(c, it - 1), fuse_s2 ? 1 : 0);
+            return k_dirichlet(c, ic[k], c->gamma_new, c->gamma_trace + (size_t)it * sg, c->eta_new, c->eta_trace + (size_t)it * 16,
+                               prior_slot(c, it), it - 1, nb_prev[k], prior_slot(c, it - 1), fuse_s2 ? 1 : 0, big_opt ? (big ? 0 : 1) : -1);
         }));
         TRY(ch.launch([&](dsm_ctx *, int k) { return words[k].acquire(it, &u[k]); }));
         TRY(ch.launch([&](dsm_ctx *c, int k) {
-            return k_tau_sweep(c, 3, c->gamma, c->eta, c->eta_new, c->tau_trace + (size_t)(it + 1) * c->V, nullptr, ic[k], &nb_prev[k], u[k]);
+            return k_tau_sweep(c, 3, c->gamma_new, c->eta, c->eta_new, c->tau_trace + (size_t)(it + 1) * c->V, nullptr, ic[k], &nb_prev[k], u[k]);
         }));
         TRY(ch.each([&](dsm_ctx *c, int k) -> int {
             TRY(words[k].release(it));
             std::swap(c->eta, c->eta_new);
+            std::swap(c->gamma, c->gamma_new);
             return DSM_OK;
         }));
     }
@@ -875,8 +926,10 @@
             return k_finalize(c, nb_prev[k], n_iter - 1, 0, prior_slot(c, n_iter - 1), c->gamma_trace + (size_t)(n_iter - 1) * sg,
                               c->eta_trace + (size_t)(n_iter - 1) * 16, 0, want_rare ? c->h_rare : nullptr);
         }));
+    if (big_opt && n_iter > 0) TRY(big_window(false));
     HIP_TRY(hipStreamSynchronize(lead->stream));
     if (want_rare) lead->tau_rare_n = *lead->h_rare;
+    if (big_opt && n_iter > 0) lead->big_launch_on = *lead->h_big_seen != 0u;
     return DSM_OK;
 }
 
@@ -1086,6 +1139,21 @@
     if (!c || mode < -1 || mode > 1) { dsm_set_error("set_tau_neartie: -1 (by the abundances), 0 or 1"); return DSM_ERR_ARG; }
     c->tau_neartie_mode = mode;
     return DSM_OK;
+}
+
+extern "C" int dsm_ctx_set_big_launch(dsm_ctx *c, int mode)
+{
+    if (!c || mode < -1 || mode > 1) { dsm_set_error("set_big_launch: -1 (by the chain's lists), 0 or 1"); return DSM_ERR_ARG; }
+    c->big_launch_mode = mode;
+    return DSM_OK;
+}
+
+extern "C" int dsm_ctx_get_big_launch(dsm_ctx *c)
+{
+    if (!c || c->G < 1) { dsm_set_error("get_big_launch: no chain state"); return DSM_ERR_STATE; }
+    const int spec = stats_spec(c);
+    if (!(spec >= 2 && spec != 4 && c->G < 10)) return 1;
+    return c->big_launch_mode == 1 || (c->big_launch_mode == -1 && c->big_launch_on) ? 1 : 0;
 }
 
 extern "C" int dsm_ctx_set_tau_screen(dsm_ctx *c, int on)
diff --git a/desman_amd/csrc/dsm_host.h b/desman_amd/csrc/dsm_host.h
--- a/desman_amd/csrc/dsm_host.h
+++ b/desman_amd/csrc/dsm_host.h
@@ -11,6 +11,7 @@
 #define DSM_BIG_NL 64
 #define DSM_BIG_STRIDE 16
 #define DSM_BIG_NT 3
+#define DSM_BIG_WORDS (DSM_BIG_NT * DSM_BIG_NL * DSM_BIG_STRIDE)
 #define DSM_U_CHUNK 8
 
 #define DSM_STATS_AGG 2
@@ -76,6 +77,12 @@
     unsigned long long *big_list = nullptr;
     uint32_t *big_count = nullptr;
     size_t big_cap = 0;
+    size_t big_seg = 0;
+    int big_par = 0;
+    int big_launch_mode = -1;
+    bool big_launch_on = true;
+    uint32_t *big_seen = nullptr;
+    uint32_t *h_big_seen = nullptr;
     int stats_grid = 0;
     int stats_grid_key = -1;
     int item_stride = 1;
@@ -89,6 +96,7 @@
     double *gamma = nullptr;
     double *eta = nullptr;
     double *eta_new = nullptr;
+    double *gamma_new = nullptr;
     bool have_state = false;
     double alpha = 0.1, delta = 0.1, epsilon = 1e-6;
     unsigned long long *sum_mu = nullptr;
@@ -188,12 +196,14 @@
 int k_tau_rare_count(dsm_ctx *c, bool wait);
 int tau_rare_from_host(const double *gamma, int S, int G);
 int k_stats(dsm_ctx *c, uint32_t iter);
-int k_stats_stage1(dsm_ctx *c, uint32_t iter);
+int k_stats_stage1(dsm_ctx *c, uint32_t iter, bool big_launch = true);
+static inline uint32_t *big_count_cur(const dsm_ctx *c) { return c->big_count + (size_t)c->big_par * DSM_BIG_WORDS; }
+static inline uint32_t *big_count_prev(const dsm_ctx *c) { return c->big_count + (size_t)(c->big_par ^ 1) * DSM_BIG_WORDS; }
 int k_stats_stage2(dsm_ctx *c, uint32_t iter);
 int k_binom_test(dsm_ctx *c, int kind, uint32_t n, const double *w, uint64_t seed, int nsamp, uint32_t *d_out, int spec);
 int k_esum_fold(dsm_ctx *c);
 int k_dirichlet(dsm_ctx *c, uint32_t iter, double *gamma_out, double *gamma_trace, double *eta_out, double *eta_trace,
-                double *prior_out, int fin_it, int fin_nblocks, const double *fin_prior, int do_s2 = 0);
+                double *prior_out, int fin_it, int fin_nblocks, const double *fin_prior, int do_s2 = 0, int big_left = -1);
 int k_prior(dsm_ctx *c, const double *gamma, const double *eta, double *prior_out);
 int k_prior_batch(dsm_ctx *c, const double *gamma, const double *eta, int n, double *prior_out);
 struct TauFinalRider { int nblocks, it; const double *prior, *gamma_src, *eta_src; };
diff --git a/desman_amd/csrc/dsm_stage2.h b/desman_amd/csrc/dsm_stage2.h
--- a/desman_amd/csrc/dsm_stage2.h
+++ b/desman_amd/csrc/dsm_stage2.h
@@ -1,5 +1,6 @@
 #pragma once
 #include "dsm_binom.h"
+#include "dsm_host.h"
 #include "log_table.h"
 
 #define S2_MAX_NODES 32
@@ -29,6 +30,83 @@
 
 S2Plan make_stage2_plan(int G);
 
+template <int SPEC>
+__device__ __forceinline__ void stats_big_item(uint32_t cell, int b, uint32_t xb, uint64_t t, const double *grow, int G, const double *es,
+                                               uint32_t iter, uint32_t k0, uint32_t k1, const double *rcp, const double2 *ltab,
+                                               uint32_t (&n)[4], uint32_t (&H)[4])
+{
+    H[0] = H[1] = H[2] = H[3] = 0u;
+    double Gam[4] = {0.0, 0.0, 0.0, 0.0};
+    for (int g = 0; g < G; ++g) {
+        const int a = (int)((t >> (2 * g)) & 3);
+        const double x = grow[g];
+#pragma unroll
+        for (int k = 0; k < 4; ++k) if (a == k) { H[k] |= 1u << g; Gam[k] = Gam[k] + x; }
+    }
+    double W[4];
+#pragma unroll
+    for (int a = 0; a < 4; ++a) W[a] = es[a * 4 + b] * Gam[a];
+    const double Wt = ((W[0] + W[1]) + W[2]) + W[3];
+    if (!(Wt > 0.0)) {
+#pragma unroll
+        for (int a = 0; a < 4; ++a) W[a] = Gam[a];
+    }
+    uint32_t cbase[4];
+    philox4x32_10(cell, 0u, iter, DSM_STREAM_STA1, k0, k1, cbase);
+    Xo128 rng = item_seed<SPEC>(cbase, (uint32_t)b, k0, k1);
+    bool defer = false;
+    mult4<true, SPEC>(rng, xb, W, n, rcp, ltab, defer);
+}
+
+struct BigLeft {
+    const uint32_t *count;
+    const unsigned long long *list;
+    size_t seg;
+    const int32_t *cnt_vs;
+    const uint64_t *tau;
+    const double *gamma, *eta;
+    uint32_t *seen;
+    int draw;
+    int V, S, G, v_off, V_tot;
+};
+#define BIG_LEFT_MAX_G 9
+struct BigLeftLds { uint32_t x[1 << BIG_LEFT_MAX_G]; uint32_t cnt[DSM_BIG_NT * DSM_BIG_NL]; double es[16]; };
+
+template <int SPEC>
+__device__ __forceinline__ void big_left_walk(const BigLeft &bl, BigLeftLds &w, uint32_t my_count, int s, int a_eta, unsigned long long *ef,
+                                              uint32_t iter, uint32_t k0, uint32_t k1, const double *rcp, const double2 *ltab)
+{
+    const int tid = threadIdx.x, nthr = blockDim.x;
+    if (tid < DSM_BIG_NT * DSM_BIG_NL) w.cnt[tid] = my_count;
+    if (tid < 16) w.es[tid] = bl.eta[tid];
+    if (s >= 0) for (int i = tid; i < (1 << bl.G); i += nthr) w.x[i] = 0u;
+    __syncthreads();
+    for (int sub = 0; sub < DSM_BIG_NT * DSM_BIG_NL; ++sub) {
+        const uint32_t cnt = w.cnt[sub];
+        const uint32_t nl = cnt < (uint32_t)bl.seg ? cnt : (uint32_t)bl.seg;
+        const unsigned long long *list = bl.list + (size_t)sub * bl.seg;
+        for (uint32_t i = tid; i < nl; i += nthr) {
+            const unsigned long long item = list[i];
+            const uint32_t cell = (uint32_t)(item >> 2);
+            const int b = (int)(item & 3ull);
+            const int si = (int)(cell / (uint32_t)bl.V_tot), v = (int)(cell - (uint32_t)si * (uint32_t)bl.V_tot) - bl.v_off;
+            if (s >= 0 && si != s) continue;
+            if ((unsigned)v >= (unsigned)bl.V || si >= bl.S) continue;
+            const uint32_t xb = (uint32_t)bl.cnt_vs[((size_t)v * bl.S + si) * 4 + b];
+            uint32_t n[4], H[4];
+            stats_big_item<SPEC>(cell, b, xb, bl.tau[v], bl.gamma + (size_t)si * bl.G, bl.G, w.es, iter, k0, k1, rcp, ltab, n, H);
+            if (s >= 0) {
+#pragma unroll
+                for (int a = 0; a < 4; ++a) if (n[a]) atomicAdd(&w.x[H[a]], n[a]);
+            } else {
+                const uint32_t na = a_eta == 0 ? n[0] : a_eta == 1 ? n[1] : a_eta == 2 ? n[2] : n[3];
+                if (na) atomicAdd(&ef[b], (unsigned long long)na);
+            }
+        }
+    }
+    __syncthreads();
+}
+
 #define S2_SMEM_BYTES (DSM_LOG_TAB_N * 16 + DSM_EXP_TAB_N * 8 + DSM_RCP_TAB_N * 8 + 32 * 8 + S2_TAB_ENTRIES * 4 + 32 * 4 + 5 * S2_MAX_NODES * 4)
 
 #ifdef DSM_AB_SWITCHES
@@ -38,7 +116,8 @@
 #define S2_CLK(row, k) do { } while (0)
 #endif
 template <int SPEC>
-__device__ __forceinline__ const uint32_t *stage2_sample(const Stage2Params &p, const S2Plan &pl, int s, char *smem, bool to_global, int part = 0)
+__device__ __forceinline__ const uint32_t *stage2_sample(const Stage2Params &p, const S2Plan &pl, int s, char *smem, bool to_global, int part = 0,
+                                                         bool left_on = false, const BigLeft &left = BigLeft{}, uint32_t left_my = 0u, BigLeftLds *lw = nullptr)
 {
     const int G = p.G, tid = threadIdx.x, nthr = blockDim.x;
     double2 *ltab = reinterpret_cast<double2 *>(smem);
@@ -72,7 +151,13 @@
         n_child[tid] = pl.child[tid];
     }
     for (int i = tid; i < S2_TAB_ENTRIES; i += nthr) tab[i] = 0u;
-    __syncthreads();
+    const uint32_t *lx = nullptr;
+    if (left_on) {
+        if (__syncthreads_or(left_my != 0u)) {
+            big_left_walk<SPEC>(left, *lw, left_my, s, 0, nullptr, p.iter, p.k0, p.k1, rcp, ltab);
+            lx = lw->x;
+        }
+    } else __syncthreads();
     S2_CLK(s, 1);
 
     const int nlev = pl.nlevels > 1 ? pl.nlevels - 1 : pl.nlevels;
@@ -107,6 +192,7 @@
                         if (m) { cell[r * cstride] = 0u; n += m; }
                     }
                 }
+                if (lx) n += lx[Hs];
             } else n = tab[base + j];
             if (w == 1) {
                 if (level == 0) leaf[lo] = n;
diff --git a/desman_amd/csrc/kernels_gibbs.hip b/desman_amd/csrc/kernels_gibbs.hip
--- a/desman_amd/csrc/kernels_gibbs.hip
+++ b/desman_amd/csrc/kernels_gibbs.hip
@@ -566,7 +566,7 @@
     Stage2Params s2;
 };
 
-__device__ __forceinline__ void dirichlet_body(const DirParams &q, const S2Plan &plan)
+__device__ __forceinline__ void dirichlet_body(const DirParams &q, const S2Plan &plan, const BigLeft &bl)
 {
     unsigned long long *__restrict__ sum_mu = q.sum_mu, *__restrict__ esum = q.esum;
     const int S = q.S, G = q.G;
@@ -579,6 +579,8 @@
     const FinalParams &fin = q.fin;
     const Stage2Params &s2 = q.s2;
     __shared__ __attribute__((aligned(16))) char smem_d[S2_SMEM_BYTES];
+    __shared__ BigLeftLds left_lds;
+    __shared__ unsigned long long ef[4];
     if (do_fin && (int)blockIdx.x == S + 4) {
         double *red = reinterpret_cast<double *>(smem_d), *redp = red + 256;
         int *flag = reinterpret_cast<int *>(redp + 256);
@@ -588,13 +590,31 @@
     const int row = blockIdx.x;
     const bool is_gamma = row < S;
     const uint32_t *leaf = nullptr;
+    const bool have_bl = bl.count != nullptr && do_s2;
+    const bool left = have_bl && bl.draw;
+    uint32_t left_my = 0u;
+    if (have_bl && (left || row == 0) && threadIdx.x < DSM_BIG_NT * DSM_BIG_NL) {
+        left_my = bl.count[threadIdx.x * DSM_BIG_STRIDE];
+        if (row == 0 && left_my && bl.seen) atomicOr(bl.seen, 1u);
+    }
     if (do_s2 && is_gamma)
-        leaf = do_s2 >= 3 ? stage2_sample<3>(s2, plan, row, smem_d, false) : stage2_sample<2>(s2, plan, row, smem_d, false);
+        leaf = do_s2 >= 3 ? stage2_sample<3>(s2, plan, row, smem_d, false, 0, left, bl, left_my, &left_lds)
+                          : stage2_sample<2>(s2, plan, row, smem_d, false, 0, left, bl, left_my, &left_lds);
     if (!is_gamma) {
         static_assert(DSM_ESUM_PARTS * 4 == 256, "one thread per (copy, observed base)");
-        unsigned long long *ef = reinterpret_cast<unsigned long long *>(smem_d);
         if (threadIdx.x < 4) ef[threadIdx.x] = 0ull;
-        __syncthreads();
+        if (left) {
+            if (__syncthreads_or(left_my != 0u)) {
+                const int tid = threadIdx.x;
+                double2 *ltab = reinterpret_cast<double2 *>(smem_d);
+                double *etab = reinterpret_cast<double *>(ltab + DSM_LOG_TAB_N), *rcp = etab + DSM_EXP_TAB_N;
+                if (tid < DSM_LOG_TAB_N) ltab[tid] = reinterpret_cast<const double2 *>(s2.log_tab)[tid];
+                if (tid < DSM_EXP_TAB_N) etab[tid] = s2.log_tab[2 * DSM_LOG_TAB_N + tid];
+                for (int k = tid; k < DSM_RCP_TAB_N; k += 256) rcp[k] = k ? 1.0 / (double)k : 0.0;
+                if (do_s2 >= 3) big_left_walk<3>(bl, left_lds, left_my, -1, row - S, ef, iter, k0, k1, rcp, ltab);
+                else big_left_walk<2>(bl, left_lds, left_my, -1, row - S, ef, iter, k0, k1, rcp, ltab);
+            }
+        } else __syncthreads();
         const int ob = threadIdx.x & 3, k = threadIdx.x >> 2;
         unsigned long long *pp = esum + 16 + k * 16 + ob * 4 + (row - S);
         const unsigned long long v = *pp;
@@ -611,7 +631,7 @@
         double shape;
         uint32_t vid;
         if (is_gamma) { vid = (uint32_t)(row * G + lane); shape = alpha + (double)(sum_mu[vid] + (leaf ? (unsigned long long)leaf[lane] : 0ull)); }
-        else { const int a = row - S; vid = (uint32_t)(SG + a * 4 + lane); shape = delta + (double)(esum[lane * 4 + a] + reinterpret_cast<const unsigned long long *>(smem_d)[lane]); }
+        else { const int a = row - S; vid = (uint32_t)(SG + a * 4 + lane); shape = delta + (double)(esum[lane * 4 + a] + ef[lane]); }
         y = gamma_variate(shape, vid, iter, k0, k1);
         if (zero_after) { if (is_gamma) sum_mu[row * G + lane] = 0ull; else esum[lane * 4 + (row - S)] = 0ull; }
     }
@@ -639,8 +659,8 @@
 #endif
 
 struct DirBatch { DirParams p[DSM_MAX_BATCH]; S2Plan plan; };
-__global__ __launch_bounds__(256) void dirichlet_kernel(DirParams q, S2Plan plan) { dirichlet_body(q, plan); }
-__global__ __launch_bounds__(256) void dirichlet_kernel_b(DirBatch b) { dirichlet_body(b.p[blockIdx.y], b.plan); }
+__global__ __launch_bounds__(256) void dirichlet_kernel(DirParams q, S2Plan plan, BigLeft bl) { dirichlet_body(q, plan, bl); }
+__global__ __launch_bounds__(256) void dirichlet_kernel_b(DirBatch b) { dirichlet_body(b.p[blockIdx.y], b.plan, BigLeft{}); }
 static_assert(sizeof(DirBatch) <= 4096, "kernarg segment");
 
 __global__ __launch_bounds__(256) void prior_kernel(const double *__restrict__ gamma, const double *__restrict__ eta,
@@ -1179,7 +1199,7 @@
 }
 
 int k_dirichlet(dsm_ctx *c, uint32_t iter, double *gamma_out, double *gamma_trace, double *eta_out, double *eta_trace,
-                double *prior_out, int fin_it, int fin_nblocks, const double *fin_prior, int do_s2)
+                double *prior_out, int fin_it, int fin_nblocks, const double *fin_prior, int do_s2, int big_left)
 {
     KTimer tm(c, DSM_K_DIRICH);
     double lg, le;
@@ -1194,7 +1214,16 @@
     if (do_s2) {
         s2.ntab = c->ntab; s2.rep = c->ntab_rep; s2.ld = c->ntab_ld; s2.gamma = c->gamma; s2.sum_mu = c->sum_mu; s2.log_tab = c->log_tab;
         s2.S = c->S; s2.G = c->G; s2.k0 = k0; s2.k1 = k1; s2.iter = iter; s2.hmul = DSM_NTAB_HMUL; s2.swz = DSM_NTAB_SWZ;
-        s2.big_count = c->big_count;
+        s2.big_count = big_count_prev(c);
+    }
+    BigLeft bl = {};
+    if (do_s2 && big_left >= 0 && g_batch.K == 0) {
+        if (big_left && (c->G > BIG_LEFT_MAX_G || gamma_out == c->gamma || eta_out == c->eta || c->shard_on || stats_spec(c) == 4)) {
+            dsm_set_error("k_dirichlet: the deferred items cannot be drawn in this launch"); return DSM_ERR_STATE;
+        }
+        bl.count = big_count_cur(c); bl.list = c->big_list; bl.seg = c->big_seg; bl.cnt_vs = c->cnt_vs; bl.tau = c->tau;
+        bl.gamma = c->gamma; bl.eta = c->eta; bl.seen = c->big_seen; bl.draw = big_left ? 1 : 0;
+        bl.V = c->V; bl.S = c->S; bl.G = c->G; bl.v_off = 0; bl.V_tot = c->V;
     }
     DirParams q;
     q.sum_mu = c->sum_mu; q.esum = c->esum; q.S = c->S; q.G = c->G;
@@ -1204,7 +1233,7 @@
     q.do_fin = do_fin; q.fin = fin; q.do_s2 = do_s2 ? stats_draw_version(stats_spec(c)) : 0; q.s2 = s2;
     if (g_batch.K == 0) {
         const S2Plan plan = do_s2 ? make_stage2_plan(c->G) : S2Plan{};
-        hipLaunchKernelGGL(dirichlet_kernel, dim3(c->S + 4 + do_fin), dim3(256), 0, c->stream, q, plan);
+        hipLaunchKernelGGL(dirichlet_kernel, dim3(c->S + 4 + do_fin), dim3(256), 0, c->stream, q, plan, bl);
     } else {
         static thread_local DirBatch acc;
         acc.p[g_batch.k] = q;
diff --git a/desman_amd/csrc/kernels_stats.hip b/desman_amd/csrc/kernels_stats.hip
--- a/desman_amd/csrc/kernels_stats.hip
+++ b/desman_amd/csrc/kernels_stats.hip
@@ -1,5 +1,6 @@
 #include "dsm_binom.h"
 #include "dsm_host.h"
+#include "dsm_stage2.h"
 #include "log_table.h"
 
 #include <string.h>
@@ -377,27 +378,8 @@
         uint32_t xb;
         if (p.pat_x) { uint32_t *xw = p.pat_x + ((size_t)v * 4 + b) * S + s; xb = *xw; *xw = 0u; }
         else xb = (uint32_t)p.cnt_vs[((size_t)v * S + s) * 4 + b];
-        uint32_t H[4] = {0, 0, 0, 0};
-        double Gam[4] = {0.0, 0.0, 0.0, 0.0};
-        for (int g = 0; g < G; ++g) {
-            const int a = (int)((t >> (2 * g)) & 3);
-            const double x = p.gamma[(size_t)s * G + g];
-#pragma unroll
-            for (int k = 0; k < 4; ++k) if (a == k) { H[k] |= 1u << g; Gam[k] = Gam[k] + x; }
-        }
-        double W[4];
-#pragma unroll
-        for (int a = 0; a < 4; ++a) W[a] = es[a * 4 + b] * Gam[a];
-        const double Wt = ((W[0] + W[1]) + W[2]) + W[3];
-        if (!(Wt > 0.0)) {
-#pragma unroll
-            for (int a = 0; a < 4; ++a) W[a] = Gam[a];
-        }
-        uint32_t n[4], cbase[4];
-        philox4x32_10(cell, 0u, p.iter, DSM_STREAM_STA1, p.k0, p.k1, cbase);
-        Xo128 rng = item_seed<SPEC>(cbase, (uint32_t)b, p.k0, p.k1);
-        bool defer = false;
-        mult4<true, SPEC>(rng, xb, W, n, rcp, ltab, defer);
+        uint32_t n[4], H[4];
+        stats_big_item<SPEC>(cell, b, xb, t, p.gamma + (size_t)s * G, G, es, p.iter, p.k0, p.k1, rcp, ltab, n, H);
         uint32_t *erow = eacc + (b * 4) * 256 + tid;
 #pragma unroll
         for (int a = 0; a < 4; ++a) {
@@ -439,8 +421,6 @@
 __global__ __launch_bounds__(256) void stats_big_kernel(StatsAggParams p) { stats_big_body<SPEC>(p); }
 template <int SPEC>
 __global__ __launch_bounds__(256) void stats_big_kernel_b(BatchArgs<StatsAggParams> b) { stats_big_body<SPEC>(b.p[blockIdx.y]); }
-
-#include "dsm_stage2.h"
 
 struct Stage2Batch { Stage2Params p[DSM_MAX_BATCH]; S2Plan plan; };
 template <int SPEC>
@@ -564,13 +544,14 @@
     if (c->big_list && c->big_cap == need) return DSM_OK;
     if (c->big_list) { (void)hipFree(c->big_list); c->big_list = nullptr; }
     if (!c->big_count) {
-        hipError_t e = hipMalloc((void **)&c->big_count, DSM_BIG_NT * DSM_BIG_NL * DSM_BIG_STRIDE * sizeof(uint32_t));
+        hipError_t e = hipMalloc((void **)&c->big_count, 2 * DSM_BIG_WORDS * sizeof(uint32_t));
         if (e != hipSuccess) { dsm_set_error("hipMalloc failed: %s", hipGetErrorString(e)); return DSM_ERR_NOMEM; }
     }
     hipError_t e = hipMalloc((void **)&c->big_list, need * sizeof(unsigned long long));
     if (e != hipSuccess) { dsm_set_error("hipMalloc(%zu B) failed: %s", need * 8, hipGetErrorString(e)); return DSM_ERR_NOMEM; }
     c->big_cap = need;
-    HIP_TRY(hipMemsetAsync(c->big_count, 0, DSM_BIG_NT * DSM_BIG_NL * DSM_BIG_STRIDE * sizeof(uint32_t), c->stream));
+    HIP_TRY(hipMemsetAsync(c->big_count, 0, 2 * DSM_BIG_WORDS * sizeof(uint32_t), c->stream));
+    c->big_par = 0;
     return DSM_OK;
 }
 
@@ -601,7 +582,7 @@
     return DSM_OK;
 }
 
-int k_stats_stage1(dsm_ctx *c, uint32_t iter)
+int k_stats_stage1(dsm_ctx *c, uint32_t iter, bool big_launch)
 {
     int r = ensure_ntab(c);
     if (r != DSM_OK) return r;
@@ -643,6 +624,8 @@
     const size_t seg = (size_t)std::min<long>((long)V * S * 4, ((grid + DSM_BIG_NL - 1) / DSM_BIG_NL) * per_wg);
     r = ensure_big_list(c, seg);
     if (r != DSM_OK) return r;
+    c->big_par ^= 1;
+    c->big_seg = seg;
     StatsAggParams p;
     p.cnt_vs = c->cnt_vs; p.tau = c->tau; p.gamma = c->gamma; p.eta = c->eta;
     p.V = V; p.S = S; p.G = G; p.big_seg = seg;
@@ -651,7 +634,7 @@
     p.ntab = c->ntab; p.rep = c->ntab_rep; p.ld = c->ntab_ld; p.esum = c->esum; p.log_tab = c->log_tab;
     p.xcd = 0;
     p.hmul = DSM_NTAB_HMUL; p.swz = DSM_NTAB_SWZ;
-    p.big_list = c->big_list; p.big_count = c->big_count;
+    p.big_list = c->big_list; p.big_count = big_count_cur(c);
     p.pat_rep = nullptr; p.pat_x = nullptr; p.pat_list = nullptr; p.pat_n = nullptr;
     if (pat) {
         r = ensure_pat(c);
@@ -711,6 +694,7 @@
         void *args[] = {(void *)&p};
         HIP_TRY(hipLaunchKernel(fn, dim3(grid), dim3(256), args, sh, c->stream));
     }
+    if (!big_launch) return DSM_OK;
     KTimer tm(c, DSM_K_STATSBIG);
     if (spec >= 3) hipLaunchKernelGGL(stats_big_kernel<3>, dim3(big_grid), dim3(256), 0, c->stream, p);
     else hipLaunchKernelGGL(stats_big_kernel<2>, dim3(big_grid), dim3(256), 0, c->stream, p);
@@ -751,7 +735,7 @@
     p.ntab = c->ntab; p.rep = c->ntab_rep; p.ld = c->ntab_ld; p.gamma = c->gamma; p.sum_mu = c->sum_mu; p.log_tab = c->log_tab;
     p.S = c->S; p.G = c->G; p.hmul = DSM_NTAB_HMUL; p.swz = DSM_NTAB_SWZ;
     p.k0 = (uint32_t)c->ctr_seed; p.k1 = (uint32_t)(c->ctr_seed >> 32); p.iter = iter;
-    p.big_count = c->big_count;
+    p.big_count = big_count_prev(c);
     const int nthr = c->G >= 10 ? 1024 : 256;
     const bool v3 = stats_draw_version(stats_spec(c)) >= 3;
     p.nsplit = 1; p.scratch = nullptr; p.ticket = nullptr;
diff --git a/include/desman_hip.h b/include/desman_hip.h
--- a/include/desman_hip.h
+++ b/include/desman_hip.h
@@ -177,6 +177,9 @@
 int dsm_ctx_set_nmft_persist(dsm_ctx *ctx, int mode);
 int dsm_ctx_set_tau_screen(dsm_ctx *ctx, int on);
 int dsm_ctx_set_tau_neartie(dsm_ctx *ctx, int mode);
+int dsm_ctx_set_big_launch(dsm_ctx *ctx, int mode);
+int dsm_ctx_get_big_launch(dsm_ctx *ctx);
+int dsm_ctx_debug_big_lists(dsm_ctx *ctx, uint32_t iter, uint32_t *kinds, uint32_t *per_sample);
 int dsm_ctx_tau_launch_info(dsm_ctx *ctx, int *launched, int *resident);
 int dsm_ctx_get_counters(dsm_ctx *ctx, uint64_t *ctr_seed, uint32_t *iter_ctr);
 int dsm_ctx_set_counters(dsm_ctx *ctx, uint64_t ctr_seed, uint32_t iter_ctr);
```

Measured after the change: 6.364 billion V*S updates/s (median of 3 runs). Within noise of the previous version (+0.1%).
